# andrewginns/quorum

Measured on AMD Instinct MI355X. Metric: proxied req/sec (whole node) + p50 TTFT, 2-backend concatenate stream at 1/2/4/8 GPU, higher is better.
Workload: dtype bytes (utf-8 SSE text; no float compute)

## Files before the change

quorum_amd/csrc/qmx_engine.cpp:

```cpp
#include "qmx_env.h"
#include "qmx_engine.h"

#include <cstdlib>
#include <ctime>

#include <algorithm>
#include <cstdio>
#include <cstring>
#include <stdexcept>

namespace qmx {

const char* kDeltaSuffix = "\"}, \"finish_reason\": null}]}\n\n";
const char* kFinalSuffix = "\"}, \"finish_reason\": \"stop\"}]}\n\n";

TagSet make_tagset(const std::vector<std::string>& tags) {
  TagSet ts;
  std::memset(&ts, 0, sizeof(ts));
  std::vector<std::string> seen;
  for (const auto& t0 : tags) {
    std::string t;
    for (char c : t0) t.push_back((char)lower_ascii((uint8_t)c));
    if (std::find(seen.begin(), seen.end(), t) != seen.end()) continue;
    for (char ch : t) {
// ... 271 lines not shown
  int slot;
  if (!free_.empty()) {
    slot = free_.back();
    free_.pop_back();
  } else {
    slot = (int)meta_.size();
    meta_.emplace_back();
    core_.emplace_back();
  }
  open_reserved(slot, index, filter, emit, gen);
  return slot;
}

void HostEngine::reserve(int k, std::vector<int>& out) {
  std::lock_guard<std::mutex> g(mu_);
  for (int i = 0; i < k; ++i) {
    if (!free_.empty()) {
      out.push_back(free_.back());
      free_.pop_back();
    } else {
      out.push_back((int)meta_.size());
      meta_.emplace_back();
      core_.emplace_back();
    }
  }
}

void HostEngine::open_reserved(int slot, int index, bool filter, bool emit, uint32_t* gen) {
  auto recycle = [](std::string& x) {
    if (x.capacity() > (64u << 10)) std::string().swap(x);
    else x.clear();
  };
  Meta& m = meta_[slot];
  m.gen += 1;
  m.live = true;
  m.dirty = m.eof = m.closed = m.busy = false;
  m.fresh = true;
  recycle(m.incoming);
  if (gen) *gen = m.gen;
  SlotCore& c = core_[slot];
  c.filter = filter;
  c.emit = emit;
  c.started = c.aborted = c.done = false;
  c.index = index;
  recycle(c.carry);
  c.fs = FilterState();
  recycle(c.content);
  recycle(c.tpl_pre);
  recycle(c.tpl_suf);
}

void HostEngine::feed(int slot, const std::string& data) {
  std::lock_guard<std::mutex> g(mu_);
  feed_locked(slot, data);
}

void HostEngine::finish(int slot) {
  std::lock_guard<std::mutex> g(mu_);
  finish_locked(slot);
}

void HostEngine::release(int slot) {
  std::lock_guard<std::mutex> g(mu_);
  release_locked(slot);
}

void HostEngine::apply_ops(std::vector<EngineOp>& ops, bool move_data) {
  std::lock_guard<std::mutex> g(mu_);
  for (auto& op : ops) {
    if (op.kind == EngineOp::FEED) {
      if (move_data) feed_locked_move(op.slot, op.data);
      else feed_locked(op.slot, op.data);
    }
    else if (op.kind == EngineOp::FINISH) finish_locked(op.slot);
    else release_locked(op.slot);
  }
}

void HostEngine::feed_locked(int slot, const std::string& data) {
  if (slot < 0 || slot >= (int)meta_.size() || !meta_[slot].live) return;
  Meta& m = meta_[slot];
  m.incoming += data;
  bytes_in_ += data.size();
  if (!m.dirty) {
    m.dirty = true;
    m.t_dirty = mono_s();
    dirty_.push_back(slot);
  }
}

void HostEngine::feed_locked_move(int slot, std::string& data) {
  if (slot < 0 || slot >= (int)meta_.size() || !meta_[slot].live) return;
  if (!meta_[slot].incoming.empty()) return feed_locked(slot, data);
  bytes_in_ += data.size();
  meta_[slot].incoming.swap(data);
  Meta& m = meta_[slot];
  if (!m.dirty) {
    m.dirty = true;
    m.t_dirty = mono_s();
    dirty_.push_back(slot);
  }
}

void HostEngine::finish_locked(int slot) {
  if (slot < 0 || slot >= (int)meta_.size() || !meta_[slot].live) return;
  Meta& m = meta_[slot];
  m.eof = true;
  if (!m.dirty) {
    m.dirty = true;
    m.t_dirty = mono_s();
    dirty_.push_back(slot);
  }
}

void HostEngine::release_locked(int slot) {
  if (slot < 0 || slot >= (int)meta_.size() || !meta_[slot].live) return;
  meta_[slot].live = false;
  meta_[slot].incoming.clear();
  pending_free_.push_back(slot);
}

int HostEngine::submit_finalize(const std::vector<int>& slots, bool strip, bool texts, const std::string& joiner,
                                int64_t created) {
  std::lock_guard<std::mutex> g(mu_);
  FinalizeReq r{++next_fid_, slots, strip, texts, joiner, created};
  fin_.push_back(std::move(r));
  return next_fid_;
}

bool HostEngine::has_work() {
  std::lock_guard<std::mutex> g(mu_);
  if (!fin_.empty()) return true;
  for (int s : dirty_)
    if (!meta_[s].busy) return true;
  return false;
}

bool HostEngine::pending(int slot) {
  std::lock_guard<std::mutex> g(mu_);
  if (slot < 0 || slot >= (int)meta_.size()) return false;
  const Meta& m = meta_[slot];
  return m.live && (m.dirty || m.busy || !m.incoming.empty());
}

bool HostEngine::job_take(Job& j, bool allow_fin) {
  j.work.clear();
  j.fin.clear();
  thread_local std::vector<int> keep;
  keep.clear();
  std::lock_guard<std::mutex> g(mu_);
  for (int s : pending_free_) {
    if (meta_[s].busy) {
      keep.push_back(s);
      continue;
    }
    on_free(s);
    free_.push_back(s);
  }
  pending_free_.swap(keep);
  keep.clear();
  j.work.reserve(dirty_.size());
  double now = 0;
  for (int s : dirty_) {
    Meta& m = meta_[s];
    if (m.busy && m.live) {
      keep.push_back(s);
      continue;
    }
    m.dirty = false;
    if (!m.live) continue;
    if (m.t_dirty > 0) {
      if (now == 0) now = mono_s();
      take_wait_s_ += now - m.t_dirty;
      ++takes_;
    }
    Work w{s, std::string(), m.eof, m.fresh};
    w.data.swap(m.incoming);
    m.fresh = false;
    m.busy = true;
    j.work.push_back(std::move(w));
  }
  dirty_.swap(keep);
  if (allow_fin) j.fin.swap(fin_);
  if (!j.work.empty() || !j.fin.empty()) ++ticks_;
  return !j.work.empty() || !j.fin.empty();
}

void HostEngine::job_finish(Job& j, std::vector<SlotResult>& results, std::vector<int>& taken) {
  size_t out = 0;
  for (auto& r : results) out += r.size();
  for (auto& w : j.work) taken.push_back(w.slot);
  std::lock_guard<std::mutex> g(mu_);
  bytes_out_ += out;
  for (auto& r : results) r.gen = meta_[r.slot].gen;
}

bool HostEngine::tick(int64_t created, std::vector<SlotResult>& results, std::vector<FinalizeRes>& fres, int lane,
                      std::vector<int>* taken) {
  thread_local Job j;
  thread_local std::vector<int> slots;
  slots.clear();
  if (!job_take(j, true)) return false;
  run_tick(j.work, j.fin, created, results, fres, lane);
  std::vector<int>& tk = taken ? *taken : slots;
  job_finish(j, results, tk);
  if (!taken) settle(slots);
  return true;
}

void HostEngine::settle(const std::vector<int>& taken) {
  std::lock_guard<std::mutex> g(mu_);
  for (int s : taken) meta_[s].busy = false;
}

std::string HostEngine::text(int slot) {
  if (slot < 0 || slot >= (int)nslots()) return std::string();
  const SlotCore& c = core_[slot];
  return c.aborted ? std::string() : c.content;
}

size_t HostEngine::content_size(int slot) {
  if (slot < 0 || slot >= (int)nslots()) return 0;
  return core_[slot].content.size();
}

void HostEngine::set_remote_content(int slot, const std::string* bytes, size_t len, bool ) {
  if (slot < 0 || slot >= (int)nslots()) return;
  core_[slot].content = bytes ? *bytes : std::string(len, '\0');
}

std::unordered_map<std::string, double> HostEngine::stats() {
  std::lock_guard<std::mutex> g(mu_);
  return {{"ticks", (double)ticks_}, {"bytes_in", (double)bytes_in_}, {"bytes_out", (double)bytes_out_},
          {"takes", (double)takes_}, {"take_wait_us", take_wait_s_ * 1e6},
          {"slots", (double)meta_.size()}, {"free", (double)free_.size()}};
// ... 18 lines not shown
  }
}

}

namespace qmx {

struct AsyncCpuEngine::Done {
  std::vector<SlotResult> results;
  std::vector<FinalizeRes> fres;
  std::atomic<bool> ready{false};
};

AsyncCpuEngine::AsyncCpuEngine(const std::vector<std::string>& tags) : CpuEngine(tags) {
  th_ = std::thread([this] { run(); });
}

AsyncCpuEngine::~AsyncCpuEngine() {
  {
    std::lock_guard<std::mutex> g(qmu_);
    stop_ = true;
  }
  qcv_.notify_all();
  if (th_.joinable()) th_.join();
}

void AsyncCpuEngine::job_post(Job& j) {
  auto d = std::make_shared<Done>();
  j.impl = d;
  inflight_.fetch_add(1, std::memory_order_acq_rel);
  {
    std::lock_guard<std::mutex> g(qmu_);
    q_.push_back(&j);
  }
  qcv_.notify_one();
}

void AsyncCpuEngine::run() {
  for (;;) {
    Job* j = nullptr;
    {
      std::unique_lock<std::mutex> lk(qmu_);
      qcv_.wait(lk, [this] { return stop_ || !q_.empty(); });
      if (q_.empty()) return;
      j = q_.front();
      q_.erase(q_.begin());
    }
    auto d = std::static_pointer_cast<Done>(j->impl);
    run_tick(j->work, j->fin, j->created, d->results, d->fres, 0);
    d->ready.store(true, std::memory_order_release);
  }
}

bool AsyncCpuEngine::job_ready(Job& j, double* expect_us) {
  if (expect_us) *expect_us = 5.0;
  auto d = std::static_pointer_cast<Done>(j.impl);
  return !d || d->ready.load(std::memory_order_acquire);
}

void AsyncCpuEngine::job_complete(Job& j, std::vector<SlotResult>& results, std::vector<FinalizeRes>& fres) {
  auto d = std::static_pointer_cast<Done>(j.impl);
  if (!d) return;
  for (auto& r : d->results) results.push_back(std::move(r));
  for (auto& f : d->fres) fres.push_back(std::move(f));
  j.impl.reset();
  inflight_.fetch_sub(1, std::memory_order_acq_rel);
}

}
```

quorum_amd/csrc/qmx_engine.h:

```cpp
#pragma once
#include <stdint.h>

#include <atomic>
#include <condition_variable>
#include <memory>
#include <thread>
#include <mutex>
#include <string>
#include <unordered_map>
#include <stdexcept>
#include <unordered_set>
#include <vector>

#include "qmx_text.h"

namespace qmx {

enum ResultFlags : int { RF_DONE = 1, RF_ABORTED = 2, RF_ESCALATED = 4 };

TagSet make_tagset(const std::vector<std::string>& tags);

struct FilterState {
  int depth = 0;
  int tail_len = 0;
// ... 82 lines not shown

template <class T>
class SlotTable {
 public:
  static constexpr int kShift = 8, kChunk = 1 << kShift, kMaxChunks = 4096;
  SlotTable() : chunks_(new std::unique_ptr<T[]>[kMaxChunks]) {}
  T& operator[](size_t i) { return chunks_[i >> kShift][i & (kChunk - 1)]; }
  const T& operator[](size_t i) const { return chunks_[i >> kShift][i & (kChunk - 1)]; }
  size_t size() const { return n_.load(std::memory_order_acquire); }
  void emplace_back() {
    const size_t n = n_.load(std::memory_order_relaxed);
    if ((n >> kShift) >= (size_t)kMaxChunks) throw std::length_error("slot table full");
    if ((n & (kChunk - 1)) == 0) chunks_[n >> kShift].reset(new T[kChunk]());
    n_.store(n + 1, std::memory_order_release);
  }

 private:
  std::unique_ptr<std::unique_ptr<T[]>[]> chunks_;
  std::atomic<size_t> n_{0};
};

class HostEngine {
 public:
  explicit HostEngine(const std::vector<std::string>& tags);
  virtual ~HostEngine() = default;

  int open(int index, bool filter, bool emit, uint32_t* gen = nullptr);
  void reserve(int k, std::vector<int>& out);
  void open_reserved(int slot, int index, bool filter, bool emit, uint32_t* gen = nullptr);
  void feed(int slot, const std::string& data);
  void finish(int slot);
  void release(int slot);
  void apply_ops(std::vector<EngineOp>& ops, bool move_data = false);
  int submit_finalize(const std::vector<int>& slots, bool strip, bool texts, const std::string& joiner,
                      int64_t created);
  bool has_work();
  bool pending(int slot);
  bool tick(int64_t created, std::vector<SlotResult>& results, std::vector<FinalizeRes>& fres, int lane = 0,
            std::vector<int>* taken = nullptr);
  void settle(const std::vector<int>& taken);

  struct Work {
    int slot;
    std::string data;
    bool eof;
    bool fresh;
  };
  struct Job {
    std::vector<Work> work;
    std::vector<FinalizeReq> fin;
    int64_t created = 0;
    int lane = 0;
    bool live = false;
    std::shared_ptr<void> impl;
  };
  virtual bool pipelined() const { return false; }
  bool pipeline_ = false;
  bool job_take(Job& j, bool allow_fin);
  virtual void job_prepare(Job&) {}
  virtual void job_post(Job&) {}
  virtual void job_wait_near(Job&) {}
  virtual void job_complete(Job&, std::vector<SlotResult>&, std::vector<FinalizeRes>&) {}
  void job_finish(Job& j, std::vector<SlotResult>& results, std::vector<int>& taken);
  virtual bool async_jobs() const { return false; }
  virtual bool job_ready(Job&, double* expect_us = nullptr) {
    if (expect_us) *expect_us = 0;
    return true;
  }
  virtual int free_doors() const { return 1; }
  virtual std::string text(int slot);
  virtual std::unordered_map<std::string, double> stats();
  virtual void* content_device_ptr(int , size_t* cap) {
    *cap = 0;
    return nullptr;
  }
  virtual size_t content_size(int slot);
  virtual void set_remote_content(int slot, const std::string* bytes, size_t len, bool host_copied = false);

  const TagSet& tagset() const { return ts_; }

 protected:
  virtual void run_tick(std::vector<Work>& work, std::vector<FinalizeReq>& fin, int64_t created,
                        std::vector<SlotResult>& results, std::vector<FinalizeRes>& fres, int lane) = 0;
  virtual void on_free(int ) {}

  void feed_locked(int slot, const std::string& data);
  void feed_locked_move(int slot, std::string& data);
  void finish_locked(int slot);
  void release_locked(int slot);

  struct Meta {
    bool live = false;
    bool dirty = false;
    bool eof = false;
    bool fresh = true;
    bool closed = false;
    bool busy = false;
    uint32_t gen = 0;
    double t_dirty = 0;
    std::string incoming;
  };

  TagSet ts_;
  std::mutex mu_;
  SlotTable<Meta> meta_;
  SlotTable<SlotCore> core_;
  size_t nslots() const { return core_.size(); }
  std::vector<int> free_, pending_free_;
  std::vector<int> dirty_;
  std::vector<FinalizeReq> fin_;
  int next_fid_ = 0;
  uint64_t ticks_ = 0, bytes_in_ = 0, bytes_out_ = 0, takes_ = 0;
  double take_wait_s_ = 0;
};

class CpuEngine : public HostEngine {
 public:
  explicit CpuEngine(const std::vector<std::string>& tags) : HostEngine(tags) {}
  bool pipelined() const override { return pipeline_; }
  void job_complete(Job& j, std::vector<SlotResult>& results, std::vector<FinalizeRes>& fres) override {
    run_tick(j.work, j.fin, j.created, results, fres, j.lane);
  }

 protected:
  void run_tick(std::vector<Work>& work, std::vector<FinalizeReq>& fin, int64_t created,
                std::vector<SlotResult>& results, std::vector<FinalizeRes>& fres, int lane) override;
};

class AsyncCpuEngine : public CpuEngine {
 public:
  explicit AsyncCpuEngine(const std::vector<std::string>& tags);
  ~AsyncCpuEngine() override;
  bool async_jobs() const override { return true; }
  void job_post(Job& j) override;
  bool job_ready(Job& j, double* expect_us = nullptr) override;
  void job_complete(Job& j, std::vector<SlotResult>& results, std::vector<FinalizeRes>& fres) override;
  int free_doors() const override { return 2 - inflight_.load(std::memory_order_acquire); }

 private:
  struct Done;
  void run();
  std::mutex qmu_;
  std::condition_variable qcv_;
  std::vector<Job*> q_;
  bool stop_ = false;
  std::atomic<int> inflight_{0};
  std::thread th_;
};

void finalize_texts(const TagSet& ts, const std::vector<std::string>& texts, const FinalizeReq& r,
                    FinalizeRes& out);

}
```

quorum_amd/csrc/qmx_hip.h:

```cpp
#pragma once
#include <hip/hip_runtime.h>

#include <atomic>
#include <chrono>
#include <cstddef>
#include <functional>
#include <memory>
#include <mutex>
#include <shared_mutex>
#include <vector>

#include "qmx_engine.h"
#include "qmx_streams.h"

namespace qmx {

struct WorkItem {
  uint32_t slot, in_off, in_len, out_off, out_cap, flags, index, content_len;
};
struct WorkResult {
  uint32_t consumed, out_len, status, content_len;
  uint32_t seq;
  uint32_t pad;
  uint64_t t0, t1;
// ... 154 lines not shown
  uint64_t launches = 0, items = 0, h2d_bytes = 0, d2h_bytes = 0;
  uint64_t s3_full = 0, s3_tpl = 0, s3_events = 0, stage_n = 0;
  uint64_t s3_cyc_full = 0, s3_cyc_tpl = 0, s3_cyc_lex = 0, s3_hole = 0, s3_cyc_hole = 0;
  uint64_t s3a_unres = 0;
  double kernel_ms = 0.0, host_prep_us = 0, gpu_wait_us = 0, process_us = 0;
  double first_result_us = 0;
  double item_us = 0, start_spread_us = 0;
  double items_host_us = 0;
  double relay_us = 0, pickup_us = 0, grid_span_us = 0, grid_ticks = 0;
  double stage_us[38] = {0};
  double clk_cycles = 0, clk_us = 0;
  FinItem* h_fin = nullptr;
  size_t fin_cap = 0;
  FinResult* h_finres = nullptr;
  size_t finres_cap = 0;
  FinText* h_fint = nullptr;
  size_t fint_cap = 0;
  uint8_t* h_fin_in = nullptr;
  size_t fin_in_cap = 0;
  uint8_t* h_fout = nullptr;
  size_t fout_cap = 0;
  uint32_t* h_tl = nullptr;
  size_t tl_cap = 0;
  uint8_t* d_join = nullptr;
  size_t join_cap = 0;
  uint8_t* d_fout = nullptr;
  size_t dfout_cap = 0;
  uint8_t* d_segs = nullptr;
  size_t segs_cap = 0;
  uint64_t fin_launches = 0, fin_items = 0, fin_host = 0;
  uint64_t fin_staged = 0;
  uint32_t seq = 0;
  double ema_us = 40.0;
  double span_ema_us = 30.0;
  double lead_ema_us = 8.0;
  double post_seen_us = 0, done_host_us = 0, hop_ticks = 0;
  double clo = -1e300, chi = 1e300, clo_prev = -1e300, cwin_t0 = 0, cwin_sum = 0, cwin_n = 0;
  bool timing_pending = false;
  uint64_t poll_fallbacks = 0;
  PDoor* h_door = nullptr;
  PCtl* d_ctl = nullptr;
  bool p_running = false;
  uint32_t p_gen = 0;
  double p_last_post = 0;
  uint64_t p_revivals = 0;
  uint64_t p_launches = 0, p_ticks = 0;
};

class HipEngine : public HostEngine {
 public:
  HipEngine(const std::vector<std::string>& tags, int device, int tile_bytes, int max_slots, int content_cap,
            int lanes = 1, HipGrid* grid = nullptr, int door = -1, int ndoors = 1);
  ~HipEngine() override;
  bool job_ready(Job& j, double* expect_us = nullptr) override;
  bool async_jobs() const override { return grid_ != nullptr; }
  int free_doors() const override;
  std::string text(int slot) override;
  void* content_device_ptr(int slot, size_t* cap) override;
  size_t content_size(int slot) override;
  void set_remote_content(int slot, const std::string* bytes, size_t len, bool host_copied = false) override;
  void set_remote_hbm_direct(bool on) { remote_hbm_direct_ = on; }
  bool remote_hbm_direct() const { return remote_hbm_direct_; }
  std::unordered_map<std::string, double> kernel_stats();
  int lanes() const { return (int)lanes_.size(); }
  void host_open(int slot);

 protected:
  void run_tick(std::vector<Work>& work, std::vector<FinalizeReq>& fin, int64_t created,
                std::vector<SlotResult>& results, std::vector<FinalizeRes>& fres, int lane) override;
  void on_free(int slot) override;

 public:
  bool pipelined() const override { return poll_ && pipeline_; }
  void job_prepare(Job& j) override;
  void job_post(Job& j) override;
  void job_wait_near(Job& j) override;
  void job_complete(Job& j, std::vector<SlotResult>& results, std::vector<FinalizeRes>& fres) override;

 private:
  struct HipJob;
  HipJob& hjob(Job& j);
  void prepare(HipJob& J);
  void post(HipJob& J);
  void wait_near(HipJob& J);
  void complete(HipJob& J, std::vector<SlotResult>& results, std::vector<FinalizeRes>& fres);
  void escalate(int slot, bool fresh);
  void finalize_host(const FinalizeReq& r, std::vector<FinalizeRes>& out);
  std::vector<const FinalizeReq*> prep_finalize(TickLane& L, std::vector<FinalizeReq>& fin,
                                                std::vector<const FinalizeReq*>& host);
  void collect_finalize(TickLane& L, const std::vector<const FinalizeReq*>& gpu, std::vector<FinalizeRes>& out);
  void wait_stream(TickLane& L);
  void wait_results(TickLane& L, int n, int m, uint32_t seq, const WorkResult* res,
                    std::chrono::steady_clock::time_point t0, const std::function<void(int)>& on_item);
  void collect_timing(TickLane& L);
  void ensure_in(TickLane::Buf& B, size_t bytes);
  void ensure_out(TickLane& L, size_t bytes);
  void build_params(TickLane& L, int64_t created);
  std::string device_content(int slot, uint32_t len);
  uint32_t next_seq(TickLane& L);
  void ensure_persistent(TickLane& L);
  void stop_persistent(TickLane& L);
  void retire_host(void* p);
  void retire_dev(void* p);
  void note_alloc(double t0, size_t bytes);
  std::atomic<uint64_t> allocs_{0}, alloc_bytes_{0};
  std::atomic<double> alloc_us_{0.0}, alloc_max_us_{0.0};

 public:
  void* halloc(size_t bytes);
  void* dalloc(size_t bytes);

 private:
  std::vector<void*> grave_host_, grave_dev_;
  std::mutex grave_mu_;

  int device_;
  int tile_;
  int max_slots_;
  uint32_t content_cap_;
  KParams base_params_;
  std::vector<std::unique_ptr<TickLane>> lanes_;
  DevSlot* d_state_ = nullptr;
  uint8_t* d_content_ = nullptr;
  std::vector<uint8_t> host_mode_;
  std::vector<uint8_t> remote_host_;
  std::vector<uint32_t> content_len_;
  std::atomic<uint64_t> escalations_{0}, fin_host_{0}, remote_dev_{0}, remote_staged_{0}, remote_copied_{0},
      remote_copied_inline_{0}, light_opens_{0},
      requeues_{0};
  bool remote_hbm_direct_ = true;
  int spin_us_ = 0;
  bool poll_ = true;
  int poll_us_ = 1;
  bool persistent_ = true;
  bool views_ = true;
  bool keep_stale_records_ = false;
  bool stage_timing_ = false;
  int p_grid_ = 64;
  int p_idle_ms_ = 50;
  HipGrid* grid_ = nullptr;
  int door_ = -1;
  int ndoors_ = 1;
  std::vector<char> door_busy_;

 public:
  bool persistent() const { return persistent_; }
// ... 6 lines not shown
```

quorum_amd/csrc/qmx_hip.hip:

```cpp
#include "qmx_env.h"
#include "qmx_hip.h"
#include "qmx_streams.h"

#include <rocprofiler-sdk-roctx/roctx.h>

#include <sched.h>
#include <sys/prctl.h>
#include <time.h>

#include <chrono>
#include <thread>

#include "qmx_lex.h"

#include <algorithm>
#include <cstdio>
#include <cstdlib>
#include <cstring>
#include <stdexcept>
#include <string>

namespace qmx {

#define HIP_CHECK(x)                                                                       \
// ... 2679 lines not shown
    if (ndone == n && null_done) {
      last = 1e3 * (steady_s() - t0);
      break;
    }
    sched_yield();
  }
  const double t1 = steady_s();
  bool drained = false;
  while (steady_s() - t1 < 5.0) {
    bool all = hipEventQuery(ev) == hipSuccess;
    for (int i = 0; i < n && all; ++i) all = done(i);
    if (all) {
      drained = true;
      break;
    }
    std::this_thread::sleep_for(std::chrono::milliseconds(1));
  }
  if (drained) {
    for (hipStream_t s : st) stream_destroy(s, StreamKind::Shared);
    hipEventDestroy(ev);
    hipFree(dsrc);
    hipHostFree(marks);
  }
  return {{"streams", (double)n}, {"completed", (double)ndone}, {"null_stream_copy_done", null_done ? 1.0 : 0.0},
          {"all_done_ms", last}, {"drained", drained ? 1.0 : 0.0}};
}

std::unordered_map<std::string, double> stream_stats() {
  const char* hq = env_get("GPU_MAX_HW_QUEUES");
  const int queues = hq ? std::max(1, atoi(hq)) : 4;
  const int ex = g_streams_excl.load(), sh = g_streams_shared.load();
  const bool own = exclusive_queues();
  return {{"streams_shared", (double)sh},
          {"streams_exclusive", (double)ex},
          {"streams_created", (double)g_streams_created.load()},
          {"hw_queues_per_priority", (double)queues},
          {"grid_queue_exclusive", own ? 1.0 : 0.0},
          {"grid_queue_ok", own && ex <= queues ? 1.0 : 0.0}};
}

void HipEngine::wait_stream(TickLane& L) {
  HIP_CHECK(hipEventRecord(L.evb, L.stream));
  if (spin_us_ > 0) {
    const auto t0 = std::chrono::steady_clock::now();
    while (hipEventQuery(L.evb) == hipErrorNotReady) {
      if (std::chrono::steady_clock::now() - t0 > std::chrono::microseconds(spin_us_)) break;
      sched_yield();
    }
  }
  HIP_CHECK(hipEventSynchronize(L.evb));
}

void HipEngine::wait_results(TickLane& L, int n, int m, uint32_t seq, const WorkResult* res,
                             std::chrono::steady_clock::time_point t0, const std::function<void(int)>& on_item) {
  using HC = std::chrono::steady_clock;
  static thread_local bool slack = (prctl(PR_SET_TIMERSLACK, 1000UL, 0, 0, 0), true);
  (void)slack;
  auto nap = [](double us) {
    if (us < 1) return;
    timespec ts{0, (long)(us * 1000)};
    nanosleep(&ts, nullptr);
  };
  auto done = [&](int& i) {
    while (i < n && __atomic_load_n(&res[i].seq, __ATOMIC_ACQUIRE) == seq) on_item(i++);
    while (i >= n && i < n + m && __atomic_load_n(&L.h_finres[i - n].seq, __ATOMIC_ACQUIRE) == seq) ++i;
    return i == n + m;
  };
  int i = 0;
  bool revived = false;
  double revive_at = 2e5;
  nap(0.6 * L.ema_us - 6.0 - std::chrono::duration<double, std::micro>(HC::now() - t0).count());
  while (!done(i)) {
    const double el = std::chrono::duration<double, std::micro>(HC::now() - t0).count();
    if (grid_) {
      if (el > revive_at) {
        revive_at = el + 1e5;
        grid_->revive_if_exited();
      }
      if (el > 1e7)
        throw std::runtime_error("tick results missing after 10 s (door " + std::to_string(door_) + ", seq " +
                                 std::to_string(seq) + ", relayed " +
                                 std::to_string(__atomic_load_n(&L.h_door->relayed, __ATOMIC_ACQUIRE)) + ")");
      nap(el < 2e3 ? poll_us_ : 50.0);
      continue;
    }
    if (L.p_running && !revived && el > 2.0 * L.ema_us + 500.0) {
      const uint32_t ex = __atomic_load_n(&L.h_door->exits, __ATOMIC_ACQUIRE);
      const uint32_t rl = __atomic_load_n(&L.h_door->relayed, __ATOMIC_ACQUIRE);
      if ((ex >> 16) == 1 && (ex & 0xffffu) == (L.p_gen & 0xffffu) && rl != seq) {
        uint32_t seq0 = seq - 1;
        if (seq0 == 0) seq0 = (uint32_t)-1;
        HIP_CHECK(hipStreamSynchronize(L.stream));
        L.h_door->base = seq0;
        hipLaunchKernelGGL(qmx_tick_persistent<2>, dim3(p_grid_), dim3(BS), 0, L.stream, L.h_door, L.d_ctl, p_grid_,
                           ++L.p_gen, (uint32_t)p_idle_ms_ * 100000u, 0);
        HIP_CHECK(hipGetLastError());
        L.p_last_post = steady_s();
        ++L.p_launches;
        ++L.p_revivals;
        revived = true;
        continue;
      }
    }
    if (el > (L.p_running ? 1e6 : 4.0 * L.ema_us + 2000.0)) {
      if (L.p_running) stop_persistent(L);
      else HIP_CHECK(hipStreamSynchronize(L.stream));
      ++L.poll_fallbacks;
      if (!done(i)) {
        std::string why = "tick results missing after the lane drained (seq " + std::to_string(seq) + ", " +
                          std::to_string(i) + "/" + std::to_string(n + m) + " published";
        if (L.h_door)
          why += "; grid: relayed " + std::to_string(__atomic_load_n(&L.h_door->relayed, __ATOMIC_ACQUIRE)) +
                 ", exits " + std::to_string(L.h_door->exits) + ", last idle exit after " +
                 std::to_string(L.h_door->idle_limit_hit_us) + " us, launches " + std::to_string(L.p_launches) +
                 ", posted " + std::to_string(L.h_door->posted);
        throw std::runtime_error(why + ")");
      }
      break;
    }
    if (el < spin_us_) {
      sched_yield();
      continue;
    }
    nap(poll_us_);
  }
  const double tot = std::chrono::duration<double, std::micro>(HC::now() - t0).count();
  L.ema_us = 0.85 * L.ema_us + 0.15 * std::min(tot, 2000.0);
}

void HipEngine::collect_timing(TickLane& L) {
  if (!L.timing_pending) return;
  L.timing_pending = false;
  HIP_CHECK(hipEventSynchronize(L.ev1));
  float ms = 0.f;
  if (hipEventElapsedTime(&ms, L.ev0, L.ev1) == hipSuccess) L.kernel_ms += ms;
}

HipEngine::HipEngine(const std::vector<std::string>& tags, int device, int tile_bytes, int max_slots,
                     int content_cap, int lanes, HipGrid* grid, int door, int ndoors)
    : HostEngine(tags),
      device_(device),
      tile_(std::min(std::max(tile_bytes, 1024), TILE_MAX) & ~15),
      max_slots_(max_slots),
      content_cap_((uint32_t)content_cap),
      grid_(grid),
      door_(door),
      ndoors_(grid ? std::min(std::max(ndoors, 1), 2) : 1) {
  HIP_CHECK(hipSetDevice(device_));
  if (grid_ && (door_ < 0 || door_ + ndoors_ > grid_->doors())) throw std::invalid_argument("HipEngine: door out of range");
  if (grid_) lanes = 1;
  door_busy_.assign(ndoors_, 0);
  if (const char* sp = env_get("QMX_WAIT_SPIN_US")) spin_us_ = atoi(sp);
  if (const char* w = env_get("QMX_WAIT")) poll_ = std::string(w) != "event";
  if (const char* pu = env_get("QMX_POLL_US")) poll_us_ = std::max(1, atoi(pu));
  if (const char* gs = env_get("QMX_GPU_SHARERS")) persistent_ = atoi(gs) <= 1;
  if (const char* pe = env_get("QMX_PERSISTENT")) persistent_ = atoi(pe) != 0;
  if (const char* va = env_get("QMX_VIEWS")) views_ = atoi(va) != 0;
  keep_stale_records_ = env_get("QMX_DEBUG_STALE_RECORDS") != nullptr;
  stage_timing_ = env_get("QMX_STAGE_TIMING") != nullptr;
  if (const char* pw = env_get("QMX_PERSISTENT_WG")) p_grid_ = std::min(std::max(8, atoi(pw)), 1024);
  if (const char* pi = env_get("QMX_PERSISTENT_IDLE_MS")) p_idle_ms_ = std::min(std::max(5, atoi(pi)), 1000);
  {
    const char* hq = env_get("GPU_MAX_HW_QUEUES");
    const int queues = hq ? std::max(1, atoi(hq)) : 4;
    if (persistent_ && lanes > (exclusive_queues() ? queues : queues - 1)) persistent_ = false;
  }
  if (grid_) {
    persistent_ = false;
    poll_ = true;
  }
  HIP_CHECK(hipMalloc(&d_state_, sizeof(DevSlot) * (size_t)max_slots_));
  HIP_CHECK(hipMemset(d_state_, 0, sizeof(DevSlot) * (size_t)max_slots_));
  HIP_CHECK(hipMalloc(&d_content_, (size_t)content_cap_ * (size_t)max_slots_));

  std::memset(&base_params_, 0, sizeof(base_params_));
  base_params_.ts = ts_;
  base_params_.npat = 2 * ts_.n;
  {
    int next = 1;
    for (int b = 0; b < 256; ++b) base_params_.code[b] = 95;
// ... 303 lines not shown
  }
  content_len_[slot] = (uint32_t)len;
}

void HipEngine::host_open(int slot) {
  if (slot >= 0 && slot < max_slots_) {
    host_mode_[slot] = 1;
    remote_host_[slot] = 0;
    content_len_[slot] = 0;
  }
  ++light_opens_;
}

void HipEngine::escalate(int slot, bool fresh) {
  SlotCore& c = core_[slot];
  if (!fresh) {
    DevSlot ds;
    HIP_CHECK(hipMemcpy(&ds, d_state_ + slot, sizeof(DevSlot), hipMemcpyDeviceToHost));
    c.fs.depth = ds.depth;
    c.fs.tail_len = ds.tail_len;
    std::memcpy(c.fs.tail, ds.tail, kMaxTail);
  } else {
    c.fs = FilterState();
  }
  if (!remote_host_[slot]) c.content = device_content(slot, content_len_[slot]);
  remote_host_[slot] = 0;
  host_mode_[slot] = 1;
  ++escalations_;
}

std::string HipEngine::text(int slot) {
  if (slot < 0 || slot >= (int)nslots()) return std::string();
  const SlotCore& c = core_[slot];
  if (c.aborted) return std::string();
  if (slot >= max_slots_ || host_mode_[slot] || remote_host_[slot]) return c.content;
  return device_content(slot, content_len_[slot]);
}

struct HipEngine::HipJob {
  struct Pending {
    int slot;
    size_t carry_len;
    size_t submitted;
    bool eof_sent;
    Work* w;
  };
  std::vector<Work>* work = nullptr;
  std::vector<FinalizeReq>* fin = nullptr;
  int64_t created = 0;
  int lane = 0, n = 0, m = 0;
  int dk = 0;
  uint32_t seq = 0;
  bool persist = false, new_params = false, posted = false;
  std::vector<Pending> pend;
  std::vector<int> requeue;
  std::vector<Work*> order;
  std::vector<Work*> b[8];
  std::vector<const FinalizeReq*> fin_gpu, fin_host;
  std::vector<SlotResult> host_results;
  TickLane::Buf* B = nullptr;
  TickLane::OutArena* arena = nullptr;
  size_t in_off = 0;
  std::chrono::steady_clock::time_point tp0, tp1;
};

void HipEngine::prepare(HipJob& J) {
  TickLane& L = *lanes_[(size_t)J.lane % lanes_.size()];
  std::lock_guard<std::mutex> lg(L.mu);
  using HC = std::chrono::steady_clock;
  J.tp0 = HC::now();
  J.pend.clear();
  J.requeue.clear();
  J.order.clear();
  J.host_results.clear();
  J.fin_gpu.clear();
  J.fin_host.clear();
  J.posted = false;
  std::vector<Work>& work = *J.work;
  TickLane::Buf* bp = nullptr;
  for (TickLane::Buf& b : L.bufs)
    if (!b.busy) {
      bp = &b;
      break;
    }
  if (!bp) throw std::logic_error("tick prepared with both buffer sets in use");
  TickLane::Buf& B = *bp;
  B.busy = true;
  J.B = &B;
  size_t out_need = 0;
  for (auto& w : work) {
    size_t tot = core_[w.slot].carry.size() + w.data.size();
    size_t sub = std::min(tot, (size_t)tile_);
    out_need += ((12 * sub + 1024) + 15) & ~(size_t)15;
  }
  ensure_in(B, work.size() * (size_t)TILE_MAX + kSpecTile + 64);
  ensure_out(L, out_need + 64);
  J.arena = L.out;
  J.arena->refs.fetch_add(1, std::memory_order_relaxed);
  if (work.size() > B.items_cap) {
    retire_host(B.h_items);
    retire_host(B.h_res);
    B.items_cap = work.size() * 2;
    B.h_items = (WorkItem*)halloc(sizeof(WorkItem) * B.items_cap);
    B.h_res = (WorkResult*)halloc(sizeof(WorkResult) * B.items_cap);
    std::memset((void*)B.h_res, 0, sizeof(WorkResult) * B.items_cap);
  }
// ... 35 lines not shown
    size_t cl = c.carry.size(), tot = cl + w.data.size();
    size_t sub = std::min(tot, (size_t)tile_);
    bool eof_sent = w.eof && sub == tot;
    in_off = (size_t)n * TILE_MAX;
    size_t a = std::min(cl, sub);
    std::memcpy(B.h_in + in_off, c.carry.data(), a);
    if (sub > a) std::memcpy(B.h_in + in_off + a, w.data.data(), sub - a);
    WorkItem& it = B.h_items[n];
    it.slot = (uint32_t)slot;
    it.in_off = (uint32_t)in_off;
    it.in_len = (uint32_t)sub;
    it.out_off = (uint32_t)out_off;
    it.out_cap = (uint32_t)(12 * sub + 1024);
    it.flags = (eof_sent ? WF_EOF : 0) | (c.filter ? WF_FILTER : 0) | (c.emit ? WF_EMIT : 0) |
               (c.started ? WF_STARTED : 0) | (w.fresh ? WF_FRESH : 0);
    it.index = (uint32_t)c.index;
    if (c.index >= 0 && c.index < kBackendTpl && !(pub_mask & (1u << c.index))) {
      pub_mask |= 1u << c.index;
      it.flags |= WF_PUBLISH;
    }
    it.content_len = content_len_[slot];
    in_bytes += sub;
    out_off += ((size_t)it.out_cap + 15) & ~(size_t)15;
    J.pend.push_back({slot, cl, sub, eof_sent, &w});
    ++n;
  }
  J.n = n;
  J.in_off = in_bytes;
  J.fin_gpu = prep_finalize(L, *J.fin, J.fin_host);
  J.m = (int)J.fin_gpu.size();
  if (!keep_stale_records_) {
    for (int i = 0; i < n; ++i) __atomic_store_n(&B.h_res[i].seq, 0u, __ATOMIC_RELAXED);
    for (int i = 0; i < J.m; ++i) __atomic_store_n(&L.h_finres[i].seq, 0u, __ATOMIC_RELAXED);
  }
  if (n + J.m > 0) {
    if (J.created != L.params_created) {
      build_params(L, J.created);
      L.params_created = J.created;
      ++L.params_ver;
    }
    unsigned long long* const dbg0 = L.params.dbg;
    L.params.dbg = nullptr;
    if (stage_timing_) {
      if (B.dbg_cap < (size_t)n) {
        if (B.h_dbg) retire_host(B.h_dbg);
        B.dbg_cap = std::max((size_t)n, B.items_cap);
        HIP_CHECK(hipHostMalloc((void**)&B.h_dbg, sizeof(unsigned long long) * kDbg * B.dbg_cap, hipHostMallocMapped));
      }
      std::memset(B.h_dbg, 0, sizeof(unsigned long long) * kDbg * n);
      L.params.dbg = B.h_dbg;
    }
    if (L.params.dbg != dbg0) ++L.params_ver;
  }
  J.tp1 = HC::now();
  L.host_prep_us += std::chrono::duration<double, std::micro>(J.tp1 - J.tp0).count();
}

void HipEngine::post(HipJob& J) {
  if (J.n + J.m == 0) return;
  TickLane& L = *lanes_[(size_t)J.lane % lanes_.size()];
  std::lock_guard<std::mutex> lg(L.mu);
  TickLane::Buf& B = *J.B;
  J.persist = grid_ || (persistent_ && poll_);
  if (!J.persist && L.p_running) stop_persistent(L);
  J.new_params = B.params_ver != L.params_ver;
  if (J.new_params) {
    std::memcpy(B.h_params, &L.params, sizeof(KParams));
    if (!J.persist) HIP_CHECK(hipMemcpyAsync(B.d_params, B.h_params, sizeof(KParams), hipMemcpyHostToDevice, L.stream));
    B.params_ver = L.params_ver;
  }
  J.tp1 = std::chrono::steady_clock::now();
  roctxRangePushA("qmx_tick");
  L.h2d_bytes += J.in_off;
  J.dk = 0;
  if (grid_) {
    while (J.dk < ndoors_ && door_busy_[J.dk]) ++J.dk;
    if (J.dk == ndoors_) throw std::logic_error("tick posted with every door of the engine busy");
  }
  const uint32_t par = L.tpl_launches[J.dk] & 1;
  BackendTpl* const tpl = L.d_btpl + (size_t)J.dk * 2 * kBackendTpl;
  FinArgs fa{L.h_fin, L.h_fint, L.h_fin_in, L.d_join, L.d_fout, L.h_fout, L.h_finres, L.h_tl, (int2*)L.d_segs};
  if (grid_) {
    auto guard = grid_->post_guard();
    PDoor* door = grid_->door(door_ + J.dk);
    door_busy_[J.dk] = 1;
    uint32_t s = door->posted + 1;
    if (s == 0) s = 1;
    J.seq = s;
    TickDesc& d = door->d;
    d.items = B.h_items;
    d.in = B.h_in;
    d.out = J.arena->p;
    d.res = B.h_res;
    d.params = B.d_params;
    d.params_src = J.new_params ? B.h_params : nullptr;
    d.btpl_rd = tpl + (size_t)(par ^ 1) * kBackendTpl;
    d.btpl_wr = tpl + (size_t)par * kBackendTpl;
    d.fa = fa;
    d.state = d_state_;
    d.content = d_content_;
    d.seq = s;
    d.n_tick = (uint32_t)J.n;
    d.n_fin = (uint32_t)J.m;
    d.stop = 0;
    __atomic_store_n(&door->posted, s, __ATOMIC_RELEASE);
    grid_->note_post();
    ++L.p_ticks;
    J.posted = true;
    return;
  }
  if (J.persist) ensure_persistent(L);
  J.seq = next_seq(L);
  if (!poll_) HIP_CHECK(hipEventRecord(L.ev0, L.stream));
  if (J.persist) {
    TickDesc& d = L.h_door->d;
    d.items = B.h_items;
    d.in = B.h_in;
    d.out = J.arena->p;
    d.res = B.h_res;
    d.params = B.d_params;
    d.params_src = J.new_params ? B.h_params : nullptr;
    d.btpl_rd = tpl + (size_t)(par ^ 1) * kBackendTpl;
    d.btpl_wr = tpl + (size_t)par * kBackendTpl;
    d.fa = fa;
    d.state = d_state_;
    d.content = d_content_;
    d.seq = J.seq;
    d.n_tick = (uint32_t)J.n;
    d.n_fin = (uint32_t)J.m;
    d.stop = 0;
    __atomic_store_n(&L.h_door->posted, J.seq, __ATOMIC_RELEASE);
    L.p_last_post = steady_s();
    ++L.p_ticks;
  } else {
    hipLaunchKernelGGL(qmx_tick_kernel, dim3(J.n + J.m), dim3(BS), 0, L.stream, B.h_items, B.h_in, J.arena->p,
                       B.h_res, d_state_, d_content_, B.d_params, J.seq, (uint32_t)J.n, fa,
                       tpl + (size_t)(par ^ 1) * kBackendTpl, tpl + (size_t)par * kBackendTpl);
    HIP_CHECK(hipGetLastError());
  }
  J.posted = true;
}

void HipEngine::wait_near(HipJob& J) {
  if (!J.posted) return;
  TickLane& L = *lanes_[(size_t)J.lane % lanes_.size()];
  const double el = std::chrono::duration<double, std::micro>(std::chrono::steady_clock::now() - J.tp1).count();
  const double prep = L.launches ? L.host_prep_us / (double)L.launches : 5.0;
  const double target = L.span_ema_us + 6.0 - prep;
  if (target - el >= 2.0) {
    timespec ts{0, (long)((target - el) * 1000)};
    nanosleep(&ts, nullptr);
  }
}

void HipEngine::complete(HipJob& J, std::vector<SlotResult>& results, std::vector<FinalizeRes>& fres) {
  TickLane& L = *lanes_[(size_t)J.lane % lanes_.size()];
  std::lock_guard<std::mutex> lg(L.mu);
  using HC = std::chrono::steady_clock;
  for (auto& r : J.host_results) results.push_back(std::move(r));
  J.host_results.clear();
  const int n = J.n, m = J.m;
  TickLane::Buf& B = *J.B;
  int n_done = 0;
  auto process_item = [&](int i) {
    HipJob::Pending& p = J.pend[i];
    SlotCore& c = core_[p.slot];
    const WorkResult r = B.h_res[i];
    Work& w = *p.w;
    auto keep_remainder = [&](size_t consumed) {
      const size_t cl = p.carry_len;
      if (consumed < cl) {
        c.carry.erase(0, consumed);
        c.carry += w.data;
      } else {
        c.carry.assign(w.data, consumed - cl, std::string::npos);
      }
    };
    bool no_progress = (r.status & WS_ESCALATE) ||
                       (p.submitted == (size_t)tile_ && r.consumed == 0 && !(r.status & (WS_DONE | WS_ABORTED)));
    if (no_progress) {
      escalate(p.slot, w.fresh);
      keep_remainder(0);
      std::string all;
      all.swap(c.carry);
      bool was_closed = c.done || c.aborted;
      std::string o;
      process_slot(ts_, c, (const uint8_t*)all.data(), all.size(), w.eof, J.created, o);
      int flags = (c.done ? RF_DONE : 0) | (c.aborted ? RF_ABORTED : 0) | RF_ESCALATED;
      if (!o.empty() || ((flags & (RF_DONE | RF_ABORTED)) && !was_closed)) results.push_back({p.slot, std::move(o), flags});
      return;
    }
    if (r.status & WS_STARTED) c.started = true;
    content_len_[p.slot] = r.content_len;
    int flags = 0;
    if (r.status & WS_ABORTED) {
      c.aborted = true;
      c.carry.clear();
      flags |= RF_ABORTED;
    } else {
      keep_remainder(r.consumed);
      if (r.status & WS_DONE) {
        c.done = true;
        c.carry.clear();
        flags |= RF_DONE;
      } else if ((r.status & WS_MORE) || p.submitted < p.carry_len + w.data.size()) {
        J.requeue.push_back(p.slot);
        if (r.status & WS_MORE) ++requeues_;
      }
    }
    L.d2h_bytes += r.out_len;
    const char* bytes = (const char*)J.arena->p + B.h_items[i].out_off;
    if (r.out_len && !views_) {
      results.push_back({p.slot, std::string(bytes, r.out_len), flags});
    } else if (r.out_len) {
      SlotResult x{p.slot, std::string(), flags};
      x.view = bytes;
      x.view_len = r.out_len;
      x.hold = ViewRef(&J.arena->refs);
      results.push_back(std::move(x));
    } else if (flags) {
      results.push_back({p.slot, std::string(), flags});
    }
  };
  if (J.posted) {
    for (const FinalizeReq* r : J.fin_host) finalize_host(*r, fres);
    if (poll_) {
      wait_results(L, n, m, J.seq, B.h_res, J.tp1, [&](int i) {
        const auto ti = HC::now();
        if (n_done == 0) L.first_result_us += std::chrono::duration<double, std::micro>(ti - J.tp1).count();
        if (i == n_done) process_item(n_done++);
        L.items_host_us += std::chrono::duration<double, std::micro>(HC::now() - ti).count();
      });
      uint64_t a = ~0ull, b = 0, t0max = 0;
      double item_ticks = 0;
      for (int i = 0; i < n; ++i) {
        a = std::min(a, B.h_res[i].t0);
        b = std::max(b, B.h_res[i].t1);
        t0max = std::max(t0max, B.h_res[i].t0);
        item_ticks += (double)(B.h_res[i].t1 - B.h_res[i].t0);
      }
      if (n > 0) {
        L.item_us += item_ticks * 1e-2 / n;
        L.start_spread_us += (double)(t0max - a) * 1e-2;
      }
      if (J.persist && n > 0) {
        const PDoor* dr = grid_ ? grid_->door(door_ + J.dk) : L.h_door;
        const uint64_t ts = __atomic_load_n(&dr->t_seen, __ATOMIC_ACQUIRE);
        const uint64_t tr = __atomic_load_n(&dr->t_relayed, __ATOMIC_ACQUIRE);
        if (ts && tr >= ts && a >= tr && b >= a) {
          L.lead_ema_us = 0.85 * L.lead_ema_us + 0.15 * std::min((double)(a - ts) * 1e-2, 500.0);
          if (grid_) {
            const double post_h = std::chrono::duration<double, std::micro>(J.tp1.time_since_epoch()).count();
            const double now_h = std::chrono::duration<double, std::micro>(HC::now().time_since_epoch()).count();
            const double lo = post_h - (double)ts * 1e-2, hi = now_h - (double)b * 1e-2;
            if (now_h - L.cwin_t0 > 1e5) {
              L.clo_prev = L.clo;
              if (L.clo > -1e299 && L.chi < 1e299 && L.chi >= L.clo) {
                L.cwin_sum += L.chi - L.clo;
                ++L.cwin_n;
              }
              L.clo = -1e300;
              L.chi = 1e300;
              L.cwin_t0 = now_h;
            }
            L.clo = std::max(L.clo, lo);
            L.chi = std::min(L.chi, hi);
            const double off = std::max(L.clo, L.clo_prev);
            const double seen_h = (double)ts * 1e-2 + off, done_h = (double)b * 1e-2 + off;
            if (seen_h >= post_h - 5.0 && now_h >= done_h - 5.0) {
              L.post_seen_us += seen_h - post_h;
              L.done_host_us += now_h - done_h;
              ++L.hop_ticks;
            }
          }
          L.relay_us += (double)(tr - ts) * 1e-2;
          L.pickup_us += (double)(a - tr) * 1e-2;
          L.grid_span_us += (double)(b - ts) * 1e-2;
          ++L.grid_ticks;
        }
      }
      for (int i = 0; i < m; ++i) {
        a = std::min(a, L.h_finres[i].t0);
        b = std::max(b, L.h_finres[i].t1);
      }
      if (b > a) {
        L.kernel_ms += (double)(b - a) * 1e-5;
        L.span_ema_us = 0.85 * L.span_ema_us + 0.15 * std::min((double)(b - a) * 1e-2, 2000.0);
      }
    } else {
      HIP_CHECK(hipEventRecord(L.ev1, L.stream));
      wait_stream(L);
      L.timing_pending = true;
      collect_timing(L);
    }
    roctxRangePop();
    L.gpu_wait_us += std::chrono::duration<double, std::micro>(HC::now() - J.tp1).count();
    ++L.launches;
    ++L.tpl_launches[J.dk];
    if (grid_) door_busy_[J.dk] = 0;
    L.items += n;
    if (m > 0) {
      ++L.fin_launches;
      L.fin_items += m;
    }
    if (L.params.dbg && L.params.dbg == B.h_dbg) {
      for (int i = 0; i < n; ++i) {
        const unsigned long long* d = B.h_dbg + kDbg * i;
        if (d[12] > d[11] && d[10] > d[0]) {
          L.clk_cycles += (double)(d[12] - d[11]);
          L.clk_us += (double)(d[10] - d[0]) * 0.01;
        }
        int prev = 0;
        for (int k = 1; k < 11; ++k) {
          if (!d[k]) continue;
          L.stage_us[k] += (double)(d[k] - d[prev]) * 0.01;
          prev = k;
        }
        auto sub = [&](int slot, int a, int b) {
          if (d[a] && d[b] && d[b] >= d[a]) L.stage_us[slot] += (double)(d[b] - d[a]) * 0.01;
        };
        sub(11, 3, 21);
        sub(12, 21, 22);
        sub(13, 22, 4);
        sub(14, 5, 23);
        sub(15, 23, 24);
        sub(16, 23, 25);
        sub(17, 25, 24);
        sub(18, 9, 26);
        sub(19, 26, 10);
        sub(21, 5, 28);
        sub(22, 28, 29);
        sub(23, 29, 23);
        sub(24, 25, 30);
        sub(25, 30, 31);
        sub(26, 31, 24);
        sub(27, 24, 32);
        sub(28, 32, 33);
        sub(29, 33, 7);
        sub(30, 3, 34);
        sub(31, 34, 21);
        sub(32, 3, 35);
        sub(33, 35, 36);
        sub(34, 36, 34);
        sub(35, 35, 38);
        sub(36, 38, 39);
        sub(37, 39, 36);
        if (d[27] && d[27] >= B.h_res[i].t1 && B.h_res[i].t1) L.stage_us[20] += (double)(d[27] - B.h_res[i].t1) * 0.01;
      }
      L.stage_n += n;
      for (int i = 0; i < n; ++i) {
        L.s3_full += B.h_dbg[kDbg * i + 13];
        L.s3_tpl += B.h_dbg[kDbg * i + 14];
        L.s3_events += B.h_dbg[kDbg * i + 15];
        L.s3_cyc_full += B.h_dbg[kDbg * i + 16];
        L.s3_cyc_tpl += B.h_dbg[kDbg * i + 17];
        L.s3_cyc_lex += B.h_dbg[kDbg * i + 18];
        L.s3_hole += B.h_dbg[kDbg * i + 19];
        L.s3_cyc_hole += B.h_dbg[kDbg * i + 20];
        L.s3a_unres += B.h_dbg[kDbg * i + 37];
      }
    }
  }
  for (; n_done < n; ++n_done) process_item(n_done);
  if (m > 0) collect_finalize(L, J.fin_gpu, fres);
  if (!J.posted)
    for (const FinalizeReq* r : J.fin_host) finalize_host(*r, fres);
  if (!J.requeue.empty()) {
    std::lock_guard<std::mutex> g(mu_);
    for (int s : J.requeue) {
      Meta& mt = meta_[s];
      if (!mt.live || mt.dirty) continue;
      mt.dirty = true;
      dirty_.push_back(s);
    }
  }
  J.arena->refs.fetch_sub(1, std::memory_order_release);
  J.B->busy = false;
  L.process_us += std::chrono::duration<double, std::micro>(HC::now() - J.tp0).count();
}

void HipEngine::run_tick(std::vector<Work>& work, std::vector<FinalizeReq>& fin, int64_t created,
                         std::vector<SlotResult>& results, std::vector<FinalizeRes>& fres, int lane) {
  thread_local HipJob J;
  J.work = &work;
  J.fin = &fin;
  J.created = created;
  J.lane = lane;
  prepare(J);
  post(J);
  complete(J, results, fres);
}

HipEngine::HipJob& HipEngine::hjob(Job& j) {
  if (!j.impl) j.impl = std::make_shared<HipJob>();
  HipJob& J = *std::static_pointer_cast<HipJob>(j.impl);
  J.work = &j.work;
  J.fin = &j.fin;
  J.created = j.created;
  J.lane = j.lane;
  return J;
}
int HipEngine::free_doors() const {
  int k = 0;
  for (char b : door_busy_) k += !b;
  return k;
}

bool HipEngine::job_ready(Job& j, double* expect_us) {
  HipJob& J = hjob(j);
  if (expect_us) *expect_us = 0;
  if (!J.posted) return true;
  TickLane& L = *lanes_[(size_t)J.lane % lanes_.size()];
  const WorkResult* res = J.B->h_res;
  for (int i = 0; i < J.n; ++i)
    if (__atomic_load_n(&res[i].seq, __ATOMIC_ACQUIRE) != J.seq) goto pending;
  for (int i = 0; i < J.m; ++i)
    if (__atomic_load_n(&L.h_finres[i].seq, __ATOMIC_ACQUIRE) != J.seq) goto pending;
  return true;
pending:
  if (expect_us)
    *expect_us = L.lead_ema_us + L.span_ema_us + 3.0 -
                 std::chrono::duration<double, std::micro>(std::chrono::steady_clock::now() - J.tp1).count();
  return false;
}

void HipEngine::job_prepare(Job& j) { prepare(hjob(j)); }
void HipEngine::job_post(Job& j) { post(hjob(j)); }
void HipEngine::job_wait_near(Job& j) { wait_near(hjob(j)); }
void HipEngine::job_complete(Job& j, std::vector<SlotResult>& results, std::vector<FinalizeRes>& fres) {
  complete(hjob(j), results, fres);
}

void HipEngine::finalize_host(const FinalizeReq& r, std::vector<FinalizeRes>& out) {
  std::vector<std::string> texts;
  for (int s : r.slots) texts.push_back(text(s));
  FinalizeRes fr;
  finalize_texts(ts_, texts, r, fr);
  out.push_back(std::move(fr));
  ++fin_host_;
}

template <class T>
static void grow_mapped(HipEngine* e, T** p, size_t* cap, size_t need, void (HipEngine::*retire)(void*)) {
  if (need <= *cap) return;
  if (*p) (e->*retire)(*p);
  *cap = std::max(need, *cap * 2);
  *p = (T*)e->halloc(sizeof(T) * *cap + 64);
  std::memset((void*)*p, 0, sizeof(T) * *cap + 64);
}
static void grow_device(HipEngine* e, uint8_t** p, size_t* cap, size_t need, void (HipEngine::*retire)(void*)) {
  if (need <= *cap) return;
  if (*p) (e->*retire)(*p);
  *cap = std::max(need, *cap * 2);
  *p = (uint8_t*)e->dalloc(*cap + 64);
}

std::vector<const FinalizeReq*> HipEngine::prep_finalize(TickLane& L, std::vector<FinalizeReq>& reqs,
                                                         std::vector<const FinalizeReq*>& host) {
  std::vector<const FinalizeReq*> gpu;
  if (reqs.empty()) return gpu;
  const int nsl = (int)nslots();
  size_t ntext = 0, in_bytes = 0;
  for (auto& r : reqs) {
    bool dev = true;
    for (int s : r.slots) dev = dev && s >= 0 && s < max_slots_ && s < nsl && !host_mode_[s];
    if (!dev) {
      host.push_back(&r);
      continue;
    }
    gpu.push_back(&r);
    ntext += r.slots.size();
    in_bytes += ((r.joiner.size() + 15) & ~(size_t)15) + 256 + 64;
    for (int s : r.slots)
      if (remote_host_[s] && !core_[s].aborted) in_bytes += (content_len_[s] + 15) & ~(size_t)15;
  }
// ... 372 lines not shown
```

quorum_amd/csrc/qmx_server.cpp:

```cpp
#include "qmx_env.h"
#include "qmx_server.h"

#include <arpa/inet.h>
#include <errno.h>
#include <fcntl.h>
#include <netdb.h>
#include <netinet/tcp.h>
#include <signal.h>
#include <sys/epoll.h>
#include <sys/syscall.h>
#include <dirent.h>
#include <sys/resource.h>
#include <sys/ioctl.h>
#include <sys/eventfd.h>
#include <sys/prctl.h>
#include <sys/socket.h>
#include <unistd.h>

#include <algorithm>
#include <atomic>
#include <chrono>
#include <condition_variable>
#include <cstdio>
#include <cstring>
#include <memory>
#include <mutex>
#include <thread>

#include <functional>
#include <map>

#include <openssl/err.h>
#include <openssl/ssl.h>
#include <openssl/x509v3.h>

#include "qmx_engine.h"
#include "qmx_exchange.h"
#include "qmx_hip.h"
#include "qmx_json.h"
#include "qmx_prof.h"

namespace qmx {
namespace {

std::atomic<bool> g_stop{false};
std::atomic<bool> g_drain{false};
std::atomic<int> g_ready{0};
std::atomic<uint64_t> c_requests{0}, c_stream{0}, c_nonstream{0}, c_errors{0}, c_up_fail{0}, c_ticks{0},
    c_tick_slots{0}, c_up_conns{0}, c_clients{0}, c_remote_streams{0},
    c_route_ns{0},
    c_flush_ns{0}, c_flushes{0},
    c_apply_ns{0}, c_applies{0},
    c_link_msgs{0},
    c_coalesced{0},
    c_hold_ns{0}, c_holds{0},
    c_hold_deadline{0};
std::atomic<uint64_t> c_fail_connect{0}, c_fail_timeout{0}, c_fail_status{0}, c_fail_disconnect{0},
    c_fail_protocol{0}, c_stream_aborts{0},
    c_host_path_opens{0};
std::atomic<uint64_t> c_sp_failed{0}, c_sp_aborted{0}, c_sp_empty{0}, c_sp_text{0}, c_sp_down{0},
    c_sp_delta_mismatch{0}, c_sp_nodata{0} ,
    c_sp_eager{0} ,
    c_sp_release_deferred{0} ,
    c_sp_fetched{0} ;
std::atomic<uint64_t> c_loop_pass_1ms{0}, c_loop_pass_5ms{0};
std::atomic<uint64_t> c_paced{0};
std::atomic<int> g_sp_logs{0};

struct Hist {
  static constexpr int N = 17;
  static constexpr double le[N] = {1e-4, 2.5e-4, 5e-4, 1e-3, 2.5e-3, 5e-3, 1e-2, 2.5e-2, 5e-2,
                                   0.1,  0.25,   0.5,  1.0,  2.5,    5.0,  10.0, 30.0};
  std::atomic<uint64_t> b[N + 1];
  std::atomic<uint64_t> count{0}, sum_ns{0};
  Hist() {
    for (auto& x : b) x.store(0);
  }
  void observe(double sec) {
    int i = 0;
// ... 2 lines not shown
    count++;
    sum_ns += (uint64_t)(sec * 1e9);
  }
  void render(std::string& m, const std::string& name, const std::string& labels = std::string()) const {
    uint64_t acc = 0;
    const std::string sep = labels.empty() ? "" : ",";
    for (int i = 0; i <= N; ++i) {
      acc += b[i].load();
      char le_s[32];
      if (i < N) snprintf(le_s, sizeof(le_s), "%g", le[i]);
      else snprintf(le_s, sizeof(le_s), "+Inf");
      m += name + "_bucket{" + labels + sep + "le=\"" + le_s + "\"} " + std::to_string(acc) + "\n";
    }
    m += name + "_sum" + (labels.empty() ? "" : "{" + labels + "}") + " " + std::to_string(sum_ns.load() / 1e9) + "\n";
    m += name + "_count" + (labels.empty() ? "" : "{" + labels + "}") + " " + std::to_string(acc) + "\n";
  }
};
constexpr double Hist::le[Hist::N];
Hist h_ttft, h_latency, h_tick, h_upstream_ttfb, h_engine;
Hist h_sp_first, h_sp_final;

using Clock = std::chrono::steady_clock;
inline double now_s() { return std::chrono::duration<double>(Clock::now().time_since_epoch()).count(); }
inline bool env_flag(const char* name, bool dflt) {
  const char* v = env_get(name);
  if (!v || !*v) return dflt;
  return !(std::strcmp(v, "0") == 0 || std::strcmp(v, "false") == 0);
}

inline char alow(unsigned char c) { return (char)(c - 'A' < 26u ? c | 0x20 : c); }
inline const char* find_crlf(const char* p, size_t n) {
  const char* e = p + n;
  while (p < e) {
    const char* r = (const char*)memchr(p, '\r', (size_t)(e - p));
    if (!r || r + 1 >= e) return nullptr;
    if (r[1] == '\n') return r;
    p = r + 1;
  }
  return nullptr;
}
inline const char* find_crlfcrlf(const char* p, size_t n) {
  const char* e = p + n;
  while (p < e) {
    const char* r = find_crlf(p, (size_t)(e - p));
    if (!r || r + 3 >= e) return nullptr;
    if (r[2] == '\r' && r[3] == '\n') return r;
    p = r + 2;
  }
  return nullptr;
}
template <class F>
void for_each_header(const char* p, size_t n, F&& f) {
  auto ws = [](char ch) { return ch == ' ' || ch == '\t'; };
  size_t pos = 0;
  while (pos < n) {
    const char* e0 = find_crlf(p + pos, n - pos);
    size_t e = e0 ? (size_t)(e0 - p) : n;
    const char* colon = (const char*)memchr(p + pos, ':', e - pos);
    if (colon) {
      size_t ka = pos, kb = (size_t)(colon - p);
      while (ka < kb && ws(p[ka])) ++ka;
      while (kb > ka && (ws(p[kb - 1]) || p[kb - 1] == '\r')) --kb;
      size_t va = (size_t)(colon - p) + 1, vb = e;
      while (va < vb && ws(p[va])) ++va;
      while (vb > va && (ws(p[vb - 1]) || p[vb - 1] == '\r')) --vb;
      std::string k(p + ka, kb - ka);
      for (auto& ch : k) ch = alow((unsigned char)ch);
      f(std::move(k), std::string(p + va, vb - va));
    }
    pos = e + 2;
  }
}
bool ieq(const std::string& s, const char* lw) {
  size_t n = strlen(lw);
  if (s.size() != n) return false;
  for (size_t i = 0; i < n; ++i)
    if (alow((unsigned char)s[i]) != lw[i]) return false;
  return true;
}
bool icontains(const std::string& s, const char* lw) {
  size_t n = strlen(lw);
  for (size_t i = 0; i + n <= s.size(); ++i) {
    size_t j = 0;
    while (j < n && alow((unsigned char)s[i + j]) == lw[j]) ++j;
    if (j == n) return true;
  }
  return false;
}
const char* reason(int st) {
  switch (st) {
    case 200: return "OK";
    case 400: return "Bad Request";
    case 401: return "Unauthorized";
    case 404: return "Not Found";
    case 500: return "Internal Server Error";
    case 502: return "Bad Gateway";
    case 503: return "Service Unavailable";
    default: return "Status";
  }
}
inline int chunk_head(char* h, size_t len) {
  static const char* d = "0123456789abcdef";
  char t[16];
  int k = 0;
  do {
    t[k++] = d[len & 15];
    len >>= 4;
  } while (len);
  for (int i = 0; i < k; ++i) h[i] = t[k - 1 - i];
  h[k] = '\r';
  h[k + 1] = '\n';
  return k + 2;
}
inline int dec_str(char* o, size_t v) {
  char t[24];
  int k = 0;
  do {
    t[k++] = (char)('0' + v % 10);
    v /= 10;
  } while (v);
  for (int i = 0; i < k; ++i) o[i] = t[k - 1 - i];
  return k;
}
std::string chunk(const std::string& s) {
  char h[24];
  const int n = chunk_head(h, s.size());
  std::string r;
  r.reserve(n + s.size() + 2);
  r.append(h, n).append(s).append("\r\n");
  return r;
}
std::string err_json(const std::string& msg, const char* type) {
  JVal e;
// ... 15 lines not shown
  r += body;
  return r;
}
const char* kSseHdr =
    "HTTP/1.1 200 OK\r\ncontent-type: text/event-stream; charset=utf-8\r\ntransfer-encoding: chunked\r\n\r\n";
const char* kDone = "data: [DONE]\n\n";

std::string chunk_event_json(const char* id, int64_t created, const std::string& model_json,
                             const std::string& delta_json, const char* finish) {
  return std::string("data: {\"id\": \"") + id + "\", \"object\": \"chat.completion.chunk\", \"created\": " +
         std::to_string(created) + ", \"model\": " + model_json + ", \"choices\": [{\"index\": 0, \"delta\": " +
         delta_json + ", \"finish_reason\": " + finish + "}]}\n\n";
}

struct RespParser {
  int phase = 0;
  int status = 0;
  bool keep_headers = true;
  std::vector<std::pair<std::string, std::string>> headers;
  long remaining = 0;
  bool close = false;
  std::string buf;
  int feed(const char* p, size_t n, std::string& out) {
    const char* d = p;
    size_t len = n;
    if (!buf.empty()) {
      buf.append(p, n);
      d = buf.data();
      len = buf.size();
    }
    out.reserve(out.size() + n);
    auto find = [&](const char* pat, size_t pl, size_t from) -> size_t {
      if (from > len) return std::string::npos;
      const void* f = pl == 2 && pat[0] == '\r' && pat[1] == '\n' ? find_crlf(d + from, len - from)
                      : pl == 4 && memcmp(pat, "\r\n\r\n", 4) == 0 ? find_crlfcrlf(d + from, len - from)
                                                                  : memmem(d + from, len - from, pat, pl);
      return f ? (size_t)((const char*)f - d) : std::string::npos;
    };
    size_t i = 0;
    while (phase != 7) {
      if (phase == 0) {
        size_t he = find("\r\n\r\n", 4, i);
        if (he == std::string::npos) break;
        const char* hp = d + i;
        size_t hn = he - i;
        i = he + 4;
        const char* le0 = find_crlf(hp, hn);
        size_t le = le0 ? (size_t)(le0 - hp) : hn;
        if (le < 12 || memcmp(hp, "HTTP/", 5) != 0) return -1;
        status = 0;
        for (size_t k = 9; k < le && hp[k] >= '0' && hp[k] <= '9'; ++k) status = status * 10 + (hp[k] - '0');
        bool chunked = false, has_len = false;
        size_t pos = le0 ? le + 2 : hn;
        for_each_header(hp + pos, hn - pos, [&](std::string&& k, std::string&& v) {
          if (k == "transfer-encoding" && icontains(v, "chunked")) chunked = true;
          if (k == "content-length") {
            has_len = true;
            remaining = atol(v.c_str());
          }
          if (k == "connection" && ieq(v, "close")) close = true;
          if (keep_headers) headers.emplace_back(std::move(k), std::move(v));
        });
        if (status == 204 || status == 304) phase = 7;
        else if (chunked) phase = 2;
        else if (has_len) phase = remaining > 0 ? 1 : 7;
        else {
          phase = 6;
          close = true;
        }
        continue;
      }
      if (phase == 1) {
        size_t take = std::min((size_t)remaining, len - i);
        out.append(d + i, take);
        i += take;
        remaining -= take;
        if (remaining == 0) phase = 7;
        break;
      }
      if (phase == 6) {
        out.append(d + i, len - i);
        i = len;
        break;
      }
      if (phase == 2) {
        size_t le = find("\r\n", 2, i);
        if (le == std::string::npos) break;
        remaining = strtol(d + i, nullptr, 16);
        i = le + 2;
        phase = remaining == 0 ? 5 : 3;
        continue;
      }
      if (phase == 3) {
        size_t take = std::min((size_t)remaining, len - i);
        out.append(d + i, take);
        i += take;
        remaining -= take;
        if (remaining > 0) break;
        phase = 4;
        continue;
      }
      if (phase == 4) {
        if (len - i < 2) break;
        i += 2;
        phase = 2;
        continue;
      }
      if (phase == 5) {
        size_t le = find("\r\n", 2, i);
        if (le == std::string::npos) break;
        bool empty = le == i;
        i = le + 2;
        if (empty) phase = 7;
        continue;
      }
    }
    if (d == p) buf.assign(p + i, n - i);
    else buf.erase(0, i);
    return 0;
  }
  bool done() const { return phase == 7; }
  const std::string* header(const std::string& k) const {
    for (auto& h : headers)
      if (h.first == k) return &h.second;
    return nullptr;
  }
};

struct Session;
struct Client {
  int fd = -1;
  std::string in, out;
  size_t out_off = 0;
  Session* sess = nullptr;
  bool keepalive = true;
  bool dead = false;
  bool close_after = false;
  bool queued = false;
  int served = 0;
  uint64_t serial = 0;
  double t_accept = 0;
  bool want_out = false;
  bool held = false;
  double held_t0 = 0;
};

enum UpMode { UP_ENGINE, UP_BUFFER, UP_PASS };
struct Up {
  int fd = -1;
  int backend = -1;
  Session* sess = nullptr;
  int bi = -1;
  UpMode mode = UP_BUFFER;
  std::string req;
  size_t req_off = 0;
  bool connecting = false, reused = false, got_bytes = false, headers_seen = false;
  RespParser rp;
  std::string body;
  double last_io = 0, deadline = 0, timeout = 60, t_open = 0;
  SSL* ssl = nullptr;
  bool tls_hs = false;
  bool out_armed = false;
};

struct BState {
  int backend = -1;
  int slot = -1;
  int remote = -1;
  int rx_data = 0;
  double t_sp_open = 0, t_sp_last = 0;
  bool via_link = false;
  bool bulk_waiting = false;
  XMsg bulk_msg;
  Up* up = nullptr;
  int state = 0;
  int status = 0;
  bool aborted = false;
  double t_fed = 0;
  bool is_json = false;
  JVal js;
  std::string text;
  std::vector<std::pair<std::string, std::string>> rheaders;
};

enum SKind { K_PAR, K_SINGLE, K_NONSTREAM, K_REMOTE };
struct Session {
  Client* cl = nullptr;
  SKind kind = K_PAR;
  JVal body;
  std::string raw;
  std::vector<std::pair<std::string, std::string>> fwd;
  std::string auth;
  std::vector<BState> bs;
  int finished = 0;
  bool filter = true, emit = true;
  int stage = 0;
  int fin_id = -1;
  bool fin_texts = false;
  std::vector<std::string> texts;
  std::vector<std::string> text_names;
  Up* agg = nullptr;
  bool msplit = false;
  std::string mpre, mpost;
  std::string first_buf;
  bool first_decided = false, saw_done = false, pass_started = false;
  std::string done_tail;
  std::string role_model_json;
  double t0 = 0;
  uint64_t skey = 0;
  int remote_n = 0;
  int owner_rank = -1, owner_loop = 0, shadow_bi = 0;
  bool via_link = false;
  uint64_t owner_skey = 0;
  int data_sent = 0;
  bool bulk_pending = false;
  bool fetching = false, fetched = false;
  std::string fetched_text;
  bool first_content = false;
};

struct ResultBatch {
  std::vector<SlotResult> r;
  std::vector<FinalizeRes> f;
  double t_routed = 0;
};

std::atomic<uint64_t> c_verify_checked{0}, c_verify_mismatch{0};

class Verifier {
 public:
  explicit Verifier(const std::vector<std::string>& tags) : cpu_(tags) {}
  void open(int slot, uint32_t gen, int index, bool f, bool e) {
    std::lock_guard<std::mutex> g(mu_);
    Track t;
    t.gen = gen;
    t.shadow = cpu_.open(index, f, e);
    rmap_[t.shadow] = slot;
    map_[slot] = std::move(t);
  }
  void feed(int slot, const std::string& d) {
    std::lock_guard<std::mutex> g(mu_);
    auto it = map_.find(slot);
    if (it != map_.end()) cpu_.feed(it->second.shadow, d);
  }
// ... 365 lines not shown

class Loop {
 public:
  Loop(const ServerCfg& cfg, int idx) : cfg_(cfg), idx_(idx) { xfd_ = eventfd(0, EFD_NONBLOCK); }
  void attach_exchange(Exchange* x) { xch_ = x; }
  int index() const { return idx_; }
  void attach_hub(GpuHub* h) {
    hub_ = h;
    if (h)
      h->attach(idx_, [this](ResultBatch&& rb) {
        {
          std::lock_guard<std::mutex> g(rmu_);
          rq_.push_back(std::move(rb));
        }
        rq_pending_.store(true, std::memory_order_seq_cst);
        if (lazy_wake_ && !in_wait_.load(std::memory_order_seq_cst)) return;
        uint64_t one = 1;
        ssize_t w = write(evfd_, &one, 8);
        (void)w;
      });
  }
  void attach_tls(SSL_CTX* t) { tls_ = t; }
  void attach_grid(HipGrid* g) { grid_ = g; }
  void attach_loops(const std::vector<Loop*>* ls) { loops_ = ls; }
  std::mutex smu_;
  std::unordered_map<std::string, double> snap_;
  std::atomic<double> pass_max_{0.0};
  std::atomic<double> pass_t0_{0.0};
  std::atomic<int> tid_{0};
  enum { SC_CLIENT_SEND, SC_UP_SEND, SC_RECV, SC_EPOLL_WAIT, SC_EPOLL_CTL, SC_WAKE_READ, SC_N };
  std::atomic<uint64_t> sc_[SC_N] = {};
  void cnt(int i) { sc_[i].store(sc_[i].load(std::memory_order_relaxed) + 1, std::memory_order_relaxed); }
  void snapshot() {
    if (!eng_) return;
    std::unordered_map<std::string, double> m;
    for (auto& kv : eng_->stats()) m["qmx_engine_" + kv.first] = kv.second;
    if (heng_)
      for (auto& kv : heng_->kernel_stats()) m["qmx_kernel_" + kv.first] = kv.second;
    std::lock_guard<std::mutex> g(smu_);
    snap_.swap(m);
  }
  void x_deliver(std::vector<XMsg>&& v) {
    {
      std::lock_guard<std::mutex> g(xmu_);
      for (auto& m : v) xin_.push_back(std::move(m));
    }
    uint64_t one = 1;
    ssize_t w = write(xfd_, &one, 8);
    (void)w;
  }
  ~Loop() {
    for (int fd : {lfd_, afd_})
      if (fd >= 0) close(fd);
    for (auto& kv : idle_ssl_) SSL_free(kv.second);
    for (auto& kv : ups_)
      if (kv.second->ssl) SSL_free(kv.second->ssl);
  }

  void run() {
    prof_thread();
    crash_thread();
    tid_.store((int)syscall(SYS_gettid));
    setup();
    if (++g_ready == cfg_.threads && !cfg_.ready_file.empty()) {
      FILE* f = fopen(cfg_.ready_file.c_str(), "w");
      if (f) {
        fprintf(f, "%d\n", (int)getpid());
        if (cfg_.admin_port > 0) fprintf(f, "admin_port %d\n", cfg_.admin_port);
        fclose(f);
      }
    }
    std::vector<epoll_event> evs(512);
    double last_sweep = now_s();
    while (!g_stop.load()) {
      if (pace_s_ > 0 && small_reads_ >= pace_min_reads_) {
        const double due = tnow_ + pace_s_, t = now_s();
        if (t < due) {
          timespec ts{0, (long)((due - t) * 1e9)};
          nanosleep(&ts, nullptr);
          c_paced++;
        }
      }
      small_reads_ = 0;
      int to = (!hub_ && !aeng_ && kick_) ? 0 : deferq_.empty() ? 50 : 1;
      if (lazy_wake_ && hub_) {
        in_wait_.store(true, std::memory_order_seq_cst);
        if (rq_pending_.load(std::memory_order_seq_cst)) to = 0;
      }
      int n;
      if (jobs_live_) {
        double exp_us = 1e9;
        bool ready = false;
        for (int k = 0; k < 2 && !ready; ++k) {
          double e = 0;
          if (!job_live_[k]) continue;
          ready = aeng_->job_ready(job_[k], &e);
          exp_us = std::min(exp_us, e);
        }
        if (ready || exp_us <= spin_us_) {
          n = epoll_wait(ep_, evs.data(), (int)evs.size(), 0);
        } else {
          const double us = std::min(std::max(exp_us - spin_us_, (double)poll_us_), 1000.0 * std::max(to, 1));
          timespec ts{0, (long)(us * 1000.0)};
          n = epoll_pwait2(ep_, evs.data(), (int)evs.size(), &ts, nullptr);
          if (n < 0 && errno == ENOSYS) {
            nanosleep(&ts, nullptr);
            n = epoll_wait(ep_, evs.data(), (int)evs.size(), 0);
          }
        }
      } else {
        n = epoll_wait(ep_, evs.data(), (int)evs.size(), to);
      }
      tnow_ = now_s();
      if (stall_log_) pass_t0_.store(tnow_, std::memory_order_relaxed);
      double ph[7] = {0, 0, 0, 0, 0, 0, 0};
      rusage ru0{};
      if (stall_log_) getrusage(RUSAGE_THREAD, &ru0);
      if (lazy_wake_ && hub_) {
        in_wait_.store(false, std::memory_order_seq_cst);
        if (rq_pending_.load(std::memory_order_acquire)) on_results(false);
      }
      cnt(SC_EPOLL_WAIT);
      if (jobs_live_ && any_ready()) loop_tick();
      if (stall_log_) ph[0] = now_s();
      double ev_max = 0;
      int ev_kind = -1;
      for (int i = 0; i < n; ++i) {
        if (stall_log_) {
          const double e0 = now_s();
          dispatch(evs[i]);
          const double de = now_s() - e0;
          if (de > ev_max) {
            ev_max = de;
            ev_kind = (int)(evs[i].data.u64 >> 32);
          }
        } else {
          dispatch(evs[i]);
        }
        if (eager_post_ && aeng_ && !ops_.empty() && (evs[i].data.u64 >> 32) == 4 && aeng_->free_doors() > 0) {
          flush_ops();
          loop_tick();
        }
        if ((i & 7) == 7 && early_flush_ && rq_pending_.load(std::memory_order_acquire)) on_results(false);
        if ((i + 1) % check_every_ == 0 && jobs_live_ && any_ready()) loop_tick();
      }
      if (stall_log_) ph[1] = now_s();
      if (g_drain.load() && drain_step()) break;
      if ((hub_ || aeng_) && early_flush_) {
        flush_ops();
        if (aeng_) {
          loop_tick();
        } else if (kick_) {
          kick_ = false;
          hub_->kick();
        }
        if (!flushq_.empty()) flush_queued();
      }
      if (stall_log_) ph[2] = now_s();
      if (!pending_requests_.empty()) {
        std::vector<int>& fds = scratch_fds_;
        fds.clear();
        fds.swap(pending_requests_);
        for (int fd : fds) {
          auto it = clients_.find(fd);
          if (it != clients_.end() && !it->second->sess && !it->second->dead) process_requests(it->second.get());
          if (req_check_ && jobs_live_ && any_ready()) loop_tick();
        }
      }
      double t = now_s();
      if (stall_log_) ph[3] = t;
      if (t - last_sweep > 0.1) {
        sweep_timeouts(t);
        last_sweep = t;
        snapshot();
        if (grid_) grid_->housekeep();
        for (int k = 0; k < 2 && jobs_live_; ++k) {
          if (!job_live_[k] || t - job_t_post_[k] < 0.2) continue;
          if (grid_) grid_->revive_if_exited();
          if (t - job_t_post_[k] > 10.0) {
            fprintf(stderr, "qmx: io loop %d: a tick posted %.1f s ago never completed — exiting\n", idx_,
                    t - job_t_post_[k]);
            fflush(stderr);
            _exit(70);
          }
        }
      }
      if (stall_log_) ph[4] = now_s();
      flush_ops();
      if (aeng_) {
        loop_tick();
      } else if (!hub_) {
        if (kick_ || eng_->has_work()) {
          kick_ = false;
          tick_inline();
          flush_ops();
        }
      } else if (kick_) {
        kick_ = false;
        hub_->kick();
      }
      if (stall_log_) ph[5] = now_s();
      if (!deferq_.empty()) release_deferred(now_s());
      if (!flushq_.empty()) flush_queued();
      if (!pending_close_.empty()) reap_clients();
      flush_x();
      const double pass = now_s() - tnow_;
      if (stall_log_) pass_t0_.store(0.0, std::memory_order_relaxed);
      if (pass > 1e-3) {
        c_loop_pass_1ms++;
        if (pass > 5e-3) c_loop_pass_5ms++;
        if (pass > pass_max_.load(std::memory_order_relaxed)) pass_max_.store(pass, std::memory_order_relaxed);
        if (stall_log_ && pass > 5e-3 && stall_logs_++ < 50) {
          rusage ru1{};
          getrusage(RUSAGE_THREAD, &ru1);
          auto tv = [](const timeval& t) { return 1e3 * t.tv_sec + 1e-3 * t.tv_usec; };
          fprintf(stderr, "qmx loop %d: stalled pass: cpu %.2f ms (user %.2f), vcsw %ld, ivcsw %ld, minflt %ld, majflt %ld\n",
                  idx_, tv(ru1.ru_utime) + tv(ru1.ru_stime) - tv(ru0.ru_utime) - tv(ru0.ru_stime),
                  tv(ru1.ru_utime) - tv(ru0.ru_utime), ru1.ru_nvcsw - ru0.ru_nvcsw, ru1.ru_nivcsw - ru0.ru_nivcsw,
                  ru1.ru_minflt - ru0.ru_minflt, ru1.ru_majflt - ru0.ru_majflt);
          ph[6] = tnow_ + pass;
          double prev = tnow_, d[7];
          for (int k = 0; k < 7; ++k) {
            d[k] = ph[k] > 0 ? 1e3 * (ph[k] - prev) : 0.0;
            if (ph[k] > 0) prev = ph[k];
          }
          fprintf(stderr, "qmx loop %d: %.2f ms pass (%d events): results %.2f, events %.2f, early flush %.2f, "
                  "requests %.2f, sweep %.2f, flush+tick %.2f, output %.2f ms; engine allocs %.0f (%.0f us); "
                  "grid launches %.0f stops %.0f; slowest event kind %d (%.2f ms)\n", idx_,
                  1e3 * pass, n, d[0], d[1], d[2], d[3], d[4], d[5], d[6],
                  heng_ ? heng_->kernel_stats()["runtime_allocs"] : 0.0,
                  heng_ ? heng_->kernel_stats()["runtime_alloc_us"] : 0.0,
                  grid_ ? grid_->stats()["grid_launches"] : 0.0, grid_ ? grid_->stats()["grid_stops"] : 0.0, ev_kind,
                  1e3 * ev_max);
        }
      }
    }
    for (int w = 0; jobs_live_ && w < 200000; ++w) {
      for (int k = 0; k < 2; ++k)
        if (job_live_[k] && aeng_->job_ready(job_[k])) finish_job(k);
      if (jobs_live_) std::this_thread::sleep_for(std::chrono::microseconds(50));
    }
  }
  void release_deferred(double t) {
    size_t k = 0;
    for (size_t i = 0; i < deferq_.size(); ++i) {
      auto it = clients_.find(deferq_[i].fd);
      if (it == clients_.end()) continue;
      Client* c = it->second.get();
      if (c->serial != deferq_[i].serial) continue;
      if (c->queued || c->want_out || c->dead || c->out_off >= c->out.size()) {
        unhold(c);
        continue;
      }
      if (deferq_[i].deadline <= t || g_drain.load()) {
        if (c->held) c_hold_deadline++;
        unhold(c);
        c->queued = true;
        flushq_.push_back(c->fd);
        continue;
      }
      deferq_[k++] = deferq_[i];
    }
    deferq_.resize(k);
  }

 private:
  void setup() {
    ep_ = epoll_create1(0);
    lfd_ = socket(AF_INET, SOCK_STREAM | SOCK_NONBLOCK, 0);
    int one = 1;
    setsockopt(lfd_, SOL_SOCKET, SO_REUSEADDR, &one, sizeof(one));
    setsockopt(lfd_, SOL_SOCKET, SO_REUSEPORT, &one, sizeof(one));
    sockaddr_in a{};
    a.sin_family = AF_INET;
    a.sin_port = htons(cfg_.port);
    inet_pton(AF_INET, cfg_.host.c_str(), &a.sin_addr);
    if (bind(lfd_, (sockaddr*)&a, sizeof(a)) != 0) throw std::runtime_error("bind failed: " + std::string(strerror(errno)));
    listen(lfd_, 4096);
    add(lfd_, EPOLLIN, tag_listen());
    if (idx_ == 0 && cfg_.admin_port > 0) {
      afd_ = socket(AF_INET, SOCK_STREAM | SOCK_NONBLOCK, 0);
      setsockopt(afd_, SOL_SOCKET, SO_REUSEADDR, &one, sizeof(one));
      sockaddr_in b = a;
      b.sin_port = htons(cfg_.admin_port);
      if (bind(afd_, (sockaddr*)&b, sizeof(b)) != 0)
        throw std::runtime_error("admin port bind failed: " + std::string(strerror(errno)));
      listen(afd_, 256);
      add(afd_, EPOLLIN, tag(6, 0));
    }
    evfd_ = eventfd(0, EFD_NONBLOCK);
    add(evfd_, EPOLLIN, tag_event());
    add(xfd_, EPOLLIN, tag(5, 0));
    idle_.resize(cfg_.backends.size());
    if (!hub_) {
      if (grid_) {
        prctl(PR_SET_TIMERSLACK, 1000UL, 0, 0, 0);
        const int per = std::max(128, cfg_.max_slots / std::max(1, cfg_.threads));
        heng_ = new HipEngine(cfg_.tags, cfg_.device, cfg_.tile, per, cfg_.content_cap, 1, grid_,
                              idx_ * loop_doors_, loop_doors_);
        heng_->set_remote_hbm_direct(remote_hbm_direct(cfg_));
        eng_.reset(heng_);
        aeng_ = heng_;
        loop_slots_ = per;
      } else if (cfg_.tick_mode == "loops") {
        aeng_ = new AsyncCpuEngine(cfg_.tags);
        eng_.reset(aeng_);
      } else {
        eng_.reset(new CpuEngine(cfg_.tags));
      }
      if (cfg_.verify) ver_.reset(new Verifier(cfg_.tags));
    }
  }

  static uint64_t tag(int kind, int fd) { return ((uint64_t)kind << 32) | (uint32_t)fd; }
  static uint64_t tag_listen() { return tag(1, 0); }
  static uint64_t tag_event() { return tag(2, 0); }
  void add(int fd, uint32_t ev, uint64_t t) {
    epoll_event e{};
    e.events = ev;
    e.data.u64 = t;
    epoll_ctl(ep_, EPOLL_CTL_ADD, fd, &e);
    cnt(SC_EPOLL_CTL);
  }
  void mod(int fd, uint32_t ev, uint64_t t) {
    epoll_event e{};
    e.events = ev;
    e.data.u64 = t;
    epoll_ctl(ep_, EPOLL_CTL_MOD, fd, &e);
    cnt(SC_EPOLL_CTL);
  }

  void dispatch(const epoll_event& e) {
    int kind = (int)(e.data.u64 >> 32);
    int fd = (int)(uint32_t)e.data.u64;
    if (kind == 1) return on_accept(lfd_);
    if (kind == 6) return on_accept(afd_);
    if (kind == 2) return on_results();
    if (kind == 5) return on_xmsgs();
    if (kind == 7) return on_link(fd, e.events);
    if (kind == 3) {
      auto it = clients_.find(fd);
      if (it != clients_.end()) on_client(it->second.get(), e.events);
      return;
    }
    if (kind == 4) {
      auto it = ups_.find(fd);
      if (it != ups_.end()) on_up(it->second.get(), e.events);
      else on_parked(fd);
      return;
    }
  }

  bool any_ready() {
    for (int k = 0; k < 2; ++k)
      if (job_live_[k] && aeng_->job_ready(job_[k])) return true;
    return false;
  }
  void loop_tick() {
    bool applied = false;
    for (int k = 0; k < 2; ++k)
      if (job_live_[k] && aeng_->job_ready(job_[k])) {
        finish_job(k);
        applied = true;
      }
    if (applied) flush_ops();
    kick_ = false;
    if (aeng_->free_doors() == 0) return;
    const int k = job_live_[0] ? 1 : 0;
    const bool fin_ok = !(job_live_[k ^ 1] && !job_[k ^ 1].fin.empty());
    HostEngine::Job& j = job_[k];
    j.created = (int64_t)time(nullptr);
    j.lane = 0;
    if (!eng_->job_take(j, fin_ok)) return;
    job_t_post_[k] = now_s();
    eng_->job_prepare(j);
    eng_->job_post(j);
    job_live_[k] = true;
    ++jobs_live_;
    if (aeng_->job_ready(j)) finish_job(k);
  }
  void finish_job(int k) {
    ResultBatch rb;
    taken_.clear();
    HostEngine::Job& j = job_[k];
    eng_->job_complete(j, rb.r, rb.f);
    eng_->job_finish(j, rb.r, taken_);
    job_live_[k] = false;
    --jobs_live_;
    eng_->settle(taken_);
    h_tick.observe(now_s() - job_t_post_[k]);
    if (ver_) ver_->check(j.created, rb.r, rb.f);
    c_ticks++;
    c_tick_slots += rb.r.size();
    apply(rb);
  }
  void tick_inline() {
    ResultBatch rb;
    const double tt = now_s();
    const int64_t created = (int64_t)time(nullptr);
    eng_->tick(created, rb.r, rb.f);
    h_tick.observe(now_s() - tt);
    if (ver_) ver_->check(created, rb.r, rb.f);
    c_ticks++;
    c_tick_slots += rb.r.size();
    apply(rb);
  }
  void on_results(bool read_fd = true) {
    if (read_fd) {
      uint64_t v;
      ssize_t r = read(evfd_, &v, 8);
      cnt(SC_WAKE_READ);
      (void)r;
    }
    std::vector<ResultBatch>& q = scratch_rq_;
    q.clear();
    {
      std::lock_guard<std::mutex> g(rmu_);
      q.swap(rq_);
      rq_pending_.store(false, std::memory_order_relaxed);
    }
    const double t = now_s();
    for (auto& rb : q) {
      if (rb.t_routed > 0) {
        c_apply_ns += (uint64_t)((t - rb.t_routed) * 1e9);
        c_applies++;
      }
      apply(rb);
    }
    q.clear();
  }
  void apply(ResultBatch& rb) {
    for (auto& r : rb.r) {
      auto it = slot_owner_.find(r.slot);
      if (it == slot_owner_.end() || it->second.gen != r.gen) {
        r.hold = ViewRef();
        continue;
      }
      Session* s = it->second.s;
      int bi = it->second.bi;
      if (fault_drop_every_ > 0 && !r.empty() && ++fault_n_ % fault_drop_every_ == 0)
        r.clear_sse();
      if (!r.empty()) {
        if (s->kind == K_REMOTE) {
          post_owner(s, X_DATA, (r.flags & (RF_DONE | RF_ABORTED)) ? XF_LAST : 0, 0, r.data(), r.size());
          s->data_sent++;
        } else if (s->cl) {
          const bool last = (r.flags & (RF_DONE | RF_ABORTED)) != 0;
          const bool hold = coalesce_s_ > 0 && s->first_content &&
                            (last ? session_hold(s, bi) : more_pending(r.slot, s->bs[bi].up));
          send_content(s, r.data(), r.size(), hold);
        }
      } else if (s->cl && s->cl->held && s->kind != K_REMOTE && !more_pending(r.slot, s->bs[bi].up))
        release_held(s->cl);
      r.hold = ViewRef();
      if ((r.flags & RF_ABORTED)) c_stream_aborts++;
      if ((r.flags & (RF_DONE | RF_ABORTED)) && s->bs[bi].state == 0) {
        s->bs[bi].state = 1;
        s->bs[bi].aborted = (r.flags & RF_ABORTED) != 0;
        if (s->bs[bi].t_fed > 0) h_engine.observe(lnow() - s->bs[bi].t_fed);
        s->finished++;
      }
      if (s->stage == 0 && s->finished == (int)s->bs.size()) begin_final(s);
    }
    for (auto& f : rb.f) {
      auto it = fin_owner_.find(f.id);
      if (it == fin_owner_.end()) continue;
      Session* s = it->second.first;
      const int bi = it->second.second;
      fin_owner_.erase(it);
      if (s->fin_id == f.id) s->fin_id = -1;
      on_finalized(s, f, bi);
    }
  }
  void kick() { kick_ = true; }
  HostEngine& eng() { return hub_ ? hub_->engine() : *eng_; }
  int e_open(Session* s, int bi, int index, bool f, bool e, bool verify = true) {
    uint32_t gen = 0;
    int slot;
    if (hub_) {
      slot = hub_->open(idx_, index, f, e, &gen, verify);
    } else {
      slot = eng_->open(index, f, e, &gen);
      if (heng_ && slot >= loop_slots_) c_host_path_opens++;
      else if (heng_ && light_host_ > 0) {
        sess_ema_ = 0.95 * sess_ema_ + 0.05 * (double)sessions_.size();
        if (jobs_live_ == 0 && sess_ema_ <= (double)light_host_) heng_->host_open(slot);
      }
      if (ver_ && verify) ver_->open(slot, gen, index, f, e);
    }
    slot_owner_[slot] = SlotOwner{s, bi, gen};
    return slot;
  }
  void e_feed_move(int slot, std::string& d) {
    if (ops_t0_ == 0) ops_t0_ = now_s();
    ops_.push_back(EngineOp{EngineOp::FEED, slot, std::move(d)});
  }
  void e_finish(int slot) { ops_.push_back(EngineOp{EngineOp::FINISH, slot, std::string()}); }
  void e_release(int slot) { ops_.push_back(EngineOp{EngineOp::RELEASE, slot, std::string()}); }
  void flush_ops() {
    if (ops_.empty()) return;
    if (ops_t0_ > 0) {
      c_flush_ns += (uint64_t)((now_s() - ops_t0_) * 1e9);
      c_flushes++;
      ops_t0_ = 0;
    }
    if (hub_) {
      hub_->apply_ops(ops_);
    } else {
      if (ver_) ver_->apply_ops(ops_);
      eng_->apply_ops(ops_, true);
    }
    ops_.clear();
    kick_ = true;
  }
  int e_submit(const std::vector<int>& slots, bool strip, bool texts, const std::string& joiner, int64_t created) {
    if (hub_) return hub_->submit(idx_, slots, strip, texts, joiner, created);
    int id = eng_->submit_finalize(slots, strip, texts, joiner, created);
    if (ver_) ver_->submit(id, slots, strip, texts, joiner, created);
    return id;
  }

  bool drain_step() {
    const double t = now_s();
    if (!draining_) {
      draining_ = true;
      drain_deadline_ = t + cfg_.drain_s;
      for (int* l : {&lfd_, &afd_}) {
        if (*l < 0) continue;
        on_accept(*l);
        epoll_ctl(ep_, EPOLL_CTL_DEL, *l, nullptr);
        cnt(SC_EPOLL_CTL);
        close(*l);
        *l = -1;
      }
    }
    for (auto& kv : clients_) {
      Client* c = kv.second.get();
      const bool idle = !c->sess && c->in.empty() && c->out_off >= c->out.size();
      if (idle && (c->served > 0 || t - c->t_accept > 1.0)) mark_close(c);
    }
    if (!flushq_.empty()) flush_queued();
    if (!pending_close_.empty()) reap_clients();
    return (sessions_.empty() && clients_.empty()) || t > drain_deadline_;
  }

  void on_accept(int lfd) {
    while (true) {
      int fd = accept4(lfd, nullptr, nullptr, SOCK_NONBLOCK);
      if (fd < 0) break;
      int one = 1;
      setsockopt(fd, IPPROTO_TCP, TCP_NODELAY, &one, sizeof(one));
      auto c = std::make_unique<Client>();
      c->fd = fd;
      c->serial = ++next_serial_;
      c->t_accept = lnow();
      add(fd, EPOLLIN, tag(3, fd));
      clients_[fd] = std::move(c);
      c_clients++;
    }
  }
  void reap_clients() {
    std::vector<int> fds;
    fds.swap(pending_close_);
    for (int fd : fds) {
      auto it = clients_.find(fd);
      if (it == clients_.end()) continue;
      Client* c = it->second.get();
      if (c->dead || (c->close_after && c->out_off >= c->out.size())) close_client(c);
    }
  }
  void mark_close(Client* c) {
    c->close_after = true;
    pending_close_.push_back(c->fd);
  }
  void on_client(Client* c, uint32_t ev) {
    if (ev & EPOLLOUT) flush_client(c);
    if (c->dead) return close_client(c);
    if (ev & (EPOLLIN | EPOLLHUP | EPOLLERR)) {
      char buf[65536];
      while (true) {
        ssize_t r = recv(c->fd, buf, sizeof(buf), 0);
        cnt(SC_RECV);
        if (r > 0) {
          c->in.append(buf, r);
          if (r < (ssize_t)sizeof(buf)) break;
          continue;
        }
        if (r == 0 || (errno != EAGAIN && errno != EWOULDBLOCK)) c->dead = true;
        break;
      }
      if (!c->dead && !c->sess) process_requests(c);
      if (c->dead) return close_client(c);
    }
  }
  void close_client(Client* c) {
    if (c->sess) {
      c->sess->cl = nullptr;
      abort_session(c->sess);
    }
    epoll_ctl(ep_, EPOLL_CTL_DEL, c->fd, nullptr);
    cnt(SC_EPOLL_CTL);
    close(c->fd);
    clients_.erase(c->fd);
  }
  void write_client(Client* c, const std::string& data) {
    if (c->dead) return;
    if (c->out.size() == c->out_off) {
      c->out.clear();
      c->out_off = 0;
    }
    c->out += data;
    if (!c->queued && !c->want_out) {
      c->queued = true;
      flushq_.push_back(c->fd);
    }
  }
  void write_chunk(Client* c, const std::string& data) { write_chunk(c, data.data(), data.size()); }
  void write_chunk(Client* c, const char* data, size_t len) {
    if (c->dead || len == 0) return;
    append_chunk(c, data, len);
    if (!c->queued && !c->want_out) {
      c->queued = true;
      flushq_.push_back(c->fd);
    }
  }
  void append_chunk(Client* c, const char* data, size_t len) {
    if (c->dead || len == 0) return;
    if (c->out.size() == c->out_off) {
      c->out.clear();
      c->out_off = 0;
    }
    char h[24];
    const int n = chunk_head(h, len);
    c->out.append(h, n);
    c->out.append(data, len);
    c->out.append("\r\n", 2);
  }
  void flush_queued() {
    std::vector<int>& fds = scratch_flush_;
    fds.clear();
    fds.swap(flushq_);
    for (int fd : fds) {
      auto it = clients_.find(fd);
      if (it == clients_.end()) continue;
      Client* c = it->second.get();
      c->queued = false;
      unhold(c);
      if (c->dead || c->want_out) continue;
      while (c->out_off < c->out.size()) {
        ssize_t w = send(c->fd, c->out.data() + c->out_off, c->out.size() - c->out_off, MSG_NOSIGNAL);
        cnt(SC_CLIENT_SEND);
        if (w > 0) {
          c->out_off += w;
          continue;
        }
        if (w < 0 && (errno == EAGAIN || errno == EWOULDBLOCK)) {
          c->want_out = true;
          mod(c->fd, EPOLLIN | EPOLLOUT, tag(3, c->fd));
        } else {
          c->dead = true;
          pending_close_.push_back(c->fd);
        }
        break;
      }
      if (c->out_off >= c->out.size()) {
        c->out.clear();
        c->out_off = 0;
        if (c->close_after) pending_close_.push_back(c->fd);
      }
    }
  }
  void flush_client(Client* c) {
    while (c->out_off < c->out.size()) {
      ssize_t w = send(c->fd, c->out.data() + c->out_off, c->out.size() - c->out_off, MSG_NOSIGNAL);
      cnt(SC_CLIENT_SEND);
      if (w > 0) {
        c->out_off += w;
        continue;
      }
      if (w < 0 && (errno == EAGAIN || errno == EWOULDBLOCK)) return;
      c->dead = true;
      return;
    }
    c->out.clear();
    c->out_off = 0;
    c->want_out = false;
    mod(c->fd, EPOLLIN, tag(3, c->fd));
    if (c->close_after) pending_close_.push_back(c->fd);
  }

  void process_requests(Client* c) {
    while (!c->sess && !c->dead) {
      size_t he = c->in.find("\r\n\r\n");
      if (he == std::string::npos) {
        if (c->in.size() > (1 << 20)) c->dead = true;
        return;
      }
      const char* head = c->in.data();
      const size_t le0 = c->in.find("\r\n");
      const size_t le = le0 == std::string::npos || le0 > he ? he : le0;
      const char* sp1p = (const char*)memchr(head, ' ', le);
      const char* sp2p = (const char*)memrchr(head, ' ', le);
      if (!sp1p || sp2p == sp1p) {
        c->dead = true;
        return;
      }
      const size_t sp1 = (size_t)(sp1p - head), sp2 = (size_t)(sp2p - head);
      thread_local std::string method, target;
      method.assign(head, sp1);
      target.assign(head + sp1 + 1, sp2 - sp1 - 1);
      const bool http10 = le - sp2 - 1 == 8 && memcmp(head + sp2 + 1, "HTTP/1.0", 8) == 0;
      std::vector<std::pair<std::string, std::string>> hdrs;
      hdrs.reserve(12);
      const size_t pos = le + 2;
      long clen = 0;
      bool chunked = false;
      bool keepalive = !http10;
      for_each_header(head + std::min(pos, he), he - std::min(pos, he), [&](std::string&& k, std::string&& v) {
        if (k == "content-length") clen = atol(v.c_str());
        if (k == "transfer-encoding" && icontains(v, "chunked")) chunked = true;
        if (k == "connection") {
          if (ieq(v, "close")) keepalive = false;
          if (ieq(v, "keep-alive")) keepalive = true;
        }
        hdrs.emplace_back(std::move(k), std::move(v));
      });
      std::string body;
      size_t used;
      if (chunked) {
        size_t i = he + 4;
        bool complete = false;
        while (true) {
          size_t l2 = c->in.find("\r\n", i);
          if (l2 == std::string::npos) break;
          long sz = strtol(c->in.c_str() + i, nullptr, 16);
          if (sz == 0) {
            size_t t = c->in.find("\r\n\r\n", l2);
            if (t == std::string::npos) {
              if (c->in.size() >= l2 + 4 && c->in.compare(l2, 4, "\r\n\r\n") == 0) t = l2;
              else break;
            }
            i = t + 4;
            complete = true;
            break;
          }
          if (c->in.size() < l2 + 2 + sz + 2) break;
          body.append(c->in, l2 + 2, sz);
          i = l2 + 2 + sz + 2;
        }
        if (!complete) return;
        used = i;
      } else {
        if (c->in.size() < he + 4 + (size_t)clen) return;
        body = c->in.substr(he + 4, clen);
        used = he + 4 + clen;
      }
      c->in.erase(0, used);
      c->keepalive = keepalive && !draining_;
      handle_request(c, method, target, hdrs, body);
      if (!c->sess && !c->keepalive) {
        mark_close(c);
        return;
      }
    }
  }

  void respond(Client* c, int status, const std::string& ctype, const std::string& body,
               const std::vector<std::pair<std::string, std::string>>* extra = nullptr) {
    write_client(c, http_response(status, ctype, body, extra));
  }

  void handle_request(Client* c, const std::string& method, std::string target,
                      std::vector<std::pair<std::string, std::string>>& hdrs, std::string& body) {
    size_t q = target.find('?');
    if (q != std::string::npos) target.resize(q);
    if (method == "GET" && target == "/health") return respond(c, 200, "application/json", "{\"status\":\"healthy\"}");
    if (method == "GET" && target == "/metrics") return respond(c, 200, "text/plain; version=0.0.4", metrics_text());
    if (method == "GET" && target == "/openapi.json" && !cfg_.openapi_json.empty())
      return respond(c, 200, "application/json", cfg_.openapi_json);
    if (method == "GET" && target == "/docs" && !cfg_.docs_html.empty())
      return respond(c, 200, "text/html; charset=utf-8", cfg_.docs_html);
    if (method == "GET" && target == "/docs/oauth2-redirect" && !cfg_.oauth2_redirect_html.empty())
      return respond(c, 200, "text/html; charset=utf-8", cfg_.oauth2_redirect_html);
    if (method == "GET" && target == "/redoc" && !cfg_.redoc_html.empty())
      return respond(c, 200, "text/html; charset=utf-8", cfg_.redoc_html);
    if (target != "/chat/completions" && target != "/v1/chat/completions")
      return respond(c, 404, "application/json", "{\"detail\":\"Not Found\"}");
    if (method != "POST") return respond(c, 405, "application/json", "{\"detail\":\"Method Not Allowed\"}");
    c_requests++;
    c->served++;
    auto s = std::make_unique<Session>();
    s->t0 = lnow();
    std::string perr;
    if (!json_parse(body.data(), body.size(), s->body, &perr)) {
      c_errors++;
      return respond(c, 500, "application/json", err_json("Error processing request: " + perr, "proxy_error"));
    }
    if (s->body.t != JVal::OBJ) {
      c_errors++;
      const char* tn = s->body.t == JVal::ARR ? "list" : s->body.t == JVal::STR ? "str" : "int";
      return respond(c, 500, "application/json",
                     err_json(std::string("Error processing request: '") + tn + "' object has no attribute 'get'",
                              "proxy_error"));
    }
    const JVal* sv = s->body.get("stream");
    bool streaming = sv && sv->truthy();
    bool has_auth = false, has_ctype = false;
    s->fwd.reserve(hdrs.size() + 2);
    for (auto& h : hdrs) {
      if (h.first == "host") continue;
      if (h.first == "authorization") {
        has_auth = true;
        s->auth = h.second;
        continue;
      }
      if (h.first == "content-type") has_ctype = true;
      if (h.first == "content-length" || h.first == "transfer-encoding" || h.first == "connection" ||
          h.first == "keep-alive" || h.first == "te" || h.first == "upgrade" || h.first == "accept-encoding")
        continue;
      s->fwd.push_back(std::move(h));
    }
    if (!has_auth) {
      std::string env_key = cfg_.env_api_key;
      if (cfg_.api_key_from_env) {
        const char* e = env_get("OPENAI_API_KEY");
        env_key = e ? e : "";
      }
      if (env_key.empty()) {
        c_errors++;
        return respond(c, 401, "application/json",
                       err_json("Authorization header is required and OPENAI_API_KEY environment variable is not set",
                                "auth_error"));
      }
      s->auth = "Bearer " + env_key;
    }
    s->fwd.emplace_back("Authorization", s->auth);
    if (!has_ctype) s->fwd.emplace_back("Content-Type", "application/json");
    if (!valid_init_) {
      valid_init_ = true;
      for (int i = 0; i < (int)cfg_.backends.size(); ++i)
        if (cfg_.backends[i].valid) valid_.push_back(i);
    }
    const std::vector<int>& valid = valid_;
    if (valid.empty())
      return respond(c, 500, "application/json", err_json("No valid backends configured", "configuration_error"));
    if (!s->body.get("model")) {
      bool any = false;
      for (int i : valid) any = any || !cfg_.backends[i].model.empty();
      if (!any)
        return respond(c, 400, "application/json",
                       err_json("Model must be specified when config.yaml model is blank", "invalid_request_error"));
    }
    bool parallel = cfg_.has_iterations_and_strategy && valid.size() > 1;
    s->raw = std::move(body);
    s->cl = c;
    Session* sp = s.get();
    sessions_[sp] = std::move(s);
    c->sess = sp;
    if (streaming && parallel) start_parallel(sp, valid);
    else if (streaming) start_single(sp, valid[0]);
    else start_nonstream(sp, valid, parallel);
  }

  bool upstream_body(Session* s, int b, std::string& out, int* st, std::string* msg, const char** etype) {
    const BackendCfg& be = cfg_.backends[b];
    if (!be.has_model_key) {
      *st = 500;
      *msg = "'model'";
      *etype = "proxy_error";
      return false;
    }
    if (!be.model.empty()) {
      if (!s->msplit) {
        s->msplit = true;
        const auto& items = s->body.o;
        size_t k = 0;
        while (k < items.size() && items[k].first != "model") ++k;
        std::string& pre = s->mpre;
        pre.reserve(s->raw.size() + 32);
        pre.push_back('{');
        for (size_t i = 0; i < k; ++i) {
          if (i) pre += ", ";
          json_dump_str(items[i].first, pre);
          pre += ": ";
          json_dump(items[i].second, pre);
        }
        if (k > 0) pre += ", ";
        pre += "\"model\": ";
        for (size_t i = k + 1; i < items.size(); ++i) {
          s->mpost += ", ";
          json_dump_str(items[i].first, s->mpost);
          s->mpost += ": ";
          json_dump(items[i].second, s->mpost);
        }
        s->mpost.push_back('}');
      }
      out.reserve(s->mpre.size() + be.model.size() + s->mpost.size() + 8);
      out = s->mpre;
      json_dump_str(be.model, out);
      out += s->mpost;
      return true;
    }
    if (!s->body.get("model")) {
      *st = 400;
      *msg = "No model specified in config.yaml or request";
      *etype = "invalid_request_error";
      return false;
    }
    out = s->raw;
    return true;
  }
  std::string build_req(const BackendCfg& be, const std::vector<std::pair<std::string, std::string>>& hdrs,
                        const std::string& body) {
    size_t n = be.path.size() + be.host.size() + body.size() + 96;
    for (auto& h : hdrs) n += h.first.size() + h.second.size() + 4;
    std::string r;
    r.reserve(n);
    r.append("POST ").append(be.path).append("/chat/completions HTTP/1.1\r\nhost: ").append(be.host);
    char num[24];
    if (be.port != (be.https ? 443 : 80)) {
      r += ':';
      r.append(num, (size_t)dec_str(num, (size_t)be.port));
    }
    r.append("\r\n");
    for (auto& h : hdrs) r.append(h.first).append(": ").append(h.second).append("\r\n");
    r.append("content-length: ").append(num, (size_t)dec_str(num, body.size())).append("\r\n\r\n");
    r.append(body);
    return r;
  }
  Up* open_up(Session* s, int bi, int backend, UpMode mode, std::string req, double timeout) {
    const BackendCfg& be = cfg_.backends[backend];
    auto u = std::make_unique<Up>();
    u->backend = backend;
    u->sess = s;
    u->bi = bi;
    u->mode = mode;
    u->rp.keep_headers = mode != UP_ENGINE;
    u->req = std::move(req);
    u->timeout = timeout;
    u->last_io = lnow();
    u->t_open = u->last_io;
    u->deadline = cfg_.total_timeout > 0 ? u->last_io + cfg_.total_timeout : 0;
    if (!be.resolved || (be.https && !tls_)) return nullptr;
    int fd = -1;
    auto& pool = idle_[backend];
    while (!pool.empty() && fd < 0) {
      fd = pool.back();
      pool.pop_back();
      if (!parked_.count(fd)) {
        fd = -1;
        continue;
      }
      u->reused = true;
      auto it = idle_ssl_.find(fd);
      if (it != idle_ssl_.end()) {
        u->ssl = it->second;
        idle_ssl_.erase(it);
      }
    }
    if (fd < 0) {
      fd = socket(AF_INET, SOCK_STREAM | SOCK_NONBLOCK, 0);
      int one = 1;
      setsockopt(fd, IPPROTO_TCP, TCP_NODELAY, &one, sizeof(one));
      int r = connect(fd, (const sockaddr*)&be.addr, sizeof(be.addr));
      if (r != 0 && errno != EINPROGRESS) {
        close(fd);
        return nullptr;
      }
      u->connecting = r != 0;
      c_up_conns++;
      u->fd = fd;
      add(fd, EPOLLIN | EPOLLOUT, tag(4, fd));
      u->out_armed = true;
      if (be.https) {
        u->ssl = SSL_new(tls_);
        SSL_set_fd(u->ssl, fd);
        SSL_set_tlsext_host_name(u->ssl, be.host.c_str());
        X509_VERIFY_PARAM* vp = SSL_get0_param(u->ssl);
        in_addr ip4;
        if (inet_pton(AF_INET, be.host.c_str(), &ip4) == 1) X509_VERIFY_PARAM_set1_ip_asc(vp, be.host.c_str());
        else SSL_set1_host(u->ssl, be.host.c_str());
        u->tls_hs = true;
      }
    } else {
      u->fd = fd;
      parked_.erase(fd);
    }
    Up* p = u.get();
    ups_[fd] = std::move(u);
    if (!p->connecting) {
      if (p->tls_hs) tls_step(p);
      else write_up(p);
    }
    return p;
  }
  void tls_step(Up* u) {
    ERR_clear_error();
    int r = SSL_connect(u->ssl);
    if (r == 1) {
      u->tls_hs = false;
      return write_up(u);
    }
    int e = SSL_get_error(u->ssl, r);
    if (e == SSL_ERROR_WANT_READ) return mod(u->fd, EPOLLIN, tag(4, u->fd));
    if (e == SSL_ERROR_WANT_WRITE) return mod(u->fd, EPOLLIN | EPOLLOUT, tag(4, u->fd));
    c_fail_connect++;
    up_error(u, "All connection attempts failed");
  }
  void write_up(Up* u) {
    while (u->req_off < u->req.size()) {
      if (u->ssl) {
        ERR_clear_error();
        int w = SSL_write(u->ssl, u->req.data() + u->req_off, (int)(u->req.size() - u->req_off));
        if (w > 0) {
          u->req_off += w;
          u->last_io = lnow();
          continue;
        }
        int e = SSL_get_error(u->ssl, w);
        if (e == SSL_ERROR_WANT_WRITE) {
          u->out_armed = true;
          return mod(u->fd, EPOLLIN | EPOLLOUT, tag(4, u->fd));
        }
        if (e == SSL_ERROR_WANT_READ) {
          u->out_armed = false;
          return mod(u->fd, EPOLLIN, tag(4, u->fd));
        }
        if (u->reused && !u->got_bytes) return retry_fresh(u);
        c_fail_connect++;
        return up_error(u, "All connection attempts failed");
      }
      ssize_t w = send(u->fd, u->req.data() + u->req_off, u->req.size() - u->req_off, MSG_NOSIGNAL);
      cnt(SC_UP_SEND);
      if (w > 0) {
        u->req_off += w;
        u->last_io = lnow();
        continue;
      }
      if (w < 0 && (errno == EAGAIN || errno == EWOULDBLOCK)) {
        if (!u->out_armed) {
          u->out_armed = true;
          mod(u->fd, EPOLLIN | EPOLLOUT, tag(4, u->fd));
        }
        return;
      }
      c_fail_connect++;
      return up_error(u, "All connection attempts failed");
    }
    if (u->out_armed) {
      u->out_armed = false;
      mod(u->fd, EPOLLIN, tag(4, u->fd));
    }
  }
  ssize_t up_read(Up* u, char* buf, size_t n) {
    if (!u->ssl) {
      ssize_t r = recv(u->fd, buf, n, 0);
      cnt(SC_RECV);
      if (r > 0) return r;
      if (r < 0 && (errno == EAGAIN || errno == EWOULDBLOCK)) return 0;
      return -1;
    }
    ERR_clear_error();
    int r = SSL_read(u->ssl, buf, (int)n);
    if (r > 0) return r;
    int e = SSL_get_error(u->ssl, r);
    if (e == SSL_ERROR_WANT_READ || e == SSL_ERROR_WANT_WRITE) return 0;
    return -1;
  }
  void on_up(Up* u, uint32_t ev) {
    if (u->connecting && (ev & (EPOLLOUT | EPOLLERR | EPOLLHUP))) {
      int err = 0;
      socklen_t len = sizeof(err);
      getsockopt(u->fd, SOL_SOCKET, SO_ERROR, &err, &len);
      if (err != 0) {
        c_fail_connect++;
        return up_error(u, "All connection attempts failed");
      }
      u->connecting = false;
    }
    const int fd = u->fd;
    if (u->tls_hs) {
      if (!u->connecting) tls_step(u);
      return;
    }
    if ((ev & (EPOLLOUT | (u->ssl ? EPOLLIN : 0))) && u->req_off < u->req.size()) {
      write_up(u);
      if (ups_.find(fd) == ups_.end()) return;
      if (u->req_off < u->req.size()) return;
    }
    if (ev & (EPOLLIN | EPOLLHUP | EPOLLERR)) {
      char buf[65536];
      bool eof = false;
      std::string body;
      while (true) {
        ssize_t r = up_read(u, buf, sizeof(buf));
        if (r > 0) {
          if (!u->got_bytes) h_upstream_ttfb.observe(lnow() - u->t_open);
          u->got_bytes = true;
          u->last_io = lnow();
          const bool in_body = u->rp.phase != 0;
          if (u->rp.feed(buf, r, body) < 0) {
            c_fail_protocol++;
            return up_error(u, "invalid HTTP response");
          }
          if (in_body && r < 2048 && !u->rp.done()) ++small_reads_;
          if (!u->ssl && (r < (ssize_t)sizeof(buf) || u->rp.done())) break;
          continue;
        }
        if (r < 0) eof = true;
        break;
      }
      if (!u->headers_seen && u->rp.phase > 0) {
        u->headers_seen = true;
        on_up_headers(u);
        if (ups_.find(fd) == ups_.end()) return;
      }
      if (!body.empty()) on_up_body(u, body);
      if (u->rp.done()) return up_complete(u, true);
      if (eof) {
        if (u->rp.phase == 6) return up_complete(u, false);
        if (!u->got_bytes && u->reused) return retry_fresh(u);
        c_fail_disconnect++;
        return up_error(u, "Server disconnected without sending a response.");
      }
    }
  }
  void retry_fresh(Up* u) {
    Session* s = u->sess;
    int bi = u->bi, backend = u->backend;
    UpMode mode = u->mode;
    std::string req = u->req;
    double to = u->timeout;
    drop_up(u, false);
    Up* nu = open_up(s, bi, backend, mode, req, to);
    if (!nu) return fail_backend(s, bi, 500, "All connection attempts failed", "proxy_error");
    if (bi >= 0) s->bs[bi].up = nu;
    else s->agg = nu;
  }
  void drop_up(Up* u, bool reuse) {
    int fd = u->fd;
    if (reuse && !u->rp.close && !u->tls_hs && !u->out_armed) {
      idle_[u->backend].push_back(fd);
      parked_[fd] = u->backend;
      if (u->ssl) idle_ssl_[fd] = u->ssl;
    } else {
      epoll_ctl(ep_, EPOLL_CTL_DEL, fd, nullptr);
      cnt(SC_EPOLL_CTL);
      if (u->ssl) SSL_free(u->ssl);
      close(fd);
    }
    u->ssl = nullptr;
    ups_.erase(fd);
  }
  void on_parked(int fd) {
    auto it = parked_.find(fd);
    if (it == parked_.end()) return;
    auto& pool = idle_[it->second];
    pool.erase(std::remove(pool.begin(), pool.end(), fd), pool.end());
    parked_.erase(it);
    auto s = idle_ssl_.find(fd);
    if (s != idle_ssl_.end()) {
      SSL_free(s->second);
      idle_ssl_.erase(s);
    }
    epoll_ctl(ep_, EPOLL_CTL_DEL, fd, nullptr);
    cnt(SC_EPOLL_CTL);
    close(fd);
  }
  void up_error(Up* u, const std::string& msg) {
    Session* s = u->sess;
    int bi = u->bi;
    c_up_fail++;
    drop_up(u, false);
    if (bi >= 0) s->bs[bi].up = nullptr;
    else s->agg = nullptr;
    fail_backend(s, bi, 500, msg, "proxy_error");
  }
  void sweep_timeouts(double t) {
    std::vector<int> expired;
    for (auto& kv : ups_) {
      Up* u = kv.second.get();
      if (t - u->last_io > u->timeout || (u->deadline > 0 && t > u->deadline)) expired.push_back(kv.first);
    }
    for (int fd : expired) {
      auto it = ups_.find(fd);
      if (it != ups_.end()) {
        c_fail_timeout++;
        up_error(it->second.get(), "");
      }
    }
  }

  void on_up_headers(Up* u) {
    Session* s = u->sess;
    if (u->mode == UP_PASS && u->rp.status == 200) {
      std::string h = "HTTP/1.1 200 OK\r\n";
      bool has_ct = false;
      for (auto& kv : u->rp.headers) {
        if (kv.first == "content-length" || kv.first == "transfer-encoding" || kv.first == "content-encoding" ||
            kv.first == "connection" || kv.first == "keep-alive")
          continue;
        if (kv.first == "content-type") has_ct = true;
        h += kv.first + ": " + kv.second + "\r\n";
      }
      if (!has_ct) h += "content-type: text/event-stream; charset=utf-8\r\n";
      h += "transfer-encoding: chunked\r\n\r\n";
      s->pass_started = true;
      if (s->cl) {
        write_client(s->cl, h);
        send_chunk(s, chunk_event_json("chatcmpl-role", (int64_t)time(nullptr), s->role_model_json,
                                       "{\"role\": \"assistant\"}", "null"));
      }
    }
  }
  void on_up_body(Up* u, std::string& body) {
    Session* s = u->sess;
    if (u->rp.status == 200 && u->mode == UP_ENGINE) {
      if (s->bs[u->bi].t_fed == 0) s->bs[u->bi].t_fed = lnow();
      e_feed_move(s->bs[u->bi].slot, body);
      kick();
      return;
    }
    if (u->rp.status == 200 && u->mode == UP_PASS) return pass_body(s, body);
    u->body += body;
  }
  void up_complete(Up* u, bool reusable) {
    Session* s = u->sess;
    int bi = u->bi;
    int status = u->rp.status;
    UpMode mode = u->mode;
    std::string body = std::move(u->body);
    auto rh = std::move(u->rp.headers);
    drop_up(u, reusable);
    if (bi >= 0) s->bs[bi].up = nullptr;
    else s->agg = nullptr;
    if (mode == UP_ENGINE && status == 200) {
      e_finish(s->bs[bi].slot);
      kick();
      return;
    }
    if (mode == UP_PASS && status == 200) return pass_end(s);
// ... 116 lines not shown
  bool more_pending(int slot, const Up* up) {
    if (ops_pending(slot)) return true;
    if (hub_) return up_readable(up) || eng().pending(slot);
    return eng().pending(slot) || up_readable(up);
  }
  bool session_hold(const Session* s, int bi) const {
    if (s->stage == 0 && s->kind == K_PAR && final_follows_) return true;
    if (!session_hold_) return false;
    for (size_t k = 0; k < s->bs.size(); ++k)
      if ((int)k != bi && s->bs[k].state == 0) return true;
    return false;
  }
  void unhold(Client* c) {
    if (!c->held) return;
    c->held = false;
    c_hold_ns += (uint64_t)(1e9 * std::max(0.0, lnow() - c->held_t0));
    c_holds++;
  }
  void release_held(Client* c) {
    if (!c->held || c->queued || c->dead) return;
    unhold(c);
    if (c->out_off >= c->out.size() || c->want_out) return;
    c->queued = true;
    flushq_.push_back(c->fd);
  }
  bool up_readable(const Up* u) const {
    if (!u || u->fd < 0 || u->ssl) return false;
    int n = 0;
    return ioctl(u->fd, FIONREAD, &n) == 0 && n > 0;
  }
  bool ops_pending(int slot) const {
    for (const EngineOp& o : ops_)
      if (o.slot == slot && o.kind == EngineOp::FEED) return true;
    return false;
  }
  void start_parallel(Session* s, const std::vector<int>& valid) {
    c_stream++;
    s->kind = K_PAR;
    s->filter = cfg_.hide_intermediate;
    s->emit = !cfg_.suppress;
    if (const JVal* sup = s->body.get("suppress_individual_responses")) s->emit = !sup->truthy();
    const bool defer = role_defer_s_ > 0 && s->cl && !s->cl->queued && !s->cl->want_out;
    const int64_t now_sec = (int64_t)time(nullptr);
    if (now_sec != role_sec_) {
      role_sec_ = now_sec;
      role_head_ = kSseHdr;
      role_head_ += chunk(chunk_event_json("chatcmpl-parallel", now_sec, "\"parallel-proxy\"",
                                           "{\"role\": \"assistant\"}", "null"));
    }
    write_client(s->cl, role_head_);
    if (defer && s->cl->queued && !flushq_.empty() && flushq_.back() == s->cl->fd) {
      flushq_.pop_back();
      s->cl->queued = false;
      deferq_.push_back(Deferred{s->cl->fd, s->cl->serial, now_s() + role_defer_s_});
    }
    s->bs.resize(valid.size());
    const bool spread = xch_ && xch_->healthy() && (xch_->world() > 1 || self_spread_);
    if (spread) {
      s->skey = ((uint64_t)xch_->rank() << 56) | ((uint64_t)idx_ << 48) | next_skey_++;
      rsess_[s->skey] = s;
    }
    for (size_t i = 0; i < valid.size(); ++i) {
      s->bs[i].backend = valid[i];
      const int target = spread ? (xch_->rank() + (int)i) % xch_->world() : -1;
      if (spread && (target != xch_->rank() || (self_spread_ && (i & 1))) && xch_->peer_up(target)) {
        s->bs[i].remote = target;
        s->bs[i].via_link = link_up(target);
        s->remote_n++;
        s->bs[i].slot = e_open(s, (int)i, (int)i, false, false, false);
        size_t cap = 0;
        void* dev = eng().content_device_ptr(s->bs[i].slot, &cap);
        xch_->expect_bulk(s->skey, (int)i, dev, cap);
        continue;
      }
      s->bs[i].slot = e_open(s, (int)i, (int)i, s->filter, s->emit);
    }
    for (size_t i = 0; i < valid.size(); ++i) {
      std::string body, msg;
      int st = 0;
      const char* et = nullptr;
      if (!upstream_body(s, valid[i], body, &st, &msg, &et)) {
        fail_backend(s, (int)i, st, msg, et);
        continue;
      }
      if (s->bs[i].remote >= 0) {
        XMsg m;
        m.type = X_OPEN;
        m.flags = (uint8_t)((s->filter ? 1 : 0) | (s->emit ? 2 : 0));
        m.dst_rank = s->bs[i].remote;
        m.src_rank = xch_->rank();
        m.dst_loop = m.src_loop = (uint16_t)idx_;
        m.bi = (int)i;
        m.skey = s->skey;
        m.a = valid[i];
        m.b = (int)(cfg_.timeout * 1000.0);
        m.payload = build_req(cfg_.backends[valid[i]], s->fwd, body);
        xq(m, s->bs[i].via_link);
        s->bs[i].t_sp_open = now_s();
        continue;
      }
      Up* u = open_up(s, (int)i, valid[i], UP_ENGINE, build_req(cfg_.backends[valid[i]], s->fwd, body), cfg_.timeout);
      if (!u) fail_backend(s, (int)i, 500, "All connection attempts failed", "proxy_error");
      else s->bs[i].up = u;
    }
  }
  std::vector<int> good_slots(Session* s) {
    std::vector<int> g;
    for (auto& b : s->bs)
      if (b.state == 1 && !b.aborted) g.push_back(b.slot);
    return g;
  }
  void begin_final(Session* s) {
    s->stage = 1;
    if (s->kind == K_REMOTE) {
      const BState& b = s->bs[0];
      const size_t len = b.aborted || cfg_.skip_final ? 0 : eng().content_size(b.slot);
      if (s->emit && !b.aborted && s->data_sent == 0 && eng().content_size(b.slot) > 0) {
        c_sp_nodata++;
        if (g_sp_logs.fetch_add(1) < 20)
          fprintf(stderr, "qmx spread (rank %d loop %d): worker stream slot %d has %zu content bytes but sent no delta "
                  "(skey %llx bi %d filter %d)\n", cfg_.rank, idx_, b.slot, eng().content_size(b.slot),
                  (unsigned long long)s->owner_skey, s->shadow_bi, (int)s->filter);
      }
      if (len == 0) {
        post_owner(s, X_FINAL, b.aborted ? XF_ABORTED : 0, 0, std::string(), s->data_sent);
        return end_session(s);
      }
      const bool eager = (long long)len <= (long long)cfg_.xchg_eager_bytes;
      size_t cap0 = 0;
      const bool host_bytes = eager || !(xch_->transport() == "rccl" && xch_->rccl_active());
      if (host_bytes && !s->fetched && eng().content_device_ptr(b.slot, &cap0) != nullptr) {
        s->fetching = true;
        s->fin_id = e_submit({b.slot}, false, true, std::string(), (int64_t)time(nullptr));
        fin_owner_[s->fin_id] = {s, -1};
        kick();
        return;
      }
      if (eager) {
        const std::string t = s->fetched ? std::move(s->fetched_text) : eng().text(b.slot);
        post_owner(s, X_BULK, XF_TEXT, (int)t.size(), t.data(), t.size(), s->data_sent);
        c_sp_eager++;
        return end_session(s);
      }
      XMsg h;
      h.flags = XF_TEXT;
      h.dst_rank = s->owner_rank;
      h.src_rank = xch_->rank();
      h.dst_loop = (uint16_t)s->owner_loop;
      h.src_loop = (uint16_t)idx_;
      h.bi = s->shadow_bi;
      h.skey = s->owner_skey;
      h.b = s->data_sent;
      size_t cap = 0;
      const void* dev = eng().content_device_ptr(b.slot, &cap);
      HostEngine* e = &eng();
      const int slot = b.slot;
// ... 160 lines not shown
  void post_owner(Session* s, uint8_t type, uint8_t flags, int a, const char* payload, size_t n, int b = 0) {
    if (!xch_) return;
    XMsg m;
    m.type = type;
    m.flags = flags;
    m.dst_rank = s->owner_rank;
    m.src_rank = xch_->rank();
    m.dst_loop = (uint16_t)s->owner_loop;
    m.src_loop = (uint16_t)idx_;
    m.bi = s->shadow_bi;
    m.skey = s->owner_skey;
    m.a = a;
    m.b = b;
    xq(m, payload, n, s->via_link);
  }
  bool delta_check(Session* s, int bi, int sent, const char* how) {
    const BState& b = s->bs[bi];
    if (b.rx_data == sent) return true;
    c_sp_delta_mismatch++;
    if (g_sp_logs.fetch_add(1) < 20)
      fprintf(stderr, "qmx spread (rank %d loop %d): remote stream %d of session %llx (rank %d) ended by %s after %d "
              "of its %d deltas\n", cfg_.rank, idx_, bi, (unsigned long long)s->skey, b.remote, how, b.rx_data, sent);
    return false;
  }
  void on_xmsgs() {
    uint64_t v;
    ssize_t r = read(xfd_, &v, 8);
    cnt(SC_WAKE_READ);
    (void)r;
    std::vector<XMsg> in;
    {
      std::lock_guard<std::mutex> g(xmu_);
      in.swap(xin_);
    }
    handle_x(in, false);
  }
  void handle_x(std::vector<XMsg>& in, bool link) {
    for (auto& m : in) {
      if (m.type == X_UP) continue;
      if (m.type == X_RELEASE) {
        if (m.a >= 0) e_release(m.a);
        continue;
      }
      if (m.type == X_LINK) {
        on_link_msg(m);
        continue;
      }
      if (m.type == X_DOWN) {
        const bool link_only = m.b == 1;
        std::vector<Session*> owners, shadows;
        for (auto& kv : rsess_) owners.push_back(kv.second);
        for (auto& kv : shadow_) shadows.push_back(kv.second);
        for (Session* s : shadows)
          if (sessions_.count(s) && (m.a < 0 || s->owner_rank == m.a) && !s->bulk_pending &&
              (!link_only || s->via_link))
            end_session(s);
        for (Session* s : owners) {
          for (int i = 0; i < (int)s->bs.size() && sessions_.count(s); ++i)
            if (s->bs[i].remote >= 0 && (m.a < 0 || s->bs[i].remote == m.a) && s->bs[i].state == 0 &&
                (!link_only || s->bs[i].via_link)) {
              c_sp_down++;
              fail_backend(s, i, 500, "rank exchange failed", "proxy_error");
            }
        }
        continue;
      }
      if (m.type == X_OPEN) {
        auto sp = std::make_unique<Session>();
        Session* s = sp.get();
        sessions_[s] = std::move(sp);
        s->kind = K_REMOTE;
        s->owner_rank = m.src_rank;
        s->owner_loop = m.src_loop;
        s->owner_skey = m.skey;
        s->shadow_bi = m.bi;
        s->via_link = link;
        s->filter = m.flags & 1;
        s->emit = (m.flags & 2) != 0;
        s->bs.resize(1);
        s->bs[0].backend = m.a;
        s->bs[0].slot = e_open(s, 0, m.bi, s->filter, s->emit);
        shadow_[{m.skey, m.bi}] = s;
        c_remote_streams++;
        Up* u = (m.a >= 0 && m.a < (int)cfg_.backends.size())
                    ? open_up(s, 0, m.a, UP_ENGINE, std::move(m.payload), m.b / 1000.0) : nullptr;
        if (!u) fail_backend(s, 0, 500, "All connection attempts failed", "proxy_error");
        else s->bs[0].up = u;
        continue;
      }
      if (m.type == X_CANCEL || m.type == X_SENT) {
        auto it = shadow_.find({m.skey, m.bi});
        if (it == shadow_.end()) continue;
        Session* s = it->second;
        if (m.type == X_SENT) s->bulk_pending = false;
        if (!s->bulk_pending) end_session(s);
        continue;
      }
      auto it = rsess_.find(m.skey);
      if (it == rsess_.end()) continue;
      Session* s = it->second;
      if (m.bi < 0 || m.bi >= (int)s->bs.size()) continue;
      BState& b = s->bs[m.bi];
      if (m.type == X_DATA) {
        const double t = now_s();
        if (b.rx_data == 0 && b.t_sp_open > 0) h_sp_first.observe(t - b.t_sp_open);
        b.t_sp_last = t;
        b.rx_data++;
        if (s->cl) {
          const bool hold = coalesce_s_ > 0 && s->first_content && (m.flags & XF_LAST) && session_hold(s, m.bi);
          send_content(s, m.payload.data(), m.payload.size(), hold);
        }
        if (b.bulk_waiting && b.rx_data >= b.bulk_msg.b) {
          b.bulk_waiting = false;
          XMsg bm = std::move(b.bulk_msg);
          remote_final(s, m.bi, bm);
        }
        continue;
      }
      if (m.type == X_BULK) {
        if (b.state != 0) continue;
        if (b.rx_data < m.b) {
          b.bulk_waiting = true;
          b.bulk_msg = std::move(m);
          continue;
        }
        remote_final(s, m.bi, m);
        continue;
      }
      if (m.type == X_FINAL) {
        if (b.state != 0) continue;
        delta_check(s, m.bi, m.b, (m.flags & XF_FAILED) ? "failure" : (m.flags & XF_ABORTED) ? "abort" : "empty final");
        if (m.flags & XF_FAILED) {
          c_sp_failed++;
          if (g_sp_logs.fetch_add(1) < 20)
            fprintf(stderr, "qmx spread (rank %d loop %d): remote stream %d of session %llx failed on rank %d: %d %s\n",
                    cfg_.rank, idx_, m.bi, (unsigned long long)s->skey, m.src_rank, m.a, m.payload.substr(0, 200).c_str());
          fail_backend(s, m.bi, m.a, m.payload, "proxy_error");
          continue;
        }
        if (m.flags & XF_ABORTED) c_sp_aborted++;
// ... 85 lines not shown
      if (cfg_.include_source_names) {
        std::string lab;
        const std::string name = cfg_.documented && i < s->text_names.size() ? s->text_names[i]
                                                                              : "LLM" + std::to_string(i + 1);
        if (!py_format(cfg_.source_label_format, "backend_name", name, lab))
          return aggregate_result(s, JVal::str(joined(s->texts, exc_joiner)));
        parts.push_back(lab + s->texts[i]);
      } else {
        parts.push_back(s->texts[i]);
      }
    }
    std::string prompt;
    if (cfg_.include_original_query) {
      std::string uq;
      const JVal* msgs = s->body.get("messages");
      if (msgs && msgs->truthy() && msgs->t == JVal::ARR) {
        for (auto& m : msgs->a) {
          const JVal* r = m.get("role");
          if (r && r->t == JVal::STR && r->s == "user") {
            const JVal* ct = m.get("content");
            uq = ct ? py_str(*ct) : "";
            break;
          }
        }
      }
      if (!py_format(cfg_.query_format, "query", uq, prompt))
        return aggregate_result(s, JVal::str(joined(s->texts, exc_joiner)));
    }
    std::string inter = joined(parts, cfg_.intermediate_separator);
    std::string tmpl = cfg_.prompt_template;
    std::string out;
    for (size_t i = 0; i < tmpl.size();) {
      if (tmpl.compare(i, 11, "{responses}") == 0) {
        out += inter;
        i += 11;
      } else {
        out.push_back(tmpl[i++]);
      }
    }
    prompt += out;
    const BackendCfg& be = cfg_.backends[ab];
    JVal req;
    req.t = JVal::OBJ;
    req.set("model", JVal::str(be.model));
    JVal msgs;
    msgs.t = JVal::ARR;
    JVal m;
    m.t = JVal::OBJ;
    m.set("role", JVal::str("user"));
    m.set("content", JVal::str(prompt));
    msgs.a.push_back(m);
    req.set("messages", msgs);
    req.set("stream", JVal::boolean(false));
    std::vector<std::pair<std::string, std::string>> h = {{"Authorization", s->auth},
                                                          {"Content-Type", "application/json"}};
    if (!be.valid || !be.has_model_key) return on_aggregator_done(s, 500, std::string());
    Up* u = open_up(s, -1, ab, UP_BUFFER, build_req(be, h, json_dumps(req)), 60.0);
    if (!u) return on_aggregator_done(s, 500, std::string());
    s->agg = u;
  }
  void on_aggregator_done(Session* s, int status, const std::string& body) {
    JVal j;
    if (status == 200 && json_parse(body.data(), body.size(), j, nullptr)) {
      const JVal* ch = j.get("choices");
      if (ch && ch->t == JVal::ARR && !ch->a.empty()) {
        const JVal* msg = ch->a[0].get("message");
        const JVal* ct = msg ? msg->get("content") : nullptr;
        if (ct && cfg_.documented && cfg_.hide_aggregator_think && ct->t == JVal::STR)
          return aggregate_result(s, JVal::str(strip_final(ts_, (const uint8_t*)ct->s.data(), ct->s.size())));
        if (ct) return aggregate_result(s, *ct);
      }
    }
    aggregate_result(s, JVal::str(joined(s->texts, cfg_.intermediate_separator)));
  }
  void aggregate_result(Session* s, const JVal& v) {
    if (s->kind == K_PAR) return emit_final_value(s, v);
    finish_nonstream_combined(s, v);
  }

  void start_single(Session* s, int backend) {
    c_stream++;
    s->kind = K_SINGLE;
    s->bs.resize(1);
    s->bs[0].backend = backend;
    const JVal* m = s->body.get("model");
    if (m && m->truthy()) s->role_model_json = json_dumps(*m);
    else s->role_model_json = cfg_.backends[backend].has_model_key ? json_dumps(JVal::str(cfg_.backends[backend].model))
                                                                   : "\"unknown\"";
    std::string body, msg;
    int st = 0;
    const char* et = nullptr;
    if (!upstream_body(s, backend, body, &st, &msg, &et)) return fail_backend(s, 0, st, msg, et);
    Up* u = open_up(s, 0, backend, UP_PASS, build_req(cfg_.backends[backend], s->fwd, body), cfg_.timeout);
    if (!u) return fail_backend(s, 0, 500, "All connection attempts failed", "proxy_error");
    s->bs[0].up = u;
  }
  static bool bare_role(const std::string& ev) {
    std::string t = ev;
    if (t.compare(0, 6, "data: ") == 0) t = t.substr(6);
    JVal j;
    if (!json_parse(t.data(), t.size(), j, nullptr) || j.t != JVal::OBJ) return false;
    const JVal* ch = j.get("choices");
    if (!ch || ch->t != JVal::ARR || ch->a.empty() || ch->a[0].t != JVal::OBJ) return false;
    const JVal* d = ch->a[0].get("delta");
    if (!d || d->t != JVal::OBJ) return false;
    const JVal* r = d->get("role");
    const JVal* c = d->get("content");
    bool content_empty = !c || (c->t == JVal::STR && c->s.empty());
    return r && r->truthy() && content_empty;
  }
  void pass_forward(Session* s, const std::string& data) {
    bool all_ws = true;
    for (char ch : data)
      if (!(ch == ' ' || ch == '\n' || ch == '\r' || ch == '\t')) all_ws = false;
    if (all_ws) return;
    std::string w = s->done_tail + data;
    if (w.find("data: [DONE]") != std::string::npos) s->saw_done = true;
    s->done_tail = w.size() > 16 ? w.substr(w.size() - 16) : w;
    send_content(s, data);
  }
  void pass_body(Session* s, const std::string& body) {
    if (!s->first_decided) {
      s->first_buf += body;
      size_t j = s->first_buf.find("\n\n");
      if (j == std::string::npos) return;
      s->first_decided = true;
      std::string first = s->first_buf.substr(0, j + 2), rest = s->first_buf.substr(j + 2);
      s->first_buf.clear();
      if (!bare_role(first)) rest = first + rest;
      if (!rest.empty()) pass_forward(s, rest);
      return;
    }
    pass_forward(s, body);
  }
  void pass_end(Session* s) {
    if (!s->first_decided && !s->first_buf.empty() && !bare_role(s->first_buf)) pass_forward(s, s->first_buf);
    if (!s->saw_done) send_chunk(s, kDone);
    if (s->cl) write_client(s->cl, "0\r\n\r\n");
    s->bs[0].state = 1;
    end_session(s);
  }

  void start_nonstream(Session* s, const std::vector<int>& valid, bool parallel) {
    c_nonstream++;
    s->kind = K_NONSTREAM;
    s->stage = parallel ? 10 : 11;
    s->bs.resize(valid.size());
    for (size_t i = 0; i < valid.size(); ++i) s->bs[i].backend = valid[i];
    for (size_t i = 0; i < valid.size(); ++i) {
      std::string body, msg;
      int st = 0;
      const char* et = nullptr;
      if (!upstream_body(s, valid[i], body, &st, &msg, &et)) {
        fail_backend(s, (int)i, st, msg, et);
        if (sessions_.find(s) == sessions_.end()) return;
        continue;
      }
      Up* u = open_up(s, (int)i, valid[i], UP_BUFFER, build_req(cfg_.backends[valid[i]], s->fwd, body), cfg_.timeout);
      if (!u) {
        fail_backend(s, (int)i, 500, "All connection attempts failed", "proxy_error");
        if (sessions_.find(s) == sessions_.end()) return;
      } else {
        s->bs[i].up = u;
      }
    }
  }
  void finish_nonstream(Session* s) {
    std::vector<BState*> ok;
    for (auto& b : s->bs)
      if (b.status == 200) ok.push_back(&b);
    if (ok.empty()) {
      if (s->cl)
        respond(s->cl, 500, "application/json",
                err_json("All backends failed. First error: " + error_message(s->bs[0]), "proxy_error"));
      return end_session(s);
    }
    if (s->stage == 11) {
      BState* f = ok[0];
      const std::string* ct = nullptr;
      for (auto& h : f->rheaders)
        if (h.first == "content-type") ct = &h.second;
      std::vector<std::pair<std::string, std::string>> extra;
      for (auto& h : f->rheaders)
        if (h.first != "content-length" && h.first != "content-type" && h.first != "transfer-encoding" &&
            h.first != "content-encoding" && h.first != "connection" && h.first != "keep-alive")
          extra.push_back(h);
      std::string body = f->is_json ? json_dumps(f->js) : f->text;
      if (s->cl) respond(s->cl, 200, ct ? *ct : "application/json", body, &extra);
      return end_session(s);
    }
    const bool agg = !cfg_.aggregator_name.empty();
    const bool strip = cfg_.hide_final || (cfg_.documented && agg && cfg_.strip_intermediate);
    std::vector<std::string> processed;
    std::string err;
    for (BState* b : ok) {
      const JVal* content = nullptr;
      if (b->is_json) {
        const JVal* ch = b->js.get("choices");
        if (ch && ch->t == JVal::ARR && !ch->a.empty()) {
          const JVal* m = ch->a[0].get("message");
          if (m) content = m->get("content");
          else err = "'message'";
        } else {
          err = ch ? "list index out of range" : "'choices'";
        }
      } else {
        err = "string indices must be integers";
      }
      if (!content) {
        if (err.empty()) err = "'content'";
        break;
      }
      if (content->t != JVal::STR) {
        err = strip ? "expected string or bytes-like object" : "sequence item 0: expected str instance";
        break;
      }
// ... 44 lines not shown
        if (!u) { err = "'usage'"; break; }
        if (!v) { err = std::string("'") + k + "'"; break; }
        if (v->t == JVal::INT) { isum += atoll(v->s.c_str()); fsum += atof(v->s.c_str()); }
        else if (v->t == JVal::FLOAT) { isf = true; fsum += v->d; }
        else { err = "unsupported operand type(s) for +"; break; }
      }
      if (!err.empty()) break;
      if (isf) {
        JVal f;
        f.t = JVal::FLOAT;
        f.d = fsum;
        usage.set(k, f);
      } else {
        usage.set(k, JVal::integer(isum));
      }
    }
    const JVal& first = ok[0]->js;
    for (const char* k : {"id", "created", "model"})
      if (err.empty() && !first.get(k)) err = std::string("'") + k + "'";
    if (!err.empty()) {
      if (s->cl) respond(s->cl, 500, "application/json", err_json("Error combining responses: " + err, "proxy_error"));
      return end_session(s);
    }
    JVal out;
    out.t = JVal::OBJ;
    out.set("id", *first.get("id"));
    out.set("object", JVal::str("chat.completion"));
    out.set("created", *first.get("created"));
    out.set("model", *first.get("model"));
    const JVal* fp = first.get("system_fingerprint");
    out.set("system_fingerprint", fp ? *fp : JVal::str(""));
    JVal choice;
    choice.t = JVal::OBJ;
    choice.set("index", JVal::integer(0));
    JVal msg;
    msg.t = JVal::OBJ;
    msg.set("role", JVal::str("assistant"));
    msg.set("content", combined);
    choice.set("message", msg);
    choice.set("logprobs", JVal());
    choice.set("finish_reason", JVal::str("stop"));
    JVal choices;
    choices.t = JVal::ARR;
    choices.a.push_back(choice);
    out.set("choices", choices);
    out.set("usage", usage);
    if (s->cl) respond(s->cl, 200, "application/json", json_dumps(out));
    end_session(s);
  }

  void end_session(Session* s) {
    if (s->stage == 3) return;
    s->stage = 3;
    if (s->kind != K_REMOTE && s->t0 > 0) h_latency.observe(now_s() - s->t0);
    if (s->kind == K_REMOTE) shadow_.erase({s->owner_skey, s->shadow_bi});
    if (s->skey) {
      rsess_.erase(s->skey);
      for (int i = 0; i < (int)s->bs.size(); ++i) {
        if (s->bs[i].remote < 0 || s->bs[i].state != 0 || !xch_) continue;
        XMsg m;
        m.type = X_CANCEL;
        m.dst_rank = s->bs[i].remote;
        m.src_rank = xch_->rank();
        m.dst_loop = m.src_loop = (uint16_t)idx_;
        m.bi = i;
        m.skey = s->skey;
        xq(m, s->bs[i].via_link);
      }
    }
    for (int i = 0; i < (int)s->bs.size(); ++i) {
      BState& b = s->bs[i];
      if (b.up) {
        drop_up(b.up, false);
        b.up = nullptr;
      }
      const bool reusable = !(b.remote >= 0 && xch_ && s->skey) || xch_->forget_bulk(s->skey, i, b.slot, idx_);
      if (b.slot >= 0) {
        slot_owner_.erase(b.slot);
        if (reusable) e_release(b.slot);
        else c_sp_release_deferred++;
        b.slot = -1;
      }
    }
    if (s->agg) {
      drop_up(s->agg, false);
      s->agg = nullptr;
    }
    if (s->fin_id >= 0) fin_owner_.erase(s->fin_id);
    Client* c = s->cl;
    sessions_.erase(s);
    if (c) {
      c->sess = nullptr;
      if (!c->keepalive || c->dead) mark_close(c);
      else if (!c->in.empty()) pending_requests_.push_back(c->fd);
    }
  }
  void abort_session(Session* s) { end_session(s); }

  std::string metrics_text() {
    std::string m;
    auto put = [&](const char* k, double v) { m += std::string(k) + " " + std::to_string(v) + "\n"; };
    put("qmx_requests_total", (double)c_requests.load());
    put("qmx_stream_requests_total", (double)c_stream.load());
    put("qmx_nonstream_requests_total", (double)c_nonstream.load());
    put("qmx_errors_total", (double)c_errors.load());
    put("qmx_upstream_failures_total", (double)c_up_fail.load());
    put("qmx_upstream_connections_total", (double)c_up_conns.load());
    put("qmx_client_connections_total", (double)c_clients.load());
    put("qmx_ticks_total", (double)c_ticks.load());
    put("qmx_output_coalesced_total", (double)c_coalesced.load());
    put("qmx_output_hold_seconds_sum", (double)c_hold_ns.load() * 1e-9);
    put("qmx_output_hold_seconds_count", (double)c_holds.load());
    put("qmx_output_hold_deadline_total", (double)c_hold_deadline.load());
    put("qmx_exchange_link_messages_total", (double)c_link_msgs.load());
    put("qmx_tick_slots_total", (double)c_tick_slots.load());
    put("qmx_tick_route_seconds_total", (double)c_route_ns.load() * 1e-9);
    put("qmx_flush_wait_seconds_total", (double)c_flush_ns.load() * 1e-9);
    put("qmx_flushes_total", (double)c_flushes.load());
    put("qmx_apply_wait_seconds_total", (double)c_apply_ns.load() * 1e-9);
    put("qmx_applies_total", (double)c_applies.load());
    put("qmx_remote_streams_total", (double)c_remote_streams.load());
    for (auto& kv : {std::make_pair("failed", &c_sp_failed), std::make_pair("aborted", &c_sp_aborted),
                     std::make_pair("empty", &c_sp_empty), std::make_pair("text", &c_sp_text),
                     std::make_pair("peer_down", &c_sp_down)})
      m += std::string("qmx_spread_remote_ends_total{how=\"") + kv.first + "\"} " + std::to_string(kv.second->load()) + "\n";
    put("qmx_spread_delta_mismatch_total", (double)c_sp_delta_mismatch.load());
    put("qmx_spread_worker_nodata_total", (double)c_sp_nodata.load());
    put("qmx_spread_eager_finals_total", (double)c_sp_eager.load());
    put("qmx_spread_release_deferred_total", (double)c_sp_release_deferred.load());
    put("qmx_spread_texts_fetched_total", (double)c_sp_fetched.load());
    put("qmx_loop_passes_over_1ms_total", (double)c_loop_pass_1ms.load());
    put("qmx_loop_passes_over_5ms_total", (double)c_loop_pass_5ms.load());
    put("qmx_loop_paced_total", (double)c_paced.load());
    {
      double mx = 0;
      for (Loop* l : *loops_) mx = std::max(mx, l->pass_max_.load(std::memory_order_relaxed));
      put("qmx_loop_pass_max_seconds", mx);
    }
    m += "qmx_upstream_failures_by_class_total{class=\"connect\"} " + std::to_string(c_fail_connect.load()) + "\n";
    m += "qmx_upstream_failures_by_class_total{class=\"timeout\"} " + std::to_string(c_fail_timeout.load()) + "\n";
    m += "qmx_upstream_failures_by_class_total{class=\"http_status\"} " + std::to_string(c_fail_status.load()) + "\n";
    m += "qmx_upstream_failures_by_class_total{class=\"disconnect\"} " + std::to_string(c_fail_disconnect.load()) + "\n";
    m += "qmx_upstream_failures_by_class_total{class=\"protocol\"} " + std::to_string(c_fail_protocol.load()) + "\n";
// ... 41 lines not shown
      uint64_t v = 0;
      for (Loop* l : *loops_) v += l->sc_[i].load(std::memory_order_relaxed);
      m += std::string("qmx_syscalls_total{op=\"") + sc_names[i] + "\"} " + std::to_string(v) + "\n";
    }
    return m;
  }

  const ServerCfg& cfg_;
  int idx_;
  int ep_ = -1, lfd_ = -1, afd_ = -1, evfd_ = -1;
  HostEngine::Job job_[2];
  std::unique_ptr<HostEngine> eng_;
  std::unique_ptr<Verifier> ver_;
  GpuHub* hub_ = nullptr;
  HipGrid* grid_ = nullptr;
  HipEngine* heng_ = nullptr;
  HostEngine* aeng_ = nullptr;
  int loop_slots_ = 0;
  bool job_live_[2] = {false, false};
  int jobs_live_ = 0;
  double job_t_post_[2] = {0, 0};
  const int loop_doors_ = [] {
    const char* e = env_get("QMX_LOOP_INFLIGHT");
    return e ? std::min(std::max(atoi(e), 1), 2) : 2;
  }();
  std::vector<int> taken_;
  const int poll_us_ = [] {
    const char* e = env_get("QMX_LOOP_POLL_US");
    return e ? std::max(1, atoi(e)) : 3;
  }();
  const double spin_us_ = [] {
    const char* e = env_get("QMX_LOOP_SPIN_US");
    return e ? atof(e) : 4.0;
  }();
  const int check_every_ = [] {
    const char* e = env_get("QMX_LOOP_CHECK_EVERY");
    return e ? std::max(1, atoi(e)) : 1;
  }();
  double sess_ema_ = 0;
  const int light_host_ = [this] {
    if (cfg_.light_host >= 0) return cfg_.light_host;
    const char* e = env_get("QMX_LIGHT_HOST");
    return e ? std::max(0, atoi(e)) : 0;
  }();
  const bool req_check_ = [] {
    const char* e = env_get("QMX_LOOP_REQ_CHECK");
    return !e || atoi(e) != 0;
  }();
  TagSet ts_ = make_tagset(cfg_.tags);
  bool kick_ = false;
  std::mutex rmu_;
  std::vector<ResultBatch> rq_;
  std::atomic<bool> rq_pending_{false};
  std::unordered_map<int, std::unique_ptr<Client>> clients_;
  std::unordered_map<int, std::unique_ptr<Up>> ups_;
  std::unordered_map<Session*, std::unique_ptr<Session>> sessions_;
  struct SlotOwner {
    Session* s;
    int bi;
    uint32_t gen;
  };
  std::unordered_map<int, SlotOwner> slot_owner_;
  std::unordered_map<int, std::pair<Session*, int>> fin_owner_;
  Exchange* xch_ = nullptr;
  bool draining_ = false;
  double drain_deadline_ = 0;
  const std::vector<Loop*>* loops_ = nullptr;
  double last_snap_ = 0;
  int xfd_ = -1;
  std::vector<int> valid_;
  std::vector<int> scratch_fds_, scratch_flush_;
  std::vector<ResultBatch> scratch_rq_;
  bool valid_init_ = false;
  std::mutex xmu_;
  std::vector<XMsg> xin_;
  std::vector<std::string> xout_;
  bool xpending_ = false;
  std::vector<XLink> xl_;
  bool xlpending_ = false;
  uint64_t next_skey_ = 1;
  std::unordered_map<uint64_t, Session*> rsess_;
  std::map<std::pair<uint64_t, int>, Session*> shadow_;
  std::vector<std::vector<int>> idle_;
  std::unordered_map<int, SSL*> idle_ssl_;
  std::unordered_map<int, int> parked_;
  SSL_CTX* tls_ = nullptr;
  std::vector<int> pending_close_, pending_requests_;
  std::vector<int> flushq_;
  struct Deferred {
    int fd;
    uint64_t serial;
    double deadline;
  };
  std::vector<Deferred> deferq_;
  uint64_t next_serial_ = 0;
  const double role_defer_s_ = [] {
    const char* e = env_get("QMX_ROLE_DEFER_US");
    return (e ? atof(e) : 1000.0) * 1e-6;
  }();
  const double coalesce_s_ = [] {
    const char* e = env_get("QMX_COALESCE_US");
    return (e ? atof(e) : 500.0) * 1e-6;
  }();
  const bool session_hold_ = env_flag("QMX_SESSION_HOLD", true);
  const bool final_follows_ = env_flag("QMX_FINAL_HOLD", true) && !cfg_.skip_final;
  std::vector<EngineOp> ops_;
  const bool early_flush_ = env_flag("QMX_EARLY_FLUSH", true);
  const bool self_spread_ = env_flag("QMX_SPREAD_SELF", false);
  const bool stall_log_ = env_flag("QMX_LOOP_STALL_LOG", false);
  const bool eager_post_ = env_flag("QMX_EAGER_POST", false);
  const double pace_s_ = [this] {
    const char* e = env_get("QMX_READ_PACE_US");
    return std::max(0.0, e ? atof(e) : (double)cfg_.read_pace_us) * 1e-6;
  }();
  const int pace_min_reads_ = [] {
    const char* e = env_get("QMX_READ_PACE_MIN");
    return e ? std::max(1, atoi(e)) : 2;
  }();
  int small_reads_ = 0;
  int stall_logs_ = 0;
  const bool lazy_wake_ = env_flag("QMX_LAZY_WAKE", false);
  std::atomic<bool> in_wait_{false};
  double ops_t0_ = 0;
  double tnow_ = now_s();
  double lnow() const { return tnow_; }
  int64_t role_sec_ = -1;
  std::string role_head_;
  const long fault_drop_every_ = [] {
    const char* e = env_get("QMX_FAULT_DROP_DELTA");
    return e ? atol(e) : 0L;
  }();
  long fault_n_ = 0;
};

void on_signal(int sig) {
  if (sig == SIGTERM) g_drain.store(true);
  else g_stop.store(true);
}

}

static void presize_fd_table() {
  rlimit rl{};
  if (getrlimit(RLIMIT_NOFILE, &rl) != 0) return;
  if (rl.rlim_cur < rl.rlim_max && rl.rlim_cur < ((rlim_t)1 << 17)) {
    rlimit up = rl;
    up.rlim_cur = std::min<rlim_t>(rl.rlim_max, (rlim_t)1 << 17);
    if (setrlimit(RLIMIT_NOFILE, &up) == 0) rl = up;
  }
  const long want = (long)std::min<rlim_t>(rl.rlim_cur, (rlim_t)1 << 17);
  if (want <= 1024) return;
  if (fcntl((int)want - 1, F_GETFD) != -1 || errno != EBADF) return;
  const int fd = open("/dev/null", O_RDONLY | O_CLOEXEC);
  if (fd < 0) return;
  const int hi = dup3(fd, (int)want - 1, O_CLOEXEC);
  if (hi >= 0) close(hi);
  close(fd);
}

int run_server(const ServerCfg& cfg0) {
  env_refresh();
  ServerCfg cfg = cfg0;
  crash_handler_install();
  prof_start();
  bool any_https = false;
  for (auto& b : cfg.backends) {
    if (!b.valid || b.host.empty()) continue;
    any_https = any_https || b.https;
    addrinfo hints{}, *res = nullptr;
    hints.ai_family = AF_INET;
    hints.ai_socktype = SOCK_STREAM;
    if (getaddrinfo(b.host.c_str(), std::to_string(b.port).c_str(), &hints, &res) == 0 && res) {
      std::memcpy(&b.addr, res->ai_addr, sizeof(sockaddr_in));
      b.resolved = true;
      freeaddrinfo(res);
    }
  }
  SSL_CTX* tls = nullptr;
  if (any_https) {
    tls = SSL_CTX_new(TLS_client_method());
    SSL_CTX_set_min_proto_version(tls, TLS1_2_VERSION);
    SSL_CTX_set_verify(tls, cfg.tls_verify ? SSL_VERIFY_PEER : SSL_VERIFY_NONE, nullptr);
    if (!cfg.ca_file.empty()) SSL_CTX_load_verify_locations(tls, cfg.ca_file.c_str(), nullptr);
    else SSL_CTX_set_default_verify_paths(tls);
    SSL_CTX_set_mode(tls, SSL_MODE_ENABLE_PARTIAL_WRITE | SSL_MODE_ACCEPT_MOVING_WRITE_BUFFER);
  }
  signal(SIGPIPE, SIG_IGN);
  presize_fd_table();
  if (cfg.install_signals) {
    struct sigaction sa {};
    sa.sa_handler = on_signal;
    sigaction(SIGTERM, &sa, nullptr);
    sigaction(SIGINT, &sa, nullptr);
  }
  g_stop.store(false);
  g_drain.store(false);
  g_ready.store(0);
  std::vector<std::unique_ptr<Loop>> loops;
  std::vector<std::thread> ts;
  for (int i = 0; i < std::max(1, cfg.threads); ++i) loops.emplace_back(new Loop(cfg, i));
  std::vector<Loop*> loop_ptrs;
  for (auto& l : loops) loop_ptrs.push_back(l.get());
  std::unique_ptr<GpuHub> hub;
  std::unique_ptr<HipGrid> grid;
  const bool hip = cfg.engine == "hip";
  const bool spread = cfg.world > 1 && cfg.placement == "spread";
  (void)spread;
  const bool loop_ticks = hip && cfg.tick_mode != "lanes" && cfg.shared_engine != 1;
  const bool shared = !loop_ticks && (cfg.shared_engine < 0 ? hip : cfg.shared_engine > 0);
  if (shared) hub.reset(new GpuHub(cfg, (int)loops.size()));
  if (loop_ticks) {
    const char* w = env_get("QMX_GRID_WPD");
    const char* im = env_get("QMX_PERSISTENT_IDLE_MS");
    const char* fl = env_get("QMX_LOOP_INFLIGHT");
    const int per_loop = fl ? std::min(std::max(atoi(fl), 1), 2) : 2;
    try {
      const char* oc = env_get("QMX_GRID_OCC");
      const int wpd0 = oc && atoi(oc) == 2 ? 16 : 8;
      grid.reset(new HipGrid(cfg.device, (int)loops.size() * per_loop, w ? std::max(1, atoi(w)) : wpd0,
// ... 122 lines not shown
```

quorum_amd/csrc/qmx_server.h:

```cpp
#pragma once
#include <netinet/in.h>

#include <string>
#include <unordered_map>
#include <vector>

namespace qmx {

struct BackendCfg {
  std::string name, url, model;
  bool has_model_key = true;
  bool valid = false;
  std::string host, path;
  int port = 80;
  bool https = false;
  sockaddr_in addr{};
  bool resolved = false;
};

struct ServerCfg {
  std::string host = "127.0.0.1";
  int port = 8000;
  int threads = 2;
  std::string engine = "cpu";
  int shared_engine = -1;
  int tick_lanes = 2;
  std::string tick_mode = "auto";
  int read_pace_us = 50;
  int light_host = -1;
  int device = 0;
  int tile = 16384, max_slots = 4096, content_cap = 1 << 20;
  std::vector<BackendCfg> backends;
  bool has_iterations_and_strategy = false;
  double timeout = 60.0;
  double total_timeout = 0.0;
  std::string separator = "\n";
  bool hide_intermediate = true, hide_final = false, skip_final = false, suppress = false;
  std::vector<std::string> tags;
  std::string aggregator_name;
  std::string prompt_template, intermediate_separator, query_format, source_label_format;
  bool include_original_query = true, include_source_names = false;
  bool documented = false, strip_intermediate = false, hide_aggregator_think = false, sources_all = true;
  std::vector<std::string> sources;
  std::string env_api_key;
  bool api_key_from_env = false;
  std::string openapi_json, docs_html, redoc_html, oauth2_redirect_html;
  bool install_signals = true;
  int rank = 0, world = 1;
  std::string placement = "local";
  std::string xchg = "tcp";
  std::string xchg_addr = "127.0.0.1";
  int xchg_port = 0;
  int xchg_bulk_port = 0;
  std::string xchg_id_file;
  int xchg_round_us = 200;
  int xchg_eager_bytes = 4096;
  int xchg_links = -1;
  double xchg_timeout = 30.0;
  double drain_s = 10.0;
  std::string ready_file;
  int admin_port = 0;
  bool verify = false;
  std::string ca_file;
  bool tls_verify = true;
};

int run_server(const ServerCfg& cfg);
std::unordered_map<std::string, double> server_counters();
void stop_server();

// ... 2 lines not shown
```

Baseline: 404,000.

## Cut host overhead in proxy loop with pooled sessions, vector fd maps, header views

Replaces the fd-keyed and pointer-keyed hash maps for clients, upstreams, sessions, slot owners, idle SSL and parked connections with fd-indexed vectors, and recycles Session and Up objects through free lists. HTTP header parsing now lowercases keys into a stack buffer and passes string_view pairs. Each backend gets a precomputed request head, and requests are built into a scratch buffer. The engine batches mono_s() calls per op batch and batches result callbacks in the HIP wait loop, with an early exit when results are already ready. Together these aim to remove allocation and hashing costs on the per-request path. In exchange the object-reset code is longer and riskier, since any field missed when recycling can leak state into the next session.

```diff
diff --git a/quorum_amd/csrc/qmx_engine.cpp b/quorum_amd/csrc/qmx_engine.cpp
--- a/quorum_amd/csrc/qmx_engine.cpp
+++ b/quorum_amd/csrc/qmx_engine.cpp
@@ -347,12 +347,14 @@
 
 void HostEngine::feed(int slot, const std::string& data) {
   std::lock_guard<std::mutex> g(mu_);
-  feed_locked(slot, data);
+  double now = 0;
+  feed_locked(slot, data, now);
 }
 
 void HostEngine::finish(int slot) {
   std::lock_guard<std::mutex> g(mu_);
-  finish_locked(slot);
+  double now = 0;
+  finish_locked(slot, now);
 }
 
 void HostEngine::release(int slot) {
@@ -362,48 +364,52 @@
 
 void HostEngine::apply_ops(std::vector<EngineOp>& ops, bool move_data) {
   std::lock_guard<std::mutex> g(mu_);
+  double now = 0;
   for (auto& op : ops) {
     if (op.kind == EngineOp::FEED) {
-      if (move_data) feed_locked_move(op.slot, op.data);
-      else feed_locked(op.slot, op.data);
-    }
-    else if (op.kind == EngineOp::FINISH) finish_locked(op.slot);
+      if (move_data) feed_locked_move(op.slot, op.data, now);
+      else feed_locked(op.slot, op.data, now);
+    }
+    else if (op.kind == EngineOp::FINISH) finish_locked(op.slot, now);
     else release_locked(op.slot);
   }
 }
 
-void HostEngine::feed_locked(int slot, const std::string& data) {
+void HostEngine::feed_locked(int slot, const std::string& data, double& now) {
   if (slot < 0 || slot >= (int)meta_.size() || !meta_[slot].live) return;
   Meta& m = meta_[slot];
   m.incoming += data;
   bytes_in_ += data.size();
   if (!m.dirty) {
     m.dirty = true;
-    m.t_dirty = mono_s();
+    if (now == 0) now = mono_s();
+    m.t_dirty = now;
     dirty_.push_back(slot);
   }
 }
 
-void HostEngine::feed_locked_move(int slot, std::string& data) {
+void HostEngine::feed_locked_move(int slot, std::string& data, double& now) {
   if (slot < 0 || slot >= (int)meta_.size() || !meta_[slot].live) return;
-  if (!meta_[slot].incoming.empty()) return feed_locked(slot, data);
+  if (!meta_[slot].incoming.empty()) return feed_locked(slot, data, now);
   bytes_in_ += data.size();
   meta_[slot].incoming.swap(data);
   Meta& m = meta_[slot];
   if (!m.dirty) {
     m.dirty = true;
-    m.t_dirty = mono_s();
+    if (now == 0) now = mono_s();
+    m.t_dirty = now;
     dirty_.push_back(slot);
   }
 }
 
-void HostEngine::finish_locked(int slot) {
+void HostEngine::finish_locked(int slot, double& now) {
   if (slot < 0 || slot >= (int)meta_.size() || !meta_[slot].live) return;
   Meta& m = meta_[slot];
   m.eof = true;
   if (!m.dirty) {
     m.dirty = true;
-    m.t_dirty = mono_s();
+    if (now == 0) now = mono_s();
+    m.t_dirty = now;
     dirty_.push_back(slot);
   }
 }
@@ -476,6 +482,7 @@
     j.work.push_back(std::move(w));
   }
   dirty_.swap(keep);
+  j.t_take = now;
   if (allow_fin) j.fin.swap(fin_);
   if (!j.work.empty() || !j.fin.empty()) ++ticks_;
   return !j.work.empty() || !j.fin.empty();
@@ -600,9 +607,9 @@
   }
 }
 
-bool AsyncCpuEngine::job_ready(Job& j, double* expect_us) {
+bool AsyncCpuEngine::job_ready(Job& j, double* expect_us, double ) {
   if (expect_us) *expect_us = 5.0;
-  auto d = std::static_pointer_cast<Done>(j.impl);
+  const Done* d = static_cast<const Done*>(j.impl.get());
   return !d || d->ready.load(std::memory_order_acquire);
 }
 
diff --git a/quorum_amd/csrc/qmx_engine.h b/quorum_amd/csrc/qmx_engine.h
--- a/quorum_amd/csrc/qmx_engine.h
+++ b/quorum_amd/csrc/qmx_engine.h
@@ -158,6 +158,7 @@
     int64_t created = 0;
     int lane = 0;
     bool live = false;
+    double t_take = 0;
     std::shared_ptr<void> impl;
   };
   virtual bool pipelined() const { return false; }
@@ -169,7 +170,7 @@
   virtual void job_complete(Job&, std::vector<SlotResult>&, std::vector<FinalizeRes>&) {}
   void job_finish(Job& j, std::vector<SlotResult>& results, std::vector<int>& taken);
   virtual bool async_jobs() const { return false; }
-  virtual bool job_ready(Job&, double* expect_us = nullptr) {
+  virtual bool job_ready(Job&, double* expect_us = nullptr, double  = 0) {
     if (expect_us) *expect_us = 0;
     return true;
   }
@@ -190,9 +191,9 @@
                         std::vector<SlotResult>& results, std::vector<FinalizeRes>& fres, int lane) = 0;
   virtual void on_free(int ) {}
 
-  void feed_locked(int slot, const std::string& data);
-  void feed_locked_move(int slot, std::string& data);
-  void finish_locked(int slot);
+  void feed_locked(int slot, const std::string& data, double& now);
+  void feed_locked_move(int slot, std::string& data, double& now);
+  void finish_locked(int slot, double& now);
   void release_locked(int slot);
 
   struct Meta {
@@ -239,7 +240,7 @@
   ~AsyncCpuEngine() override;
   bool async_jobs() const override { return true; }
   void job_post(Job& j) override;
-  bool job_ready(Job& j, double* expect_us = nullptr) override;
+  bool job_ready(Job& j, double* expect_us = nullptr, double now_s = 0) override;
   void job_complete(Job& j, std::vector<SlotResult>& results, std::vector<FinalizeRes>& fres) override;
   int free_doors() const override { return 2 - inflight_.load(std::memory_order_acquire); }
 
diff --git a/quorum_amd/csrc/qmx_hip.h b/quorum_amd/csrc/qmx_hip.h
--- a/quorum_amd/csrc/qmx_hip.h
+++ b/quorum_amd/csrc/qmx_hip.h
@@ -230,7 +230,7 @@
   HipEngine(const std::vector<std::string>& tags, int device, int tile_bytes, int max_slots, int content_cap,
             int lanes = 1, HipGrid* grid = nullptr, int door = -1, int ndoors = 1);
   ~HipEngine() override;
-  bool job_ready(Job& j, double* expect_us = nullptr) override;
+  bool job_ready(Job& j, double* expect_us = nullptr, double now_s = 0) override;
   bool async_jobs() const override { return grid_ != nullptr; }
   int free_doors() const override;
   std::string text(int slot) override;
@@ -269,7 +269,7 @@
   void collect_finalize(TickLane& L, const std::vector<const FinalizeReq*>& gpu, std::vector<FinalizeRes>& out);
   void wait_stream(TickLane& L);
   void wait_results(TickLane& L, int n, int m, uint32_t seq, const WorkResult* res,
-                    std::chrono::steady_clock::time_point t0, const std::function<void(int)>& on_item);
+                    std::chrono::steady_clock::time_point t0, const std::function<void(int, int)>& on_items);
   void collect_timing(TickLane& L);
   void ensure_in(TickLane::Buf& B, size_t bytes);
   void ensure_out(TickLane& L, size_t bytes);
diff --git a/quorum_amd/csrc/qmx_hip.hip b/quorum_amd/csrc/qmx_hip.hip
--- a/quorum_amd/csrc/qmx_hip.hip
+++ b/quorum_amd/csrc/qmx_hip.hip
@@ -2755,7 +2755,8 @@
 }
 
 void HipEngine::wait_results(TickLane& L, int n, int m, uint32_t seq, const WorkResult* res,
-                             std::chrono::steady_clock::time_point t0, const std::function<void(int)>& on_item) {
+                             std::chrono::steady_clock::time_point t0,
+                             const std::function<void(int, int)>& on_items) {
   using HC = std::chrono::steady_clock;
   static thread_local bool slack = (prctl(PR_SET_TIMERSLACK, 1000UL, 0, 0, 0), true);
   (void)slack;
@@ -2765,13 +2766,16 @@
     nanosleep(&ts, nullptr);
   };
   auto done = [&](int& i) {
-    while (i < n && __atomic_load_n(&res[i].seq, __ATOMIC_ACQUIRE) == seq) on_item(i++);
+    const int i0 = i;
+    while (i < n && __atomic_load_n(&res[i].seq, __ATOMIC_ACQUIRE) == seq) ++i;
+    if (i > i0) on_items(i0, i);
     while (i >= n && i < n + m && __atomic_load_n(&L.h_finres[i - n].seq, __ATOMIC_ACQUIRE) == seq) ++i;
     return i == n + m;
   };
   int i = 0;
   bool revived = false;
   double revive_at = 2e5;
+  if (done(i)) return;
   nap(0.6 * L.ema_us - 6.0 - std::chrono::duration<double, std::micro>(HC::now() - t0).count());
   while (!done(i)) {
     const double el = std::chrono::duration<double, std::micro>(HC::now() - t0).count();
@@ -2827,8 +2831,6 @@
     }
     nap(poll_us_);
   }
-  const double tot = std::chrono::duration<double, std::micro>(HC::now() - t0).count();
-  L.ema_us = 0.85 * L.ema_us + 0.15 * std::min(tot, 2000.0);
 }
 
 void HipEngine::collect_timing(TickLane& L) {
@@ -3238,6 +3240,7 @@
   int dk = 0;
   uint32_t seq = 0;
   bool persist = false, new_params = false, posted = false;
+  bool prep_open = false;
   std::vector<Pending> pend;
   std::vector<int> requeue;
   std::vector<Work*> order;
@@ -3379,8 +3382,11 @@
     }
     if (L.params.dbg != dbg0) ++L.params_ver;
   }
-  J.tp1 = HC::now();
-  L.host_prep_us += std::chrono::duration<double, std::micro>(J.tp1 - J.tp0).count();
+  J.prep_open = grid_ != nullptr && n + J.m > 0;
+  if (!J.prep_open) {
+    J.tp1 = HC::now();
+    L.host_prep_us += std::chrono::duration<double, std::micro>(J.tp1 - J.tp0).count();
+  }
 }
 
 void HipEngine::post(HipJob& J) {
@@ -3397,6 +3403,10 @@
     B.params_ver = L.params_ver;
   }
   J.tp1 = std::chrono::steady_clock::now();
+  if (J.prep_open) {
+    J.prep_open = false;
+    L.host_prep_us += std::chrono::duration<double, std::micro>(J.tp1 - J.tp0).count();
+  }
   roctxRangePushA("qmx_tick");
   L.h2d_bytes += J.in_off;
   J.dk = 0;
@@ -3489,6 +3499,7 @@
   const int n = J.n, m = J.m;
   TickLane::Buf& B = *J.B;
   int n_done = 0;
+  HC::time_point t_done = J.tp1;
   auto process_item = [&](int i) {
     HipJob::Pending& p = J.pend[i];
     SlotCore& c = core_[p.slot];
@@ -3552,12 +3563,17 @@
   if (J.posted) {
     for (const FinalizeReq* r : J.fin_host) finalize_host(*r, fres);
     if (poll_) {
-      wait_results(L, n, m, J.seq, B.h_res, J.tp1, [&](int i) {
+      wait_results(L, n, m, J.seq, B.h_res, J.tp1, [&](int a, int b) {
         const auto ti = HC::now();
         if (n_done == 0) L.first_result_us += std::chrono::duration<double, std::micro>(ti - J.tp1).count();
-        if (i == n_done) process_item(n_done++);
-        L.items_host_us += std::chrono::duration<double, std::micro>(HC::now() - ti).count();
+        for (int i = a; i < b; ++i)
+          if (i == n_done) process_item(n_done++);
+        t_done = HC::now();
+        L.items_host_us += std::chrono::duration<double, std::micro>(t_done - ti).count();
       });
+      if (n == 0 || m > 0) t_done = HC::now();
+      L.ema_us = 0.85 * L.ema_us +
+                 0.15 * std::min(std::chrono::duration<double, std::micro>(t_done - J.tp1).count(), 2000.0);
       uint64_t a = ~0ull, b = 0, t0max = 0;
       double item_ticks = 0;
       for (int i = 0; i < n; ++i) {
@@ -3578,7 +3594,7 @@
           L.lead_ema_us = 0.85 * L.lead_ema_us + 0.15 * std::min((double)(a - ts) * 1e-2, 500.0);
           if (grid_) {
             const double post_h = std::chrono::duration<double, std::micro>(J.tp1.time_since_epoch()).count();
-            const double now_h = std::chrono::duration<double, std::micro>(HC::now().time_since_epoch()).count();
+            const double now_h = std::chrono::duration<double, std::micro>(t_done.time_since_epoch()).count();
             const double lo = post_h - (double)ts * 1e-2, hi = now_h - (double)b * 1e-2;
             if (now_h - L.cwin_t0 > 1e5) {
               L.clo_prev = L.clo;
@@ -3619,9 +3635,10 @@
       wait_stream(L);
       L.timing_pending = true;
       collect_timing(L);
+      t_done = HC::now();
     }
     roctxRangePop();
-    L.gpu_wait_us += std::chrono::duration<double, std::micro>(HC::now() - J.tp1).count();
+    L.gpu_wait_us += std::chrono::duration<double, std::micro>(t_done - J.tp1).count();
     ++L.launches;
     ++L.tpl_launches[J.dk];
     if (grid_) door_busy_[J.dk] = 0;
@@ -3688,6 +3705,7 @@
       }
     }
   }
+  const int n_tail = n - n_done;
   for (; n_done < n; ++n_done) process_item(n_done);
   if (m > 0) collect_finalize(L, J.fin_gpu, fres);
   if (!J.posted)
@@ -3703,7 +3721,8 @@
   }
   J.arena->refs.fetch_sub(1, std::memory_order_release);
   J.B->busy = false;
-  L.process_us += std::chrono::duration<double, std::micro>(HC::now() - J.tp0).count();
+  const bool tail = !J.posted || m > 0 || !J.fin_host.empty() || n_tail > 0 || stage_timing_;
+  L.process_us += std::chrono::duration<double, std::micro>((tail ? HC::now() : t_done) - J.tp0).count();
 }
 
 void HipEngine::run_tick(std::vector<Work>& work, std::vector<FinalizeReq>& fin, int64_t created,
@@ -3720,7 +3739,7 @@
 
 HipEngine::HipJob& HipEngine::hjob(Job& j) {
   if (!j.impl) j.impl = std::make_shared<HipJob>();
-  HipJob& J = *std::static_pointer_cast<HipJob>(j.impl);
+  HipJob& J = *static_cast<HipJob*>(j.impl.get());
   J.work = &j.work;
   J.fin = &j.fin;
   J.created = j.created;
@@ -3733,7 +3752,7 @@
   return k;
 }
 
-bool HipEngine::job_ready(Job& j, double* expect_us) {
+bool HipEngine::job_ready(Job& j, double* expect_us, double now_s) {
   HipJob& J = hjob(j);
   if (expect_us) *expect_us = 0;
   if (!J.posted) return true;
@@ -3745,9 +3764,13 @@
     if (__atomic_load_n(&L.h_finres[i].seq, __ATOMIC_ACQUIRE) != J.seq) goto pending;
   return true;
 pending:
-  if (expect_us)
+  if (expect_us) {
+    using HC = std::chrono::steady_clock;
+    const double now_us = now_s > 0 ? now_s * 1e6
+                                    : std::chrono::duration<double, std::micro>(HC::now().time_since_epoch()).count();
     *expect_us = L.lead_ema_us + L.span_ema_us + 3.0 -
-                 std::chrono::duration<double, std::micro>(std::chrono::steady_clock::now() - J.tp1).count();
+                 (now_us - std::chrono::duration<double, std::micro>(J.tp1.time_since_epoch()).count());
+  }
   return false;
 }
 
diff --git a/quorum_amd/csrc/qmx_server.cpp b/quorum_amd/csrc/qmx_server.cpp
--- a/quorum_amd/csrc/qmx_server.cpp
+++ b/quorum_amd/csrc/qmx_server.cpp
@@ -25,6 +25,7 @@
 #include <cstring>
 #include <memory>
 #include <mutex>
+#include <string_view>
 #include <thread>
 
 #include <functional>
@@ -133,6 +134,7 @@
 template <class F>
 void for_each_header(const char* p, size_t n, F&& f) {
   auto ws = [](char ch) { return ch == ' ' || ch == '\t'; };
+  char kbuf[128];
   size_t pos = 0;
   while (pos < n) {
     const char* e0 = find_crlf(p + pos, n - pos);
@@ -145,21 +147,36 @@
       size_t va = (size_t)(colon - p) + 1, vb = e;
       while (va < vb && ws(p[va])) ++va;
       while (vb > va && (ws(p[vb - 1]) || p[vb - 1] == '\r')) --vb;
-      std::string k(p + ka, kb - ka);
-      for (auto& ch : k) ch = alow((unsigned char)ch);
-      f(std::move(k), std::string(p + va, vb - va));
+      const size_t kn = kb - ka;
+      std::string kheap;
+      char* k = kbuf;
+      if (kn > sizeof(kbuf)) {
+        kheap.resize(kn);
+        k = &kheap[0];
+      }
+      for (size_t i = 0; i < kn; ++i) k[i] = alow((unsigned char)p[ka + i]);
+      f(std::string_view(k, kn), std::string_view(p + va, vb - va));
     }
     pos = e + 2;
   }
 }
-bool ieq(const std::string& s, const char* lw) {
+inline long sv_atol(std::string_view v) {
+  size_t i = 0;
+  while (i < v.size() && (v[i] == ' ' || (v[i] >= '\t' && v[i] <= '\r'))) ++i;
+  bool neg = false;
+  if (i < v.size() && (v[i] == '-' || v[i] == '+')) neg = v[i++] == '-';
+  long r = 0;
+  for (; i < v.size() && v[i] >= '0' && v[i] <= '9'; ++i) r = r * 10 + (v[i] - '0');
+  return neg ? -r : r;
+}
+bool ieq(std::string_view s, const char* lw) {
   size_t n = strlen(lw);
   if (s.size() != n) return false;
   for (size_t i = 0; i < n; ++i)
     if (alow((unsigned char)s[i]) != lw[i]) return false;
   return true;
 }
-bool icontains(const std::string& s, const char* lw) {
+bool icontains(std::string_view s, const char* lw) {
   size_t n = strlen(lw);
   for (size_t i = 0; i + n <= s.size(); ++i) {
     size_t j = 0;
@@ -281,14 +298,14 @@
         for (size_t k = 9; k < le && hp[k] >= '0' && hp[k] <= '9'; ++k) status = status * 10 + (hp[k] - '0');
         bool chunked = false, has_len = false;
         size_t pos = le0 ? le + 2 : hn;
-        for_each_header(hp + pos, hn - pos, [&](std::string&& k, std::string&& v) {
+        for_each_header(hp + pos, hn - pos, [&](std::string_view k, std::string_view v) {
           if (k == "transfer-encoding" && icontains(v, "chunked")) chunked = true;
           if (k == "content-length") {
             has_len = true;
-            remaining = atol(v.c_str());
+            remaining = sv_atol(v);
           }
           if (k == "connection" && ieq(v, "close")) close = true;
-          if (keep_headers) headers.emplace_back(std::move(k), std::move(v));
+          if (keep_headers) headers.emplace_back(std::string(k), std::string(v));
         });
         if (status == 204 || status == 304) phase = 7;
         else if (chunked) phase = 2;
@@ -347,6 +364,14 @@
     if (d == p) buf.assign(p + i, n - i);
     else buf.erase(0, i);
     return 0;
+  }
+  void reset() {
+    phase = status = 0;
+    keep_headers = true;
+    headers.clear();
+    remaining = 0;
+    close = false;
+    buf.clear();
   }
   bool done() const { return phase == 7; }
   const std::string* header(const std::string& k) const {
@@ -414,11 +439,12 @@
 
 enum SKind { K_PAR, K_SINGLE, K_NONSTREAM, K_REMOTE };
 struct Session {
+  bool live = false;
   Client* cl = nullptr;
   SKind kind = K_PAR;
   JVal body;
   std::string raw;
-  std::vector<std::pair<std::string, std::string>> fwd;
+  std::string fwd;
   std::string auth;
   std::vector<BState> bs;
   int finished = 0;
@@ -890,9 +916,10 @@
   ~Loop() {
     for (int fd : {lfd_, afd_})
       if (fd >= 0) close(fd);
-    for (auto& kv : idle_ssl_) SSL_free(kv.second);
-    for (auto& kv : ups_)
-      if (kv.second->ssl) SSL_free(kv.second->ssl);
+    for (SSL* x : idle_ssl_)
+      if (x) SSL_free(x);
+    for (Up* u : ups_)
+      if (u && u->ssl) SSL_free(u->ssl);
   }
 
   void run() {
@@ -910,12 +937,14 @@
     }
     std::vector<epoll_event> evs(512);
     double last_sweep = now_s();
+    double t_pass_end = 0;
     while (!g_stop.load()) {
       if (pace_s_ > 0 && small_reads_ >= pace_min_reads_) {
         const double due = tnow_ + pace_s_, t = now_s();
         if (t < due) {
           timespec ts{0, (long)((due - t) * 1e9)};
           nanosleep(&ts, nullptr);
+          t_pass_end = 0;
           c_paced++;
         }
       }
@@ -932,7 +961,7 @@
         for (int k = 0; k < 2 && !ready; ++k) {
           double e = 0;
           if (!job_live_[k]) continue;
-          ready = aeng_->job_ready(job_[k], &e);
+          ready = aeng_->job_ready(job_[k], &e, t_pass_end);
           exp_us = std::min(exp_us, e);
         }
         if (ready || exp_us <= spin_us_) {
@@ -1000,13 +1029,13 @@
         fds.clear();
         fds.swap(pending_requests_);
         for (int fd : fds) {
-          auto it = clients_.find(fd);
-          if (it != clients_.end() && !it->second->sess && !it->second->dead) process_requests(it->second.get());
+          Client* c = client_at(fd);
+          if (c && !c->sess && !c->dead) process_requests(c);
           if (req_check_ && jobs_live_ && any_ready()) loop_tick();
         }
       }
-      double t = now_s();
-      if (stall_log_) ph[3] = t;
+      const double t = tnow_;
+      if (stall_log_) ph[3] = now_s();
       if (t - last_sweep > 0.1) {
         sweep_timeouts(t);
         last_sweep = t;
@@ -1042,7 +1071,8 @@
       if (!flushq_.empty()) flush_queued();
       if (!pending_close_.empty()) reap_clients();
       flush_x();
-      const double pass = now_s() - tnow_;
+      t_pass_end = now_s();
+      const double pass = t_pass_end - tnow_;
       if (stall_log_) pass_t0_.store(0.0, std::memory_order_relaxed);
       if (pass > 1e-3) {
         c_loop_pass_1ms++;
@@ -1082,9 +1112,8 @@
   void release_deferred(double t) {
     size_t k = 0;
     for (size_t i = 0; i < deferq_.size(); ++i) {
-      auto it = clients_.find(deferq_[i].fd);
-      if (it == clients_.end()) continue;
-      Client* c = it->second.get();
+      Client* c = client_at(deferq_[i].fd);
+      if (!c) continue;
       if (c->serial != deferq_[i].serial) continue;
       if (c->queued || c->want_out || c->dead || c->out_off >= c->out.size()) {
         unhold(c);
@@ -1177,13 +1206,11 @@
     if (kind == 5) return on_xmsgs();
     if (kind == 7) return on_link(fd, e.events);
     if (kind == 3) {
-      auto it = clients_.find(fd);
-      if (it != clients_.end()) on_client(it->second.get(), e.events);
+      if (Client* c = client_at(fd)) on_client(c, e.events);
       return;
     }
     if (kind == 4) {
-      auto it = ups_.find(fd);
-      if (it != ups_.end()) on_up(it->second.get(), e.events);
+      if (Up* u = up_at(fd)) on_up(u, e.events);
       else on_parked(fd);
       return;
     }
@@ -1210,7 +1237,7 @@
     j.created = (int64_t)time(nullptr);
     j.lane = 0;
     if (!eng_->job_take(j, fin_ok)) return;
-    job_t_post_[k] = now_s();
+    job_t_post_[k] = j.t_take > 0 ? j.t_take : now_s();
     eng_->job_prepare(j);
     eng_->job_post(j);
     job_live_[k] = true;
@@ -1226,6 +1253,7 @@
     job_live_[k] = false;
     --jobs_live_;
     eng_->settle(taken_);
+    for (auto& w : j.work) body_put(w.data);
     h_tick.observe(now_s() - job_t_post_[k]);
     if (ver_) ver_->check(j.created, rb.r, rb.f);
     c_ticks++;
@@ -1269,13 +1297,13 @@
   }
   void apply(ResultBatch& rb) {
     for (auto& r : rb.r) {
-      auto it = slot_owner_.find(r.slot);
-      if (it == slot_owner_.end() || it->second.gen != r.gen) {
+      const SlotOwner* so = (size_t)r.slot < slot_owner_.size() ? &slot_owner_[r.slot] : nullptr;
+      if (!so || !so->s || so->gen != r.gen) {
         r.hold = ViewRef();
         continue;
       }
-      Session* s = it->second.s;
-      int bi = it->second.bi;
+      Session* s = so->s;
+      int bi = so->bi;
       if (fault_drop_every_ > 0 && !r.empty() && ++fault_n_ % fault_drop_every_ == 0)
         r.clear_sse();
       if (!r.empty()) {
@@ -1321,12 +1349,12 @@
       slot = eng_->open(index, f, e, &gen);
       if (heng_ && slot >= loop_slots_) c_host_path_opens++;
       else if (heng_ && light_host_ > 0) {
-        sess_ema_ = 0.95 * sess_ema_ + 0.05 * (double)sessions_.size();
+        sess_ema_ = 0.95 * sess_ema_ + 0.05 * (double)n_sessions_;
         if (jobs_live_ == 0 && sess_ema_ <= (double)light_host_) heng_->host_open(slot);
       }
       if (ver_ && verify) ver_->open(slot, gen, index, f, e);
     }
-    slot_owner_[slot] = SlotOwner{s, bi, gen};
+    grow(slot_owner_, slot, SlotOwner{nullptr, 0, 0}) = SlotOwner{s, bi, gen};
     return slot;
   }
   void e_feed_move(int slot, std::string& d) {
@@ -1372,14 +1400,15 @@
         *l = -1;
       }
     }
-    for (auto& kv : clients_) {
-      Client* c = kv.second.get();
+    for (auto& cp : clients_) {
+      Client* c = cp.get();
+      if (!c) continue;
       const bool idle = !c->sess && c->in.empty() && c->out_off >= c->out.size();
       if (idle && (c->served > 0 || t - c->t_accept > 1.0)) mark_close(c);
     }
     if (!flushq_.empty()) flush_queued();
     if (!pending_close_.empty()) reap_clients();
-    return (sessions_.empty() && clients_.empty()) || t > drain_deadline_;
+    return (n_sessions_ == 0 && n_clients_ == 0) || t > drain_deadline_;
   }
 
   void on_accept(int lfd) {
@@ -1393,7 +1422,9 @@
       c->serial = ++next_serial_;
       c->t_accept = lnow();
       add(fd, EPOLLIN, tag(3, fd));
+      if ((size_t)fd >= clients_.size()) clients_.resize(std::max((size_t)fd + 1, 2 * clients_.size()));
       clients_[fd] = std::move(c);
+      ++n_clients_;
       c_clients++;
     }
   }
@@ -1401,9 +1432,8 @@
     std::vector<int> fds;
     fds.swap(pending_close_);
     for (int fd : fds) {
-      auto it = clients_.find(fd);
-      if (it == clients_.end()) continue;
-      Client* c = it->second.get();
+      Client* c = client_at(fd);
+      if (!c) continue;
       if (c->dead || (c->close_after && c->out_off >= c->out.size())) close_client(c);
     }
   }
@@ -1439,7 +1469,8 @@
     epoll_ctl(ep_, EPOLL_CTL_DEL, c->fd, nullptr);
     cnt(SC_EPOLL_CTL);
     close(c->fd);
-    clients_.erase(c->fd);
+    --n_clients_;
+    clients_[c->fd].reset();
   }
   void write_client(Client* c, const std::string& data) {
     if (c->dead) return;
@@ -1479,9 +1510,8 @@
     fds.clear();
     fds.swap(flushq_);
     for (int fd : fds) {
-      auto it = clients_.find(fd);
-      if (it == clients_.end()) continue;
-      Client* c = it->second.get();
+      Client* c = client_at(fd);
+      if (!c) continue;
       c->queued = false;
       unhold(c);
       if (c->dead || c->want_out) continue;
@@ -1548,22 +1578,35 @@
       method.assign(head, sp1);
       target.assign(head + sp1 + 1, sp2 - sp1 - 1);
       const bool http10 = le - sp2 - 1 == 8 && memcmp(head + sp2 + 1, "HTTP/1.0", 8) == 0;
-      std::vector<std::pair<std::string, std::string>> hdrs;
-      hdrs.reserve(12);
       const size_t pos = le + 2;
       long clen = 0;
       bool chunked = false;
       bool keepalive = !http10;
-      for_each_header(head + std::min(pos, he), he - std::min(pos, he), [&](std::string&& k, std::string&& v) {
-        if (k == "content-length") clen = atol(v.c_str());
+      ReqHead& rq = reqh_;
+      rq.fwd.clear();
+      rq.auth.clear();
+      rq.has_auth = rq.has_ctype = false;
+      for_each_header(head + std::min(pos, he), he - std::min(pos, he), [&](std::string_view k, std::string_view v) {
+        if (k == "content-length") clen = sv_atol(v);
         if (k == "transfer-encoding" && icontains(v, "chunked")) chunked = true;
         if (k == "connection") {
           if (ieq(v, "close")) keepalive = false;
           if (ieq(v, "keep-alive")) keepalive = true;
         }
-        hdrs.emplace_back(std::move(k), std::move(v));
+        if (k == "host") return;
+        if (k == "authorization") {
+          rq.has_auth = true;
+          rq.auth.assign(v.data(), v.size());
+          return;
+        }
+        if (k == "content-type") rq.has_ctype = true;
+        if (k == "content-length" || k == "transfer-encoding" || k == "connection" || k == "keep-alive" || k == "te" ||
+            k == "upgrade" || k == "accept-encoding")
+          return;
+        rq.fwd.append(k).append(": ").append(v).append("\r\n");
       });
-      std::string body;
+      std::string& body = req_body_;
+      body.clear();
       size_t used;
       if (chunked) {
         size_t i = he + 4;
@@ -1590,12 +1633,12 @@
         used = i;
       } else {
         if (c->in.size() < he + 4 + (size_t)clen) return;
-        body = c->in.substr(he + 4, clen);
+        body.assign(c->in, he + 4, clen);
         used = he + 4 + clen;
       }
       c->in.erase(0, used);
       c->keepalive = keepalive && !draining_;
-      handle_request(c, method, target, hdrs, body);
+      handle_request(c, method, target, body);
       if (!c->sess && !c->keepalive) {
         mark_close(c);
         return;
@@ -1608,8 +1651,7 @@
     write_client(c, http_response(status, ctype, body, extra));
   }
 
-  void handle_request(Client* c, const std::string& method, std::string target,
-                      std::vector<std::pair<std::string, std::string>>& hdrs, std::string& body) {
+  void handle_request(Client* c, const std::string& method, std::string target, std::string& body) {
     size_t q = target.find('?');
     if (q != std::string::npos) target.resize(q);
     if (method == "GET" && target == "/health") return respond(c, 200, "application/json", "{\"status\":\"healthy\"}");
@@ -1627,7 +1669,15 @@
     if (method != "POST") return respond(c, 405, "application/json", "{\"detail\":\"Method Not Allowed\"}");
     c_requests++;
     c->served++;
-    auto s = std::make_unique<Session>();
+    Session* const s = sess_get();
+    struct Unused {
+      Loop* l;
+      Session* s;
+      bool started;
+      ~Unused() {
+        if (!started) l->sess_put(s);
+      }
+    } unused{this, s, false};
     s->t0 = lnow();
     std::string perr;
     if (!json_parse(body.data(), body.size(), s->body, &perr)) {
@@ -1643,21 +1693,8 @@
     }
     const JVal* sv = s->body.get("stream");
     bool streaming = sv && sv->truthy();
-    bool has_auth = false, has_ctype = false;
-    s->fwd.reserve(hdrs.size() + 2);
-    for (auto& h : hdrs) {
-      if (h.first == "host") continue;
-      if (h.first == "authorization") {
-        has_auth = true;
-        s->auth = h.second;
-        continue;
-      }
-      if (h.first == "content-type") has_ctype = true;
-      if (h.first == "content-length" || h.first == "transfer-encoding" || h.first == "connection" ||
-          h.first == "keep-alive" || h.first == "te" || h.first == "upgrade" || h.first == "accept-encoding")
-        continue;
-      s->fwd.push_back(std::move(h));
-    }
+    const bool has_auth = reqh_.has_auth, has_ctype = reqh_.has_ctype;
+    if (has_auth) s->auth = reqh_.auth;
     if (!has_auth) {
       std::string env_key = cfg_.env_api_key;
       if (cfg_.api_key_from_env) {
@@ -1672,8 +1709,9 @@
       }
       s->auth = "Bearer " + env_key;
     }
-    s->fwd.emplace_back("Authorization", s->auth);
-    if (!has_ctype) s->fwd.emplace_back("Content-Type", "application/json");
+    s->fwd = reqh_.fwd;
+    s->fwd.append("Authorization: ").append(s->auth).append("\r\n");
+    if (!has_ctype) s->fwd.append("Content-Type: application/json\r\n");
     if (!valid_init_) {
       valid_init_ = true;
       for (int i = 0; i < (int)cfg_.backends.size(); ++i)
@@ -1690,10 +1728,12 @@
                        err_json("Model must be specified when config.yaml model is blank", "invalid_request_error"));
     }
     bool parallel = cfg_.has_iterations_and_strategy && valid.size() > 1;
-    s->raw = std::move(body);
+    s->raw.swap(body);
     s->cl = c;
-    Session* sp = s.get();
-    sessions_[sp] = std::move(s);
+    Session* sp = s;
+    s->live = true;
+    unused.started = true;
+    ++n_sessions_;
     c->sess = sp;
     if (streaming && parallel) start_parallel(sp, valid);
     else if (streaming) start_single(sp, valid[0]);
@@ -1748,52 +1788,41 @@
     out = s->raw;
     return true;
   }
-  std::string build_req(const BackendCfg& be, const std::vector<std::pair<std::string, std::string>>& hdrs,
-                        const std::string& body) {
-    size_t n = be.path.size() + be.host.size() + body.size() + 96;
-    for (auto& h : hdrs) n += h.first.size() + h.second.size() + 4;
-    std::string r;
-    r.reserve(n);
-    r.append("POST ").append(be.path).append("/chat/completions HTTP/1.1\r\nhost: ").append(be.host);
+  void build_req(const BackendCfg& be, const std::string& hdrs, const std::string& body, std::string& r) {
+    r.clear();
+    r.reserve(be.req_head.size() + hdrs.size() + body.size() + 48);
+    r.append(be.req_head).append(hdrs);
     char num[24];
-    if (be.port != (be.https ? 443 : 80)) {
-      r += ':';
-      r.append(num, (size_t)dec_str(num, (size_t)be.port));
-    }
-    r.append("\r\n");
-    for (auto& h : hdrs) r.append(h.first).append(": ").append(h.second).append("\r\n");
     r.append("content-length: ").append(num, (size_t)dec_str(num, body.size())).append("\r\n\r\n");
     r.append(body);
-    return r;
-  }
-  Up* open_up(Session* s, int bi, int backend, UpMode mode, std::string req, double timeout) {
+  }
+  bool open_up(Session* s, int bi, int backend, UpMode mode, std::string& req, double timeout) {
     const BackendCfg& be = cfg_.backends[backend];
-    auto u = std::make_unique<Up>();
+    if (!be.resolved || (be.https && !tls_)) return false;
+    Up* const u = up_get();
     u->backend = backend;
     u->sess = s;
     u->bi = bi;
     u->mode = mode;
     u->rp.keep_headers = mode != UP_ENGINE;
-    u->req = std::move(req);
+    u->req.swap(req);
     u->timeout = timeout;
     u->last_io = lnow();
     u->t_open = u->last_io;
     u->deadline = cfg_.total_timeout > 0 ? u->last_io + cfg_.total_timeout : 0;
-    if (!be.resolved || (be.https && !tls_)) return nullptr;
     int fd = -1;
     auto& pool = idle_[backend];
     while (!pool.empty() && fd < 0) {
       fd = pool.back();
       pool.pop_back();
-      if (!parked_.count(fd)) {
+      if (parked_at(fd) < 0) {
         fd = -1;
         continue;
       }
       u->reused = true;
-      auto it = idle_ssl_.find(fd);
-      if (it != idle_ssl_.end()) {
-        u->ssl = it->second;
-        idle_ssl_.erase(it);
+      if ((size_t)fd < idle_ssl_.size() && idle_ssl_[fd]) {
+        u->ssl = idle_ssl_[fd];
+        idle_ssl_[fd] = nullptr;
       }
     }
     if (fd < 0) {
@@ -1803,7 +1832,8 @@
       int r = connect(fd, (const sockaddr*)&be.addr, sizeof(be.addr));
       if (r != 0 && errno != EINPROGRESS) {
         close(fd);
-        return nullptr;
+        up_put(u);
+        return false;
       }
       u->connecting = r != 0;
       c_up_conns++;
@@ -1822,15 +1852,16 @@
       }
     } else {
       u->fd = fd;
-      parked_.erase(fd);
-    }
-    Up* p = u.get();
-    ups_[fd] = std::move(u);
-    if (!p->connecting) {
-      if (p->tls_hs) tls_step(p);
-      else write_up(p);
-    }
-    return p;
+      parked_[fd] = -1;
+    }
+    grow(ups_, fd, (Up*)nullptr) = u;
+    if (bi >= 0) s->bs[bi].up = u;
+    else s->agg = u;
+    if (!u->connecting) {
+      if (u->tls_hs) tls_step(u);
+      else write_up(u);
+    }
+    return true;
   }
   void tls_step(Up* u) {
     ERR_clear_error();
@@ -1923,13 +1954,18 @@
     }
     if ((ev & (EPOLLOUT | (u->ssl ? EPOLLIN : 0))) && u->req_off < u->req.size()) {
       write_up(u);
-      if (ups_.find(fd) == ups_.end()) return;
+      if (up_at(fd) != u) return;
       if (u->req_off < u->req.size()) return;
     }
     if (ev & (EPOLLIN | EPOLLHUP | EPOLLERR)) {
       char buf[65536];
       bool eof = false;
-      std::string body;
+      struct BodyBuf {
+        Loop* l;
+        std::string s;
+        ~BodyBuf() { l->body_put(s); }
+      } bb{this, body_get()};
+      std::string& body = bb.s;
       while (true) {
         ssize_t r = up_read(u, buf, sizeof(buf));
         if (r > 0) {
@@ -1951,7 +1987,7 @@
       if (!u->headers_seen && u->rp.phase > 0) {
         u->headers_seen = true;
         on_up_headers(u);
-        if (ups_.find(fd) == ups_.end()) return;
+        if (up_at(fd) != u) return;
       }
       if (!body.empty()) on_up_body(u, body);
       if (u->rp.done()) return up_complete(u, true);
@@ -1970,17 +2006,15 @@
     std::string req = u->req;
     double to = u->timeout;
     drop_up(u, false);
-    Up* nu = open_up(s, bi, backend, mode, req, to);
-    if (!nu) return fail_backend(s, bi, 500, "All connection attempts failed", "proxy_error");
-    if (bi >= 0) s->bs[bi].up = nu;
-    else s->agg = nu;
+    if (!open_up(s, bi, backend, mode, req, to))
+      return fail_backend(s, bi, 500, "All connection attempts failed", "proxy_error");
   }
   void drop_up(Up* u, bool reuse) {
     int fd = u->fd;
     if (reuse && !u->rp.close && !u->tls_hs && !u->out_armed) {
       idle_[u->backend].push_back(fd);
-      parked_[fd] = u->backend;
-      if (u->ssl) idle_ssl_[fd] = u->ssl;
+      grow(parked_, fd, -1) = u->backend;
+      if (u->ssl) grow(idle_ssl_, fd, (SSL*)nullptr) = u->ssl;
     } else {
       epoll_ctl(ep_, EPOLL_CTL_DEL, fd, nullptr);
       cnt(SC_EPOLL_CTL);
@@ -1988,18 +2022,18 @@
       close(fd);
     }
     u->ssl = nullptr;
-    ups_.erase(fd);
+    ups_[fd] = nullptr;
+    up_put(u);
   }
   void on_parked(int fd) {
-    auto it = parked_.find(fd);
-    if (it == parked_.end()) return;
-    auto& pool = idle_[it->second];
+    const int be = parked_at(fd);
+    if (be < 0) return;
+    auto& pool = idle_[be];
     pool.erase(std::remove(pool.begin(), pool.end(), fd), pool.end());
-    parked_.erase(it);
-    auto s = idle_ssl_.find(fd);
-    if (s != idle_ssl_.end()) {
-      SSL_free(s->second);
-      idle_ssl_.erase(s);
+    parked_[fd] = -1;
+    if ((size_t)fd < idle_ssl_.size() && idle_ssl_[fd]) {
+      SSL_free(idle_ssl_[fd]);
+      idle_ssl_[fd] = nullptr;
     }
     epoll_ctl(ep_, EPOLL_CTL_DEL, fd, nullptr);
     cnt(SC_EPOLL_CTL);
@@ -2016,15 +2050,12 @@
   }
   void sweep_timeouts(double t) {
     std::vector<int> expired;
-    for (auto& kv : ups_) {
-      Up* u = kv.second.get();
-      if (t - u->last_io > u->timeout || (u->deadline > 0 && t > u->deadline)) expired.push_back(kv.first);
-    }
+    for (Up* u : ups_)
+      if (u && (t - u->last_io > u->timeout || (u->deadline > 0 && t > u->deadline))) expired.push_back(u->fd);
     for (int fd : expired) {
-      auto it = ups_.find(fd);
-      if (it != ups_.end()) {
+      if (Up* u = up_at(fd)) {
         c_fail_timeout++;
-        up_error(it->second.get(), "");
+        up_error(u, "");
       }
     }
   }
@@ -2247,7 +2278,7 @@
     if (defer && s->cl->queued && !flushq_.empty() && flushq_.back() == s->cl->fd) {
       flushq_.pop_back();
       s->cl->queued = false;
-      deferq_.push_back(Deferred{s->cl->fd, s->cl->serial, now_s() + role_defer_s_});
+      deferq_.push_back(Deferred{s->cl->fd, s->cl->serial, lnow() + role_defer_s_});
     }
     s->bs.resize(valid.size());
     const bool spread = xch_ && xch_->healthy() && (xch_->world() > 1 || self_spread_);
@@ -2271,7 +2302,8 @@
       s->bs[i].slot = e_open(s, (int)i, (int)i, s->filter, s->emit);
     }
     for (size_t i = 0; i < valid.size(); ++i) {
-      std::string body, msg;
+      std::string& body = body_scratch_;
+      std::string msg;
       int st = 0;
       const char* et = nullptr;
       if (!upstream_body(s, valid[i], body, &st, &msg, &et)) {
@@ -2289,14 +2321,14 @@
         m.skey = s->skey;
         m.a = valid[i];
         m.b = (int)(cfg_.timeout * 1000.0);
-        m.payload = build_req(cfg_.backends[valid[i]], s->fwd, body);
+        build_req(cfg_.backends[valid[i]], s->fwd, body, m.payload);
         xq(m, s->bs[i].via_link);
         s->bs[i].t_sp_open = now_s();
         continue;
       }
-      Up* u = open_up(s, (int)i, valid[i], UP_ENGINE, build_req(cfg_.backends[valid[i]], s->fwd, body), cfg_.timeout);
-      if (!u) fail_backend(s, (int)i, 500, "All connection attempts failed", "proxy_error");
-      else s->bs[i].up = u;
+      build_req(cfg_.backends[valid[i]], s->fwd, body, req_scratch_);
+      if (!open_up(s, (int)i, valid[i], UP_ENGINE, req_scratch_, cfg_.timeout))
+        fail_backend(s, (int)i, 500, "All connection attempts failed", "proxy_error");
     }
   }
   std::vector<int> good_slots(Session* s) {
@@ -2563,11 +2595,11 @@
         for (auto& kv : rsess_) owners.push_back(kv.second);
         for (auto& kv : shadow_) shadows.push_back(kv.second);
         for (Session* s : shadows)
-          if (sessions_.count(s) && (m.a < 0 || s->owner_rank == m.a) && !s->bulk_pending &&
+          if (s->live && (m.a < 0 || s->owner_rank == m.a) && !s->bulk_pending &&
               (!link_only || s->via_link))
             end_session(s);
         for (Session* s : owners) {
-          for (int i = 0; i < (int)s->bs.size() && sessions_.count(s); ++i)
+          for (int i = 0; i < (int)s->bs.size() && s->live; ++i)
             if (s->bs[i].remote >= 0 && (m.a < 0 || s->bs[i].remote == m.a) && s->bs[i].state == 0 &&
                 (!link_only || s->bs[i].via_link)) {
               c_sp_down++;
@@ -2577,9 +2609,9 @@
         continue;
       }
       if (m.type == X_OPEN) {
-        auto sp = std::make_unique<Session>();
-        Session* s = sp.get();
-        sessions_[s] = std::move(sp);
+        Session* s = sess_get();
+        s->live = true;
+        ++n_sessions_;
         s->kind = K_REMOTE;
         s->owner_rank = m.src_rank;
         s->owner_loop = m.src_loop;
@@ -2593,10 +2625,8 @@
         s->bs[0].slot = e_open(s, 0, m.bi, s->filter, s->emit);
         shadow_[{m.skey, m.bi}] = s;
         c_remote_streams++;
-        Up* u = (m.a >= 0 && m.a < (int)cfg_.backends.size())
-                    ? open_up(s, 0, m.a, UP_ENGINE, std::move(m.payload), m.b / 1000.0) : nullptr;
-        if (!u) fail_backend(s, 0, 500, "All connection attempts failed", "proxy_error");
-        else s->bs[0].up = u;
+        if (!(m.a >= 0 && m.a < (int)cfg_.backends.size() && open_up(s, 0, m.a, UP_ENGINE, m.payload, m.b / 1000.0)))
+          fail_backend(s, 0, 500, "All connection attempts failed", "proxy_error");
         continue;
       }
       if (m.type == X_CANCEL || m.type == X_SENT) {
@@ -2788,12 +2818,10 @@
     msgs.a.push_back(m);
     req.set("messages", msgs);
     req.set("stream", JVal::boolean(false));
-    std::vector<std::pair<std::string, std::string>> h = {{"Authorization", s->auth},
-                                                          {"Content-Type", "application/json"}};
+    const std::string h = "Authorization: " + s->auth + "\r\nContent-Type: application/json\r\n";
     if (!be.valid || !be.has_model_key) return on_aggregator_done(s, 500, std::string());
-    Up* u = open_up(s, -1, ab, UP_BUFFER, build_req(be, h, json_dumps(req)), 60.0);
-    if (!u) return on_aggregator_done(s, 500, std::string());
-    s->agg = u;
+    build_req(be, h, json_dumps(req), req_scratch_);
+    if (!open_up(s, -1, ab, UP_BUFFER, req_scratch_, 60.0)) return on_aggregator_done(s, 500, std::string());
   }
   void on_aggregator_done(Session* s, int status, const std::string& body) {
     JVal j;
@@ -2827,9 +2855,9 @@
     int st = 0;
     const char* et = nullptr;
     if (!upstream_body(s, backend, body, &st, &msg, &et)) return fail_backend(s, 0, st, msg, et);
-    Up* u = open_up(s, 0, backend, UP_PASS, build_req(cfg_.backends[backend], s->fwd, body), cfg_.timeout);
-    if (!u) return fail_backend(s, 0, 500, "All connection attempts failed", "proxy_error");
-    s->bs[0].up = u;
+    build_req(cfg_.backends[backend], s->fwd, body, req_scratch_);
+    if (!open_up(s, 0, backend, UP_PASS, req_scratch_, cfg_.timeout))
+      return fail_backend(s, 0, 500, "All connection attempts failed", "proxy_error");
   }
   static bool bare_role(const std::string& ev) {
     std::string t = ev;
@@ -2889,15 +2917,13 @@
       const char* et = nullptr;
       if (!upstream_body(s, valid[i], body, &st, &msg, &et)) {
         fail_backend(s, (int)i, st, msg, et);
-        if (sessions_.find(s) == sessions_.end()) return;
+        if (!s->live) return;
         continue;
       }
-      Up* u = open_up(s, (int)i, valid[i], UP_BUFFER, build_req(cfg_.backends[valid[i]], s->fwd, body), cfg_.timeout);
-      if (!u) {
+      build_req(cfg_.backends[valid[i]], s->fwd, body, req_scratch_);
+      if (!open_up(s, (int)i, valid[i], UP_BUFFER, req_scratch_, cfg_.timeout)) {
         fail_backend(s, (int)i, 500, "All connection attempts failed", "proxy_error");
-        if (sessions_.find(s) == sessions_.end()) return;
-      } else {
-        s->bs[i].up = u;
+        if (!s->live) return;
       }
     }
   }
@@ -3048,7 +3074,7 @@
   void end_session(Session* s) {
     if (s->stage == 3) return;
     s->stage = 3;
-    if (s->kind != K_REMOTE && s->t0 > 0) h_latency.observe(now_s() - s->t0);
+    if (s->kind != K_REMOTE && s->t0 > 0) h_latency.observe(lnow() - s->t0);
     if (s->kind == K_REMOTE) shadow_.erase({s->owner_skey, s->shadow_bi});
     if (s->skey) {
       rsess_.erase(s->skey);
@@ -3072,7 +3098,7 @@
       }
       const bool reusable = !(b.remote >= 0 && xch_ && s->skey) || xch_->forget_bulk(s->skey, i, b.slot, idx_);
       if (b.slot >= 0) {
-        slot_owner_.erase(b.slot);
+        if ((size_t)b.slot < slot_owner_.size()) slot_owner_[b.slot].s = nullptr;
         if (reusable) e_release(b.slot);
         else c_sp_release_deferred++;
         b.slot = -1;
@@ -3084,7 +3110,9 @@
     }
     if (s->fin_id >= 0) fin_owner_.erase(s->fin_id);
     Client* c = s->cl;
-    sessions_.erase(s);
+    s->live = false;
+    --n_sessions_;
+    sess_put(s);
     if (c) {
       c->sess = nullptr;
       if (!c->keepalive || c->dead) mark_close(c);
@@ -3232,15 +3260,114 @@
   std::mutex rmu_;
   std::vector<ResultBatch> rq_;
   std::atomic<bool> rq_pending_{false};
-  std::unordered_map<int, std::unique_ptr<Client>> clients_;
-  std::unordered_map<int, std::unique_ptr<Up>> ups_;
-  std::unordered_map<Session*, std::unique_ptr<Session>> sessions_;
+  template <class T>
+  static T& grow(std::vector<T>& v, int i, const T& empty) {
+    if ((size_t)i >= v.size()) v.resize(std::max((size_t)i + 1, 2 * v.size()), empty);
+    return v[i];
+  }
+  std::vector<std::unique_ptr<Client>> clients_;
+  int n_clients_ = 0;
+  Client* client_at(int fd) const { return (size_t)fd < clients_.size() ? clients_[fd].get() : nullptr; }
+  std::vector<Up*> ups_;
+  Up* up_at(int fd) const { return (size_t)fd < ups_.size() ? ups_[fd] : nullptr; }
+  int parked_at(int fd) const { return (size_t)fd < parked_.size() ? parked_[fd] : -1; }
+  std::vector<std::unique_ptr<Session>> sess_all_;
+  std::vector<Session*> sess_free_;
+  int n_sessions_ = 0;
+  std::vector<std::unique_ptr<Up>> up_all_;
+  std::vector<Up*> up_free_;
+  static void recycle(std::string& x) {
+    if (x.capacity() > (256u << 10)) std::string().swap(x);
+    else x.clear();
+  }
+  Session* sess_get() {
+    if (sess_free_.empty()) {
+      sess_all_.emplace_back(new Session());
+      return sess_all_.back().get();
+    }
+    Session* s = sess_free_.back();
+    sess_free_.pop_back();
+    return s;
+  }
+  void sess_put(Session* s) {
+    s->live = false;
+    s->cl = nullptr;
+    s->kind = K_PAR;
+    s->body = JVal();
+    recycle(s->raw);
+    recycle(s->fwd);
+    recycle(s->auth);
+    s->bs.clear();
+    s->finished = 0;
+    s->filter = s->emit = true;
+    s->stage = 0;
+    s->fin_id = -1;
+    s->fin_texts = false;
+    s->texts.clear();
+    s->text_names.clear();
+    s->agg = nullptr;
+    s->msplit = false;
+    recycle(s->mpre);
+    recycle(s->mpost);
+    recycle(s->first_buf);
+    s->first_decided = s->saw_done = s->pass_started = false;
+    recycle(s->done_tail);
+    recycle(s->role_model_json);
+    s->t0 = 0;
+    s->skey = 0;
+    s->remote_n = 0;
+    s->owner_rank = -1;
+    s->owner_loop = s->shadow_bi = 0;
+    s->via_link = false;
+    s->owner_skey = 0;
+    s->data_sent = 0;
+    s->bulk_pending = s->fetching = s->fetched = false;
+    recycle(s->fetched_text);
+    s->first_content = false;
+    sess_free_.push_back(s);
+  }
+  std::vector<std::string> body_free_;
+  std::string body_get() {
+    if (body_free_.empty()) return std::string();
+    std::string b = std::move(body_free_.back());
+    body_free_.pop_back();
+    return b;
+  }
+  void body_put(std::string& b) {
+    if (b.capacity() < 512 || b.capacity() > (256u << 10) || body_free_.size() >= 64) return;
+    b.clear();
+    body_free_.push_back(std::move(b));
+  }
+  Up* up_get() {
+    if (up_free_.empty()) {
+      up_all_.emplace_back(new Up());
+      return up_all_.back().get();
+    }
+    Up* u = up_free_.back();
+    up_free_.pop_back();
+    return u;
+  }
+  void up_put(Up* u) {
+    u->fd = u->backend = u->bi = -1;
+    u->sess = nullptr;
+    u->mode = UP_BUFFER;
+    recycle(u->req);
+    u->req_off = 0;
+    u->connecting = u->reused = u->got_bytes = u->headers_seen = false;
+    u->rp.reset();
+    recycle(u->body);
+    u->last_io = u->deadline = u->t_open = 0;
+    u->timeout = 60;
+    u->ssl = nullptr;
+    u->tls_hs = u->out_armed = false;
+    up_free_.push_back(u);
+  }
   struct SlotOwner {
     Session* s;
     int bi;
     uint32_t gen;
   };
-  std::unordered_map<int, SlotOwner> slot_owner_;
+  std::vector<SlotOwner> slot_owner_;
   std::unordered_map<int, std::pair<Session*, int>> fin_owner_;
   Exchange* xch_ = nullptr;
   bool draining_ = false;
@@ -3254,6 +3381,11 @@
   bool valid_init_ = false;
   std::mutex xmu_;
   std::vector<XMsg> xin_;
+  struct ReqHead {
+    std::string fwd, auth;
+    bool has_auth = false, has_ctype = false;
+  } reqh_;
+  std::string req_scratch_, body_scratch_, req_body_;
   std::vector<std::string> xout_;
   bool xpending_ = false;
   std::vector<XLink> xl_;
@@ -3262,8 +3394,8 @@
   std::unordered_map<uint64_t, Session*> rsess_;
   std::map<std::pair<uint64_t, int>, Session*> shadow_;
   std::vector<std::vector<int>> idle_;
-  std::unordered_map<int, SSL*> idle_ssl_;
-  std::unordered_map<int, int> parked_;
+  std::vector<SSL*> idle_ssl_;
+  std::vector<int> parked_;
   SSL_CTX* tls_ = nullptr;
   std::vector<int> pending_close_, pending_requests_;
   std::vector<int> flushq_;
@@ -3345,6 +3477,9 @@
   prof_start();
   bool any_https = false;
   for (auto& b : cfg.backends) {
+    b.req_head = "POST " + b.path + "/chat/completions HTTP/1.1\r\nhost: " + b.host;
+    if (b.port != (b.https ? 443 : 80)) b.req_head += ":" + std::to_string(b.port);
+    b.req_head += "\r\n";
     if (!b.valid || b.host.empty()) continue;
     any_https = any_https || b.https;
     addrinfo hints{}, *res = nullptr;
diff --git a/quorum_amd/csrc/qmx_server.h b/quorum_amd/csrc/qmx_server.h
--- a/quorum_amd/csrc/qmx_server.h
+++ b/quorum_amd/csrc/qmx_server.h
@@ -16,6 +16,7 @@
   bool https = false;
   sockaddr_in addr{};
   bool resolved = false;
+  std::string req_head;
 };
 
 struct ServerCfg {
```

Result: faster. 433,300, median of 6 (+7.3%).
